# nicolasavru/objective-slam

Hardware: AMD Instinct MI355X
Metric: scene_ppf_votes_per_sec (higher is better)
Workload: dtype f32; 1 GPU; 5k-point model vs 100k-point scene (BASELINE.json metric config), one resident model table, Model::ppf_lookup per step; model_points=5000, scene_points=100000, ref_point_df=8, ref_points_per_gpu=12500, vote_mode=exact, parallelism=scene-ref-shard x1, exchange=single GPU

## Files before the change

include/oslam.h:

```cpp
#ifndef OSLAM_H
#define OSLAM_H

#include <stddef.h>
#include <stdint.h>

#ifdef __cplusplus
extern "C" {
#endif

#define OSLAM_OK 0
#define OSLAM_E_INVALID 1
#define OSLAM_E_DEVICE 2
#define OSLAM_E_NOMEM 3
#define OSLAM_E_NO_VOTES 4
#define OSLAM_E_LIMIT 5
#define OSLAM_E_PEER 6

#define OSLAM_VOTE_EXACT 0
#define OSLAM_VOTE_FAST 1

typedef struct oslam_params {
    unsigned ref_point_df;
    float vote_count_threshold;
    int cpu_clustering;
    int use_l1_norm;
    int use_averaged_clusters;
    int dev;
    int vote_mode;
    int shard_rank;
    int shard_world;
    unsigned max_cells;
    unsigned pose_gpu_min;
    int no_bucket_spread;
    unsigned scratch_gib;
    int pose_two_sorts;
    int vote_order;
    int reserved[1];
} oslam_params;

typedef struct oslam_stats {
    uint64_t num_scene_ppfs;
    uint64_t num_hits;
    uint64_t num_votes;
    uint64_t num_unique_votes;
    uint64_t num_model_keys;
    uint64_t num_top;
    uint32_t max_count;
    uint32_t num_emitted;
    float ms_vote;
    float ms_total;
    uint32_t vote_launches;
    float ms_vote_kernel;
    float ms_key_kernel;
    uint32_t wide_workgroups;
    uint64_t num_pairs_probed;
    uint64_t scratch_bytes;
    uint64_t num_entries_streamed;
    uint64_t num_items;
} oslam_stats;

typedef struct oslam_cell {
    uint64_t code;
    uint32_t count;
    uint32_t pad;
} oslam_cell;

typedef struct oslam_model oslam_model;
typedef struct oslam_scene oslam_scene;

int oslam_params_default(oslam_params *p);

int oslam_d_dist_from_cloud(const float *xyz, size_t n, size_t stride_bytes, float tau_d,
                            float *d_dist_out);

int oslam_model_create(const float *xyz, const float *nrm, size_t n, size_t stride_bytes,
                       float d_dist, const oslam_params *params, oslam_model **out);
void oslam_model_destroy(oslam_model *m);

int oslam_model_save(const oslam_model *m, const char *path);
int oslam_model_load(const char *path, const oslam_params *params, oslam_model **out);
int oslam_model_info(const oslam_model *m, size_t *n_points, float *d_dist, uint64_t *table_bytes);

int oslam_model_set_point_weights(oslam_model *m, const float *weights, size_t n);

int oslam_scene_create(const float *xyz, const float *nrm, size_t n, size_t stride_bytes,
                       float d_dist, unsigned ref_point_downsample_factor,
                       const oslam_params *params, oslam_scene **out);
void oslam_scene_destroy(oslam_scene *s);

int oslam_align(oslam_model *m, oslam_scene *s, float T_rowmajor[16], oslam_stats *stats);

int oslam_align_prepare(oslam_model *m, oslam_scene *s);

typedef struct oslam_db oslam_db;
int oslam_db_create(oslam_model *const *models, size_t n, oslam_db **out);
void oslam_db_destroy(oslam_db *db);
void oslam_db_destroy_with_models(oslam_db *db);
int oslam_db_align(oslam_db *db, oslam_scene *s, float *T_out, oslam_stats *stats);
int oslam_db_size(const oslam_db *db, size_t *n_models, size_t *n_groups);

int oslam_ppf_registration(const float *const *scene_xyz, const float *const *scene_nrm,
                           const size_t *scene_n, size_t n_scenes, const float *const *model_xyz,
                           const float *const *model_nrm, const size_t *model_n, size_t n_models,
                           size_t stride_bytes, const float *model_d_dists,
                           unsigned ref_point_downsample_factor, float vote_count_threshold,
                           int cpu_clustering, int use_l1_norm, int use_averaged_clusters, int devUse,
                           const float *model_weights, float *T_out);

int oslam_ht_dist(const float A[16], const float B[16], float out[2]);

int oslam_voxel_grid(const float *xyz, const float *nrm, size_t n, size_t stride_bytes, float leaf,
                     int dev, float *xyz_out, float *nrm_out, size_t cap, size_t *n_out);

typedef struct oslam_camera {
    float fx, fy, cx, cy;
    float depth_scale;
    float z_min, z_max;
    float max_jump;
} oslam_camera;
int oslam_depth_to_cloud(const void *depth, int depth_is_u16, int width, int height, const oslam_camera *cam,
// ... 594 lines not shown
    uint32_t hits;
    uint32_t normals;
    uint32_t bricks;
    uint32_t window_bricks;
    uint32_t launches;
    int32_t anchor[3], box_lo[3], box_hi[3];
    float ms_total;
} oslam_world_raycast_result;

int oslam_world_raycast_params_default(oslam_world_raycast_params *p);
int oslam_world_raycast(oslam_world *w, oslam_volume *vol, const oslam_world_raycast_params *rp, const float T_vol_cam[16],
                        const oslam_camera *cam, int width, int height, oslam_view **view_out, oslam_world_raycast_result *res);
int oslam_world_track(oslam_world *w, oslam_volume *vol, const oslam_world_raycast_params *rp, oslam_view *v,
                      const float T_vol_cam_prev[16], const oslam_egomotion_params *ep, float T_vol_cam_out[16],
                      oslam_egomotion_result *ego_res);

#define OSLAM_NORMALS_SWEEPS 4
typedef struct oslam_normals_params {
    float radius;
    unsigned min_neighbours;
    float viewpoint[3];
    int orient;
    float line_ratio;
    int reserved[4];
} oslam_normals_params;

typedef struct oslam_normals_result {
    uint32_t n_valid;
    uint32_t n_cells;
    float edge;
    uint32_t launches;
    float ms_total;
    float ms_grid, ms_kernel;
} oslam_normals_result;

int oslam_normals_params_default(oslam_normals_params *p);
int oslam_cloud_normals(const float *xyz, size_t n, size_t stride_bytes, const oslam_normals_params *np, int dev,
                        float *nrm_out, float *curvature_out, uint8_t *valid_out, oslam_normals_result *res);
int oslam_cloud_normal_moments(const float *xyz, size_t n, size_t stride_bytes, const oslam_normals_params *np, int dev,
                               int64_t *moments_out);
int oslam_mesh_normals(const float *xyz, size_t nv, size_t stride_bytes, const uint32_t *tri, size_t nt, float *nrm_out,
                       uint8_t *valid_out);
int oslam_ply_read_mesh(const char *path, float **xyz_out, float **nrm_out, uint32_t **tri_out, size_t *nv_out,
                        size_t *nt_out);

typedef struct oslam_colour_params {
    unsigned max_weight;
    float band;
    int reserved[6];
} oslam_colour_params;

int oslam_view_set_colour(oslam_view *v, const uint8_t *rgb, size_t row_stride_bytes, const uint8_t *valid);
int oslam_view_colour(oslam_view *v, uint32_t *rgba_out);
int oslam_view_has_colour(const oslam_view *v);
int oslam_colour_params_default(oslam_colour_params *p);
int oslam_volume_colour_enable(oslam_volume *vol, const oslam_colour_params *cp);
int oslam_volume_colour_words(oslam_volume *vol, uint32_t *words_out);
int oslam_volume_set_colour_words(oslam_volume *vol, const uint32_t *words);
int oslam_volume_integrate_colour(oslam_volume *vol, const oslam_view *v, const oslam_view *c, const float T_vol_cam[16],
                                  oslam_integrate_result *res, uint32_t *coloured_out);
int oslam_volume_colours(oslam_volume *vol, const float *xyz, size_t n, size_t stride_bytes, uint8_t *rgb_out,
                         uint8_t *valid_out, size_t *n_valid_out);
int oslam_volume_paint_view(oslam_volume *vol, const float T_vol_cam[16], oslam_view *v, uint32_t *painted_out);
int oslam_ply_write_colour(const char *path, const float *xyz, const float *nrm, const uint8_t *rgb, size_t n, int binary);
int oslam_ply_write_mesh_colour(const char *path, const float *xyz, const float *nrm, const uint8_t *rgb, size_t nv,
                                const uint32_t *tri, size_t nt, int binary);
int oslam_world_colours(oslam_world *w, oslam_volume *vol, const oslam_world_surface_params *sp, const float *xyz, size_t n,
                        size_t stride_bytes, uint8_t *rgb_out, uint8_t *valid_out, size_t *n_valid_out);
int oslam_world_paint_view(oslam_world *w, oslam_volume *vol, const oslam_world_surface_params *sp, const float T_vol_cam[16],
                           oslam_view *v, uint32_t *painted_out);

int oslam_scene_keys(oslam_scene *s, size_t ref_index, uint32_t *keys_out);
int oslam_model_keys(oslam_model *m, size_t ref_index, uint32_t *keys_out);
int oslam_model_bucket(oslam_model *m, uint32_t key, uint32_t *pairs_out, size_t cap,
                       size_t *count_out);
int oslam_model_bucket_words(oslam_model *m, uint32_t key, int slice, uint32_t *words_out, size_t cap,
                             size_t *count_out);
int oslam_model_key_numbers(oslam_model *m, uint32_t *keys_out, uint32_t *numbers_out, uint64_t *weights_out, size_t cap,
                            size_t *n_out);
int oslam_vote_ref_order(const uint32_t *keep, size_t n, uint32_t *order_out);
int oslam_vote_accumulator(oslam_model *m, oslam_scene *s, size_t ref_index, uint32_t *acc_out);
int oslam_vote_hits(oslam_model *m, oslam_scene *s, size_t ref_index, uint32_t *numbers_out, uint32_t *theta_out,
                    uint32_t *idx_out, size_t cap, size_t *n_out, uint32_t *keep_out);
int oslam_sort_hits_tap(const uint32_t *numbers, const uint32_t *theta, const uint32_t *idx, const uint32_t *offsets,
                        const uint32_t *counts, size_t n_lists, uint32_t id_bits, int dev, uint32_t *numbers_out,
                        uint32_t *theta_out, uint32_t *idx_out, uint32_t *runs_out, uint32_t *run_counts_out);
int oslam_last_cells(oslam_model *m, oslam_cell *cells_out, float *poses_out, size_t cap,
                     size_t *n_out);
int oslam_tail_scores(oslam_model *m, oslam_scene *s, const oslam_cell *cells, size_t n, uint32_t global_max, int path,
                      oslam_cell *cells_out, float *scores_out, size_t cap, size_t *n_out, uint32_t *max_idx_out,
                      float T[16], int *path_out);

int oslam_set_stream(void *hip_stream);
int oslam_release_scratch(int dev);
const char *oslam_last_error(void);
int oslam_set_host_threads(int n);
int oslam_selftest_math(size_t n, uint64_t seed, uint64_t *mismatches);

#ifdef __cplusplus
}
#endif
#endif
```

objective-slam_amd/csrc/oslam_host.c:

```c
#include <pthread.h>
#include <stdio.h>

#include "oslam_internal.h"

static __thread char g_err[512];
static __thread void *g_stream;

const char *oslam_last_error(void) { return g_err; }

int oslam_set_stream(void *hip_stream)
{
    g_stream = hip_stream;
    return OSLAM_OK;
}

void *oslam_stream(void) { return g_stream; }

int oslam_fail(int code, const char *what)
{
    if (what != g_err) snprintf(g_err, sizeof g_err, "%s", what);
    return code;
}

int oslam_fail_call(const char *call, int err, const char *file, int line)
{
    snprintf(g_err, sizeof g_err, "%s: %s (%s:%d)", call, hipGetErrorString((hipError_t)err), file, line);
    return OSLAM_E_DEVICE;
}

int oslam_params_default(oslam_params *p)
{
    if (!p) return fail(OSLAM_E_INVALID, "params is NULL");
    memset(p, 0, sizeof *p);
    p->ref_point_df = 1;
    p->vote_count_threshold = 0.4f;
    p->cpu_clustering = 0;
    p->use_l1_norm = 0;
    p->use_averaged_clusters = 0;
    p->dev = 0;
    p->vote_mode = OSLAM_VOTE_EXACT;
    p->shard_rank = 0;
    p->shard_world = 1;
    p->max_cells = 1u << 22;
    p->pose_gpu_min = 0;
    p->no_bucket_spread = 0;
    p->scratch_gib = 0;
    p->vote_order = 0;
    return OSLAM_OK;
}

int oslam_d_dist_from_cloud(const float *xyz, size_t n, size_t stride_bytes, float tau_d,
                            float *d_dist_out)
{
    float lo[3], hi[3], ext;
    size_t i;
    int a;
    if (!xyz || !d_dist_out || n == 0 || stride_bytes < 12) return fail(OSLAM_E_INVALID, "bad cloud");
    for (a = 0; a < 3; a++) lo[a] = hi[a] = xyz[a];
    for (i = 1; i < n; i++) {
        const float *p = (const float *)((const char *)xyz + i * stride_bytes);
        for (a = 0; a < 3; a++) {
            if (p[a] < lo[a]) lo[a] = p[a];
            if (p[a] > hi[a]) hi[a] = p[a];
        }
    }
    ext = hi[0] - lo[0];
    if (hi[1] - lo[1] > ext) ext = hi[1] - lo[1];
    if (hi[2] - lo[2] > ext) ext = hi[2] - lo[2];
    *d_dist_out = tau_d * ext;
    return OSLAM_OK;
}

int oslam_pick_device(int dev_req, int *dev_out)
{
    int n = 0;
    hipError_t e = hipGetDeviceCount(&n);
    if (e != hipSuccess || n <= 0) return fail(OSLAM_E_DEVICE, "no HIP device available (the PPF path has no CPU fallback)");
    if (dev_req < 0) dev_req = 0;
    *dev_out = dev_req < n - 1 ? dev_req : n - 1;
    e = hipSetDevice(*dev_out);
    if (e != hipSuccess) return fail(OSLAM_E_DEVICE, hipGetErrorString(e));
    return OSLAM_OK;
}

#define DEVCACHE_SLOTS 64
#define DEVCACHE_MAX_BLOCK ((size_t)1 << 30)
typedef struct {
    void *p;
    size_t bytes;
    int dev, used;
} devblock;
static devblock g_devcache[DEVCACHE_SLOTS];
static pthread_mutex_t g_devcache_mu = PTHREAD_MUTEX_INITIALIZER;

int oslam_dev_alloc(void **out, size_t bytes)
{
    int dev = 0, i, best = -1, spare = -1;
    hipError_t e;
    size_t want;
    *out = NULL;
    if (bytes == 0) bytes = 16;
    if (hipGetDevice(&dev) != hipSuccess) return (int)hipErrorInvalidDevice;
    pthread_mutex_lock(&g_devcache_mu);
    for (i = 0; i < DEVCACHE_SLOTS; i++) {
        devblock *b = &g_devcache[i];
        if (!b->p) { if (spare < 0) spare = i; continue; }
        if (b->used || b->dev != dev || b->bytes < bytes || b->bytes > 2 * bytes + 65536) continue;
        if (best < 0 || b->bytes < g_devcache[best].bytes) best = i;
    }
    if (best >= 0) {
        g_devcache[best].used = 1;
        *out = g_devcache[best].p;
        pthread_mutex_unlock(&g_devcache_mu);
        return 0;
    }
    want = bytes <= DEVCACHE_MAX_BLOCK ? bytes + bytes / 8 + 256 : bytes;
    e = hipMalloc(out, want);
    if (e != hipSuccess) {
        (void)hipGetLastError();
        for (i = 0; i < DEVCACHE_SLOTS; i++)
            if (g_devcache[i].p && !g_devcache[i].used && g_devcache[i].dev == dev) {
                (void)hipFree(g_devcache[i].p);
                memset(&g_devcache[i], 0, sizeof g_devcache[i]);
                if (spare < 0) spare = i;
            }
        want = bytes;
        e = hipMalloc(out, want);
    }
    if (e == hipSuccess && spare >= 0 && want <= DEVCACHE_MAX_BLOCK) {
        g_devcache[spare].p = *out;
// ... 35 lines not shown
```

objective-slam_amd/csrc/oslam_internal.h:

```cpp
#ifndef OSLAM_INTERNAL_H
#define OSLAM_INTERNAL_H

#include <hip/hip_runtime_api.h>
#include <limits.h>
#include <stddef.h>
#include <stdint.h>
#include <stdlib.h>
#include <string.h>
#include <time.h>

#include "oslam.h"
#include "oslam_kernels.h"
#include "oslam_rigid.h"

typedef struct cloud_buf {
    int n;
    float *h_xyz, *h_nrm;
    float *d_soa;
    oslamk_cloud k;
} cloud_buf;

struct oslam_model {
    int dev;
    cloud_buf c;
// ... 73 lines not shown
    int dev;
    oslam_view *view;
    size_t n_hyp;
    int32_t *d_labels;
    float *d_tol;
};

typedef struct db_group {
    int n;
    size_t *members;
    uint32_t *ukeys, *reach, *kmap, *uids;
} db_group;

struct oslam_db {
    int dev;
    size_t n;
    oslam_model **models;
    int n_groups;
    db_group *groups;
};

int oslam_fail(int code, const char *what);
static inline int fail(int code, const char *what) { return oslam_fail(code, what); }
int oslam_fail_call(const char *call, int err, const char *file, int line);

#define KCHK(call)                                                                          \
    do {                                                                                    \
        const int k_ = (int)(call);                                                         \
        if (k_ != 0) { rc = oslam_fail_call(#call, k_, __FILE__, __LINE__); goto done; }    \
    } while (0)
#define HIPCHK(call) KCHK(call)

static inline double now_ms(void)
{
    struct timespec ts;
    clock_gettime(CLOCK_MONOTONIC, &ts);
    return ts.tv_sec * 1e3 + ts.tv_nsec * 1e-6;
}

static inline size_t align256(size_t b) { return (b + 255) & ~(size_t)255; }

static inline int oslam_counters_open(uint32_t **d_cnt, size_t n_words, void *stream)
{
    const int k = oslam_dev_alloc((void **)d_cnt, 256 + sizeof(uint32_t) * n_words);
    return k != 0 ? k : (int)hipMemsetAsync(*d_cnt, 0, 256, (hipStream_t)stream);
}

static inline void split_points(const float *pts6, size_t n, float *xyz_out, float *nrm_out)
{
    size_t i;
    for (i = 0; i < n; i++) {
        memcpy(xyz_out + 3 * i, pts6 + 6 * i, 3 * sizeof(float));
        memcpy(nrm_out + 3 * i, pts6 + 6 * i + 3, 3 * sizeof(float));
    }
}

void *oslam_stream(void);
int oslam_pick_device(int dev_req, int *dev_out);

void oslam_cloud_free(cloud_buf *c);
int oslam_cloud_make(cloud_buf *c, const float *xyz, const float *nrm, size_t stride, const float *d_aos6, size_t n);
oslamk_cloud oslam_soa_cloud(const float *d_soa, size_t n);
int oslam_depth_points(const void *depth, int depth_is_u16, int width, int height, const oslam_camera *cam, int dev,
                       void **d_img, float **d_pts6, uint32_t *np);

int oslam_build_kmap(oslamk_table *t, float d_dist, const oslamk_table *parts, int n_parts, int vote_order);
int oslam_build_union(oslam_model *m, uint32_t distinct, uint32_t *d_n_keys, uint32_t *d_overflow);
int oslam_build_uinfo(oslam_model *m);

void oslam_refine_release_grids(oslam_scene *s);

typedef struct scratch_pool scratch_pool;
int oslam_check_pair(const oslam_model *m, const oslam_scene *s);
int oslam_pool_enter(int dev, scratch_pool **pool);
void oslam_pool_unlock(scratch_pool *p);
int oslam_pool_reserve_counts(scratch_pool *p, size_t n_ref);
void oslam_ref_order(const uint32_t *keep, size_t n, uint32_t *order);
typedef struct oslam_vote_times {
    float ms;
    float ms_vote_kernel, ms_key_kernel;
    uint32_t launches;
    uint64_t probed;
} oslam_vote_times;
int oslam_pool_read_hits(const scratch_pool *p, uint32_t *numbers_out, uint32_t *theta_out, uint32_t *idx_out, size_t cap,
                         size_t *n_out, uint32_t *keep_out);
int oslam_run_votes_group(scratch_pool *pool, oslam_model *const *ms, int nm, oslam_scene *s, const uint32_t *d_ref_idx,
                          const float *d_tsg, int n_ref, uint32_t fixed_gmax, uint32_t *acc_dump, oslamk_counters *cnt,
                          oslam_vote_times *t);
void oslam_vote_stats(oslam_stats *st, const scratch_pool *pool, const oslam_model *m, const oslam_scene *s,
                      const oslamk_counters *cnt, const oslam_vote_times *t);
int oslam_vote_records(scratch_pool *pool, oslam_model *m, oslam_scene *s, oslamk_counters *cnt, size_t *n_cells,
                       oslam_stats *st, int to_host);
int oslam_grow_records(oslam_model *m, uint64_t need);
int oslam_cluster_scores_on_device(size_t n, const float *trans, const float *quat, const float *wv,
                                   const int32_t *cell, const uint32_t *hash_idx, float d_dist, int use_l1,
                                   float *score);

typedef struct oslam_inst_req {
    oslamk_inst_args a;
    const oslam_instance_params *ip;
    float extent;
} oslam_inst_req;
size_t oslam_pose_gpu_from(const oslam_model *m);
void oslam_drop_last(oslam_model *m);
int oslam_pose_tables(oslam_model *m, oslam_scene *s);
int oslam_ensure_pose_buffers(oslam_model *m, size_t n);
const float *oslam_rotx(void);
int oslam_finish_after_votes(oslam_model *m, oslam_scene *s, size_t n, uint32_t gmax, int try_device, float T[16],
                             oslam_stats *stats, const oslam_inst_req *req, oslamk_inst_out *sel);

int oslam_db_align_frame(oslam_db *db, oslam_scene *s, float *T_out, oslam_stats *stats, const oslam_inst_req *reqs,
                         oslamk_inst_out *sels);

int oslam_refine_check_params(const oslam_refine_params *rp, oslam_refine_params *out);
int oslam_refine_check_rigid(const float T[16]);
int oslam_refine_members(oslam_model *const *ms, size_t n, oslam_scene *s, const float *T_in, const oslam_refine_params *p,
                         float *T_out, oslam_refine_result *res);

int oslam_view_check_pair(const oslam_model *m, const oslam_view *v);
int oslam_check_poses(oslam_model *const *ms, const float *T, size_t n, int hypotheses);
int oslam_check_handles(oslam_model *const *ms, const float *T, size_t n, const oslam_view *v);
int oslam_view_camera_ok(const oslam_camera *cam, int width, int height, int with_depth_scale, int with_max_jump);
int oslam_view_new(int dev, int width, int height, const oslam_camera *cam, oslam_view **out);
void oslam_view_camera(const oslam_view *v, oslam_camera *cam);

int oslam_verify_check_params(const oslam_verify_params *vp, oslam_verify_params *out);
void oslam_verify_fill_result(oslam_verify_result *r, const uint32_t *c, const oslam_verify_params *p);
void oslam_verify_set_member(oslamk_verify_member *d, const oslam_model *m, const float T[16], float depth_tol);
int oslam_verify_members(oslam_model *const *ms, size_t n, const oslam_view *v, const float *T, const oslam_verify_params *p,
                         oslam_verify_result *res);

int oslam_track_check_params(const oslam_track_params *tp, oslam_track_params *out);
void oslam_track_release_maps(oslam_view *v);
void oslam_track_release(void);
int oslam_track_view_maps(oslam_view *v, int *built);
void oslam_ego_release(void);
int oslam_ego_check_params(const oslam_egomotion_params *ep, oslam_egomotion_params *out);
int oslam_ego_check_pyramid_schedule(const oslam_egomotion_params *p, unsigned n_levels);
typedef struct oslam_ego_pair {
    oslam_view *src, *dst;
    unsigned lattice;
} oslam_ego_pair;
int oslam_ego_run(const oslam_ego_pair *pair, const float T0[16], const oslam_egomotion_params *p, float T_out[16],
                  oslam_egomotion_result *res);
int oslam_pyramid_check_params(const oslam_pyramid_params *pp, oslam_pyramid_params *out);
void oslam_volume_lock(void);
void oslam_volume_unlock(void);
static inline size_t oslam_volume_bytes(const oslam_volume_params *p)
{
    return (size_t)p->nx * (size_t)p->ny * (size_t)p->nz * sizeof(uint32_t);
}
int oslam_volume_integrate_views(oslam_volume *vol, const oslam_view *v, const oslam_view *c, const float T_vol_cam[16],
                                 oslam_integrate_result *res, uint32_t *coloured);
void oslam_colour_release_view(oslam_view *v);
int oslam_surface_check_params(const oslam_surface_params *sp, oslam_surface_params *out);
int oslam_volume_surface_cloud(oslam_volume *vol, unsigned min_weight, int *dev, float **d_pts6, uint32_t *np);
struct oslam_world_stage;
int oslam_world_stage_fit(struct oslam_world_stage *st, size_t bytes);
int oslam_world_surface_check_params(const oslam_world_surface_params *sp, oslam_world_surface_params *out);
int oslam_world_surface_cloud(oslam_world *w, oslam_volume *vol, const oslam_world_surface_params *p, int *dev, float **d_pts6,
                              uint32_t *np);
typedef struct oslam_world_map {
    oslamk_brick_map m;
    uint8_t *d_map;
    uint32_t bricks, window_bricks, launches;
    int32_t anchor[3];
// ... 16 lines not shown
```

objective-slam_amd/csrc/oslam_kernels.h:

```cpp
#ifndef OSLAM_KERNELS_H
#define OSLAM_KERNELS_H

#include <stddef.h>
#include <stdint.h>

#ifdef __cplusplus
extern "C" {
#endif

#define OSLAMK_SLICE 2046
#define OSLAMK_ROWS 1024
#define OSLAMK_NBIN 32

typedef struct oslamk_slot {
    uint32_t key;
    uint32_t start;
    uint32_t len;
    uint32_t cur;
} oslamk_slot;

typedef struct oslamk_uv {
    float uy, uz;
} oslamk_uv;

typedef struct oslamk_entries {
    uint32_t *e4;
    oslamk_uv *uv;
    uint16_t *mi;
    uint32_t *pw;
    oslamk_uv *puv;
    uint16_t *pdir;
    uint32_t n_real;
} oslamk_entries;
#define OSLAMK_PSEG 4096
#ifndef OSLAMK_PDIR_SHIFT
#define OSLAMK_PDIR_SHIFT 0
#endif
#define OSLAMK_PDIR_CELLS_RAW(m) ((m) <= 1u ? 1u : 1u << (31 - __builtin_clz((m) - 1u)))
#define OSLAMK_PDIR_CELLS(n) (OSLAMK_PDIR_CELLS_RAW((n) << OSLAMK_PDIR_SHIFT) > 4096u ? 4096u : OSLAMK_PDIR_CELLS_RAW((n) << OSLAMK_PDIR_SHIFT))

typedef struct oslamk_cloud {
    const float *px, *py, *pz, *nx, *ny, *nz;
    int n;
} oslamk_cloud;

typedef struct oslamk_order {
    const float *sx, *sy, *sz;
    const uint32_t *perm;
    const float *box;
} oslamk_order;
#define OSLAMK_ORDER_GROUP 64

typedef struct oslamk_uinfo {
    uint32_t start;
    uint32_t len;
} oslamk_uinfo;

typedef struct oslamk_table {
    oslamk_slot *slots;
    uint32_t cap;
    uint32_t shift;
    int n_slices;
    uint32_t *ukeys;
    uint32_t ucap;
    uint32_t ushift;
    uint32_t *reach;
    uint32_t reach_words;
    uint32_t *kmap;
    uint32_t kmap_bins;
    uint32_t *uids;
    uint32_t n_ids, id_bits, uinfo_stride;
    oslamk_uinfo *uinfo;
} oslamk_table;
#define OSLAMK_UWEIGHTS(t) ((unsigned long long *)((t).uids + (t).ucap))
#define OSLAMK_KMAP_NONE 0xffffffffu
#define OSLAMK_KMAP_MAX_BINS 2048

#define OSLAMK_REACH_BINS 16384

typedef struct oslamk_counters {
    unsigned long long hits;
    unsigned long long votes;
    unsigned long long nonzero_cells;
    uint32_t gmax;
    uint32_t out_count;
    uint32_t redo_count;
    uint32_t redo_total;
    unsigned long long entries;
    unsigned long long items;
    unsigned long long prof[4];
    uint32_t list_overflow;
    uint32_t pad_;
} oslamk_counters;

typedef struct oslamk_cell {
    unsigned long long code;
    uint32_t count;
    uint32_t pad;
} oslamk_cell;

int oslamk_row_keys(oslamk_cloud c, int ref, float d_dist, float inv_d_dist, uint32_t *keys_out,
                    void *stream);

int oslamk_model_count(oslamk_cloud c, float d_dist, float inv_d_dist, oslamk_table t,
                       uint32_t *n_unique, uint32_t *overflow, void *stream);
int oslamk_table_scan(oslamk_table t, uint32_t *total_out, void *stream);
int oslamk_union_build(oslamk_table t, uint32_t *n_keys, uint32_t *overflow, void *stream);
int oslamk_reach_build(oslamk_table t, float d_dist, void *stream);
int oslamk_union_weights(oslamk_table t, unsigned long long *weights, void *stream);
int oslamk_kmap_build(oslamk_table t, float d_dist, void *stream);
int oslamk_model_fill(oslamk_cloud c, float d_dist, float inv_d_dist, oslamk_table t,
                      const float *tmg, oslamk_entries ent, void *stream);

int oslamk_bucket_spread(oslamk_table t, oslamk_entries ent, void *stream);
int oslamk_bucket_psort(oslamk_table t, oslamk_entries ent, void *stream);

typedef struct oslamk_pay {
    uint32_t theta_t22;
    uint32_t idx;
} oslamk_pay;

typedef struct oslamk_run {
    uint32_t slot_r;
    uint32_t first;
} oslamk_run;
#define OSLAMK_RUN_SHIFT 26

typedef struct oslamk_vote_args {
    oslamk_cloud scene;
    const uint32_t *ref_idx;
    const float *tsg;
    int n_ref;
    float d_dist, inv_d_dist;
    oslamk_table table;
    oslamk_entries ent;
    float thresh;
    uint32_t fixed_gmax;
    oslamk_counters *counters;
    oslamk_cell *out;
    uint32_t out_cap;
    uint32_t *acc_dump;
    int dump_ref;
    int first_ref;
    int n_launch;
    int mode;
    uint32_t *keep_count;
    const uint32_t *hit_off;
    uint32_t *hit_key;
    oslamk_pay *hit_pay;
    oslamk_pay *hit_sorted;
    oslamk_run *runs;
    uint32_t *hit_count;
    uint32_t *run_count;
    uint32_t *redo;
    const uint32_t *ref_order;
    oslamk_order order;
} oslamk_vote_args;

int oslamk_uinfo_build(oslamk_table t, void *stream);

int oslamk_scene_count(const oslamk_vote_args *a, void *stream);
int oslamk_scene_hits(const oslamk_vote_args *a, void *stream);
int oslamk_sort_hits(const oslamk_vote_args *a, void *stream);
int oslamk_vote(const oslamk_vote_args *a, void *stream);
int oslamk_vote_wide(const oslamk_vote_args *a, void *stream);
int oslamk_vote_group(const oslamk_vote_args *d_all, const oslamk_vote_args *h_all, int nm, void *stream);

int oslamk_voxel_grid(oslamk_cloud c, float leaf, float *out6, uint32_t *n_out, void *stream);

int oslamk_depth_to_cloud(const void *d_img, int is_u16, int w, int h, float fx, float fy, float cx, float cy,
                          float scale, float z_min, float z_max, float max_jump, float *d_out6, uint32_t *n_out,
                          void *stream);

int oslam_dev_alloc(void **p, size_t bytes);
void oslam_dev_free(void *p);
void oslam_dev_cache_release(int dev);

int oslamk_aos6_to_soa(const float *d_in6, size_t n, float *d_soa, void *stream);

int oslamk_cluster_scores(int n, const int *cell, const uint32_t *shash, const uint32_t *sidx,
                          const float *sq, const float *st, const float *sw, float d_dist, int use_l1,
                          float *score, int whole_host, const unsigned long long *whole_dev, uint32_t *table, void *stream);
size_t oslamk_cluster_table_words(int n);

#define OSLAMK_MAX_INSTANCES 64
typedef struct oslamk_inst_args {
    uint32_t max_instances;
    float ratio, sep2, cos_thr;
    int32_t rot_on;
    float c[3];
} oslamk_inst_args;
typedef struct oslamk_inst_out {
    uint32_t n;
    uint32_t idx[OSLAMK_MAX_INSTANCES];
    float score[OSLAMK_MAX_INSTANCES];
    float T[OSLAMK_MAX_INSTANCES][16];
} oslamk_inst_out;

int oslamk_pose_stage(const oslamk_cell *d_cells_in, uint32_t n_in, float min_votecount, const float *d_Tm16,
                      const float *d_Ts16, uint32_t df, const float *d_weights, const float *h_rotx_cs, float d_dist,
                      int use_l1, oslamk_cell *d_cells_out, float *d_poses, uint32_t gmax, uint32_t model_points,
                      uint32_t scene_points, int two_sorts, const oslamk_inst_args *ia, uint32_t *n_out, uint32_t *best_out,
                      float T_best[16], oslamk_inst_out *inst, void *stream);

int oslamk_pose_reserve(uint32_t n_max, uint32_t slots, const float *h_rotx_cs, void *stream);
int oslamk_pose_select_async(const oslamk_cell *d_in, uint32_t n_in, float min_votecount, oslamk_cell *d_sel, uint32_t slot,
                             void *stream);
uint32_t oslamk_pose_selected(uint32_t slot);
int oslamk_pose_finish_async(uint32_t n, const oslamk_cell *d_sel, const float *d_Tm16, const float *d_Ts16, uint32_t df,
                             const float *d_weights, float d_dist, int use_l1, oslamk_cell *d_cells_out, float *d_poses,
                             uint32_t gmax, uint32_t model_points, uint32_t scene_points, int two_sorts,
                             const oslamk_inst_args *ia, uint32_t slot, void *stream);
void oslamk_pose_result(uint32_t slot, uint32_t *best_out, float T_best[16]);
int oslamk_pose_scores(uint32_t n, float *h_score, void *stream);
void oslamk_pose_instances(uint32_t slot, oslamk_inst_out *out);

int oslamk_select_cells(const oslamk_cell *d_in, uint32_t n_in, float min_votecount, oslamk_cell *d_out, uint32_t *n_out,
                        void *stream);
void oslamk_pose_release(void);

int oslamk_selftest(const float *x, const float *y, const float *x2, size_t n, float *out_acos,
                    float *out_atan2, uint32_t *out_quant, uint32_t *out_bin, void *stream);

#define OSLAMK_REFINE_THREADS 256
#define OSLAMK_REFINE_SUMS 29
#define OSLAMK_REFINE_STRIDE 32
#define OSLAMK_SCAN_ITEMS 4096
#define OSLAMK_GRID_MAX_CELLS (1u << 24)
#define OSLAMK_REFINE_STEP 0
#define OSLAMK_REFINE_SCORE 1
#define OSLAMK_REFINE_TAP 2

typedef struct oslamk_grid {
    double lo[3];
    double inv_edge;
    int dim[3];
    uint32_t n_cells;
    int n;
    uint32_t *start;
    float *pts;
    uint32_t *local;
    uint32_t *bsum;
// ... 328 lines not shown
```

objective-slam_amd/csrc/oslam_model.c:

```c
#include <stdio.h>

#include "oslam_internal.h"
#include "oslam_pose.h"
#include "ppf_core.h"

void oslam_model_destroy(oslam_model *m)
{
    if (!m) return;
    (void)hipSetDevice(m->dev);
    oslam_cloud_free(&m->c);
    if (m->table.slots) (void)hipFree(m->table.slots);
    if (m->ent.e4) (void)hipFree(m->ent.e4);
    if (m->ent.uv) (void)hipFree(m->ent.uv);
    if (m->ent.pw) (void)hipFree(m->ent.pw);
    if (m->ent.puv) (void)hipFree(m->ent.puv);
    if (m->ent.pdir) (void)hipFree(m->ent.pdir);
    if (m->ent.mi) (void)hipFree(m->ent.mi);
    if (m->table.ukeys && !m->shared_union) (void)hipFree(m->table.ukeys);
    if (m->table.reach && !m->shared_union) (void)hipFree(m->table.reach);
    if (m->table.kmap && !m->shared_union) (void)hipFree(m->table.kmap);
    if (m->table.uids && !m->shared_union) (void)hipFree(m->table.uids);
    if (m->d_counters) (void)hipFree(m->d_counters);
    if (m->d_out) (void)hipFree(m->d_out);
    if (m->d_union) (void)hipFree(m->d_union);
    if (m->table.uinfo) (void)hipFree(m->table.uinfo);
    if (m->d_Tm16) (void)hipFree(m->d_Tm16);
    if (m->d_weights) (void)hipFree(m->d_weights);
    if (m->d_pose_cells) (void)hipFree(m->d_pose_cells);
    if (m->d_pose_T) (void)hipFree(m->d_pose_T);
    free(m->h_out);
    free(m->weights);
    free(m->last_cells);
    free(m->last_poses);
    free(m->h_slots);
    free(m);
}

typedef struct key_rank {
    uint64_t weight;
    uint32_t key, slot;
} key_rank;

static void rank_pass(const key_rank *src, key_rank *dst, size_t n, int by_weight, unsigned shift, uint32_t *count)
{
    size_t i;
    uint32_t run = 0, d;
    memset(count, 0, sizeof(uint32_t) * 65536);
    for (i = 0; i < n; i++) {
        d = by_weight ? 0xffffu - (uint32_t)((src[i].weight >> shift) & 0xffffu) : (src[i].key >> shift) & 0xffffu;
        count[d]++;
    }
    for (d = 0; d < 65536; d++) {
        const uint32_t c = count[d];
        count[d] = run;
        run += c;
    }
    for (i = 0; i < n; i++) {
        d = by_weight ? 0xffffu - (uint32_t)((src[i].weight >> shift) & 0xffffu) : (src[i].key >> shift) & 0xffffu;
        dst[count[d]++] = src[i];
    }
}

static key_rank *rank_keys(key_rank *r, key_rank *tmp, size_t n, uint32_t *count)
{
    uint64_t top = 0;
    unsigned shift;
    size_t i;
    key_rank *t;
    for (i = 0; i < n; i++) if (r[i].weight > top) top = r[i].weight;
    for (shift = 0; shift < 32; shift += 16) {
        rank_pass(r, tmp, n, 0, shift, count);
        t = r; r = tmp; tmp = t;
    }
    for (shift = 0; shift < 64 && (top >> shift); shift += 16) {
        rank_pass(r, tmp, n, 1, shift, count);
        t = r; r = tmp; tmp = t;
    }
    return r;
}

int oslam_build_kmap(oslamk_table *t, float d_dist, const oslamk_table *parts, int n_parts, int vote_order)
{
    int rc = OSLAM_OK, j;
    uint32_t h_reach[OSLAMK_REACH_BINS / 32], w, top = 0, n_ids = 0, slot;
    uint32_t *h_keys = NULL, *h_ids = NULL, *count = NULL;
    uint64_t *h_w = NULL;
    key_rank *r = NULL, *r2 = NULL, *res;
    const size_t ucap = t->ucap;
    const int ranked = vote_order == 0 || vote_order == 2;
    t->kmap = NULL;
    t->kmap_bins = 0;
    t->reach_words = 0;
    t->uids = NULL;
    t->n_ids = t->id_bits = t->uinfo_stride = 0;
    HIPCHK(hipMalloc((void **)&t->uids, (sizeof(uint32_t) + sizeof(uint64_t)) * ucap));
    HIPCHK(hipMemsetAsync(t->uids, 0, (sizeof(uint32_t) + sizeof(uint64_t)) * ucap, (hipStream_t)oslam_stream()));
    for (j = 0; j < n_parts; j++) {
        oslamk_table p = parts[j];
        p.ukeys = t->ukeys;
// ... 6 lines not shown
    h_w = (uint64_t *)malloc(sizeof(uint64_t) * ucap);
    count = (uint32_t *)malloc(sizeof(uint32_t) * 65536);
    if (!h_keys || !h_ids || !h_w || !count) { rc = fail(OSLAM_E_NOMEM, "host allocation failed"); goto done; }
    HIPCHK(hipStreamSynchronize((hipStream_t)oslam_stream()));
    HIPCHK(hipMemcpy(h_keys, t->ukeys, sizeof(uint32_t) * ucap, hipMemcpyDeviceToHost));
    HIPCHK(hipMemcpy(h_w, OSLAMK_UWEIGHTS(*t), sizeof(uint64_t) * ucap, hipMemcpyDeviceToHost));
    for (slot = 0; slot < ucap; slot++) n_ids += h_keys[slot] != 0u;
    if (ranked) {
        size_t i = 0;
        r = (key_rank *)malloc(sizeof *r * (n_ids ? n_ids : 1));
        r2 = (key_rank *)malloc(sizeof *r2 * (n_ids ? n_ids : 1));
        if (!r || !r2) { rc = fail(OSLAM_E_NOMEM, "host allocation failed"); goto done; }
        for (slot = 0; slot < ucap; slot++)
            if (h_keys[slot] != 0u) {
                r[i].weight = h_w[slot];
                r[i].key = h_keys[slot];
                r[i].slot = slot;
                i++;
            }
        res = rank_keys(r, r2, n_ids, count);
        for (i = 0; i < n_ids; i++) h_ids[res[i].slot] = (uint32_t)i;
    } else {
        uint32_t next = 0;
        for (slot = 0; slot < ucap; slot++)
            if (h_keys[slot] != 0u) h_ids[slot] = next++;
    }
    HIPCHK(hipMemcpy(t->uids, h_ids, sizeof(uint32_t) * ucap, hipMemcpyHostToDevice));
    t->n_ids = n_ids;
    t->id_bits = 1;
    while (t->id_bits < 32u && ((uint64_t)1 << t->id_bits) < (uint64_t)n_ids) t->id_bits++;
    t->uinfo_stride = (n_ids + 63u) & ~63u;
    if (t->uinfo_stride == 0) t->uinfo_stride = 64;
    HIPCHK(hipMemcpy(h_reach, t->reach, sizeof h_reach, hipMemcpyDeviceToHost));
    for (w = 0; w < OSLAMK_REACH_BINS / 32; w++)
        if (h_reach[w]) {
            t->reach_words = w + 1;
            top = 32u * w + (32u - (uint32_t)__builtin_clz(h_reach[w]));
        }
    t->kmap_bins = top < OSLAMK_KMAP_MAX_BINS ? top : OSLAMK_KMAP_MAX_BINS;
    if (t->kmap_bins) {
        HIPCHK(hipMalloc((void **)&t->kmap, sizeof(uint32_t) * (size_t)t->kmap_bins * PC_ANGLE_COMBOS));
        KCHK(oslamk_kmap_build(*t, d_dist, oslam_stream()));
    }
done:
    free(h_keys);
    free(h_ids);
    free(h_w);
    free(count);
    free(r);
    free(r2);
    return rc;
}

int oslam_build_union(oslam_model *m, uint32_t distinct, uint32_t *d_n_keys, uint32_t *d_overflow)
{
    int rc = OSLAM_OK;
    uint32_t lg = 16;
    while ((1u << lg) < 4u * distinct && lg < OSLAMK_RUN_SHIFT) lg++;
    if ((1u << lg) < 2u * distinct) return fail(OSLAM_E_LIMIT, "more distinct pair keys than the union table can index");
    if (m->table.ukeys && !m->shared_union) (void)hipFree(m->table.ukeys);
    if (m->table.reach && !m->shared_union) (void)hipFree(m->table.reach);
    if (m->table.kmap && !m->shared_union) (void)hipFree(m->table.kmap);
    if (m->table.uids && !m->shared_union) (void)hipFree(m->table.uids);
    m->table.ukeys = NULL;
    m->table.reach = NULL;
    m->table.kmap = NULL;
    m->table.uids = NULL;
    m->shared_union = 0;
    m->table.ucap = 1u << lg;
    m->table.ushift = 32 - lg;
    HIPCHK(hipMalloc((void **)&m->table.ukeys, sizeof(uint32_t) * (size_t)m->table.ucap));
    HIPCHK(hipMemsetAsync(m->table.ukeys, 0, sizeof(uint32_t) * (size_t)m->table.ucap, (hipStream_t)oslam_stream()));
    HIPCHK(hipMemsetAsync(d_overflow, 0, sizeof(uint32_t), (hipStream_t)oslam_stream()));
    HIPCHK(hipMemsetAsync(d_n_keys, 0, sizeof(uint32_t), (hipStream_t)oslam_stream()));
    KCHK(oslamk_union_build(m->table, d_n_keys, d_overflow, oslam_stream()));
    HIPCHK(hipMalloc((void **)&m->table.reach, sizeof(uint32_t) * (OSLAMK_REACH_BINS / 32)));
    HIPCHK(hipMemsetAsync(m->table.reach, 0, sizeof(uint32_t) * (OSLAMK_REACH_BINS / 32), (hipStream_t)oslam_stream()));
    KCHK(oslamk_reach_build(m->table, m->d_dist, oslam_stream()));
    rc = oslam_build_kmap(&m->table, m->d_dist, &m->table, 1, m->params.vote_order);
done:
    return rc;
}

int oslam_build_uinfo(oslam_model *m)
{
    int rc = OSLAM_OK;
    const size_t bytes = sizeof(oslamk_uinfo) * (size_t)m->table.n_slices * (size_t)m->table.uinfo_stride;
    if (m->table.uinfo) { (void)hipFree(m->table.uinfo); m->table.uinfo = NULL; }
    HIPCHK(hipMalloc((void **)&m->table.uinfo, bytes));
    HIPCHK(hipMemsetAsync(m->table.uinfo, 0, bytes, (hipStream_t)oslam_stream()));
    KCHK(oslamk_uinfo_build(m->table, oslam_stream()));
done:
    return rc;
}

int oslam_model_create(const float *xyz, const float *nrm, size_t n, size_t stride_bytes,
                       float d_dist, const oslam_params *params, oslam_model **out)
{
    int rc = OSLAM_OK;
    oslam_model *m = NULL;
    uint32_t *d_small = NULL;
    uint32_t h_small[64 + 3];
    float *h_tmg = NULL, *d_tmg = NULL;
    int n_slices, s;
    uint32_t cap;
    size_t n_pairs;

    if (!out) return fail(OSLAM_E_INVALID, "out is NULL");
    *out = NULL;
    if (!xyz || !nrm || stride_bytes < 12 || !(d_dist > 0.0f)) return fail(OSLAM_E_INVALID, "bad model arguments");
    if (n < 2) return fail(OSLAM_E_INVALID, "model needs at least 2 points");
    if (n > 46340) return fail(OSLAM_E_LIMIT, "model larger than 46340 points (32-bit pair index, kernel.cu:433)");
    m = (oslam_model *)calloc(1, sizeof *m);
    if (!m) return fail(OSLAM_E_NOMEM, "host allocation failed");
    if (params) m->params = *params; else oslam_params_default(&m->params);
    if (m->params.max_cells == 0) m->params.max_cells = 1u << 22;
    rc = oslam_pick_device(m->params.dev, &m->dev);
    if (rc != OSLAM_OK) goto done;
    rc = oslam_cloud_make(&m->c, xyz, nrm, stride_bytes, NULL, n);
    if (rc != OSLAM_OK) goto done;
    oslam_cloud_shape(m->c.h_xyz, n, m->cm, m->inst_c, &m->inst_extent);
    m->d_dist = d_dist;
    m->inv_d_dist = 1.0f / d_dist;
    m->weights = (float *)malloc(sizeof(float) * n);
    if (!m->weights) { rc = fail(OSLAM_E_NOMEM, "host allocation failed"); goto done; }
    for (s = 0; s < (int)n; s++) m->weights[s] = 1.0f;

    n_slices = (int)((n + OSLAMK_SLICE - 1) / OSLAMK_SLICE);
    if (n_slices > 64) { rc = fail(OSLAM_E_LIMIT, "too many model slices"); goto done; }
    HIPCHK(hipMalloc((void **)&d_small, sizeof(uint32_t) * (64 + 3)));

    for (cap = 1u << 16;; cap <<= 1) {
        int grow = 0;
        uint32_t lg = 0;
        while ((1u << lg) < cap) lg++;
        if (m->table.slots) { (void)hipFree(m->table.slots); m->table.slots = NULL; }
        HIPCHK(hipMalloc((void **)&m->table.slots, sizeof(oslamk_slot) * (size_t)cap * n_slices));
        HIPCHK(hipMemsetAsync(m->table.slots, 0, sizeof(oslamk_slot) * (size_t)cap * n_slices, (hipStream_t)oslam_stream()));
        HIPCHK(hipMemsetAsync(d_small, 0, sizeof(uint32_t) * (64 + 3), (hipStream_t)oslam_stream()));
        m->table.cap = cap;
        m->table.shift = 32 - lg;
        m->table.n_slices = n_slices;
        KCHK(oslamk_model_count(m->c.k, m->d_dist, m->inv_d_dist, m->table, d_small, d_small + 64, oslam_stream()));
        HIPCHK(hipStreamSynchronize((hipStream_t)oslam_stream()));
        HIPCHK(hipMemcpy(h_small, d_small, sizeof h_small, hipMemcpyDeviceToHost));
        if (h_small[64]) grow = 1;
        for (s = 0; s < n_slices; s++) if (h_small[s] > cap / 2) grow = 1;
        if (!grow) break;
        if (cap >= (1u << 26)) { rc = fail(OSLAM_E_LIMIT, "model hash table would exceed 2^26 slots per slice"); goto done; }
    }
    KCHK(oslamk_table_scan(m->table, d_small + 65, oslam_stream()));
    {
        uint32_t sum = 0;
        for (s = 0; s < n_slices; s++) sum += h_small[s];
        rc = oslam_build_union(m, sum, d_small + 66, d_small + 64);
        if (rc != OSLAM_OK) goto done;
    }
    HIPCHK(hipStreamSynchronize((hipStream_t)oslam_stream()));
    HIPCHK(hipMemcpy(h_small, d_small, sizeof h_small, hipMemcpyDeviceToHost));
    if (h_small[64]) { rc = fail(OSLAM_E_LIMIT, "union key table overflow"); goto done; }
    m->n_entries = h_small[65];
    m->ent.n_real = m->n_entries;
    m->num_model_keys = (uint64_t)h_small[66] + 1;
    n_pairs = m->n_entries ? m->n_entries : 1;

    h_tmg = (float *)malloc(sizeof(float) * 8 * n);
    if (!h_tmg) { rc = fail(OSLAM_E_NOMEM, "host allocation failed"); goto done; }
    oslam_T_g_rows(m->c.h_xyz, m->c.h_nrm, NULL, n, h_tmg);
    HIPCHK(hipMalloc((void **)&d_tmg, sizeof(float) * 8 * n));
    HIPCHK(hipMemcpy(d_tmg, h_tmg, sizeof(float) * 8 * n, hipMemcpyHostToDevice));
    HIPCHK(hipMalloc((void **)&m->ent.e4, sizeof(uint32_t) * (n_pairs + 256)));
    HIPCHK(hipMalloc((void **)&m->ent.mi, sizeof(uint16_t) * n_pairs));
    if (m->params.vote_mode != OSLAM_VOTE_FAST)
        HIPCHK(hipMalloc((void **)&m->ent.uv, sizeof(oslamk_uv) * n_pairs));
// ... 194 lines not shown
        goto done;
    }
    sum = fnv64(sum, xyz, 12 * n);
    sum = fnv64(sum, nrm, 12 * n);
    sum = fnv64(sum, m->weights, 4 * n);
    sum = fnv64(sum, h_slots, sizeof(oslamk_slot) * n_slots);
    {
        uint64_t run = 0;
        for (i = 0; i < n_slots; i++) {
            if (h_slots[i].start != run || run + h_slots[i].len > hd.n_entries) {
                rc = fail(OSLAM_E_INVALID, "model file: a bucket lies outside the entry arrays or out of order");
                goto done;
            }
            run += ((uint64_t)h_slots[i].len + 3u) & ~(uint64_t)3u;
        }
    }
    rc = oslam_cloud_make(&m->c, xyz, nrm, 12, NULL, n);
    if (rc != OSLAM_OK) goto done;
    oslam_cloud_shape(m->c.h_xyz, n, m->cm, m->inst_c, &m->inst_extent);
    m->d_dist = hd.d_dist;
    m->inv_d_dist = hd.inv_d_dist;
    m->table.cap = hd.cap;
    m->table.shift = hd.shift;
    m->table.n_slices = (int)hd.n_slices;
    m->table.ucap = hd.ucap;
    m->table.ushift = hd.ushift;
    m->n_entries = hd.n_entries;
    m->ent.n_real = hd.n_entries;
    m->num_model_keys = hd.num_model_keys;
    n_pairs = hd.n_entries ? hd.n_entries : 1;
    HIPCHK(hipMalloc((void **)&m->table.slots, sizeof(oslamk_slot) * n_slots));
    HIPCHK(hipMalloc((void **)&m->table.ukeys, sizeof(uint32_t) * (size_t)hd.ucap));
    HIPCHK(hipMalloc((void **)&m->table.reach, sizeof(uint32_t) * (OSLAMK_REACH_BINS / 32)));
    HIPCHK(hipMalloc((void **)&m->ent.e4, sizeof(uint32_t) * (n_pairs + 256)));
    HIPCHK(hipMalloc((void **)&m->ent.mi, sizeof(uint16_t) * n_pairs));
    if (hd.has_uv) {
        HIPCHK(hipMalloc((void **)&m->ent.pw, sizeof(uint32_t) * n_pairs));
        HIPCHK(hipMalloc((void **)&m->ent.puv, sizeof(oslamk_uv) * n_pairs));
        HIPCHK(hipMalloc((void **)&m->ent.pdir, sizeof(uint16_t) * ((n_pairs + 256) << OSLAMK_PDIR_SHIFT)));
    }
    HIPCHK(hipMemcpy(m->table.slots, h_slots, sizeof(oslamk_slot) * n_slots, hipMemcpyHostToDevice));
    HIPCHK(hipMemsetD32Async((hipDeviceptr_t)m->ent.e4, (int)PC_ROW_SINK, n_pairs + 256, (hipStream_t)oslam_stream()));
    HIPCHK(hipStreamSynchronize((hipStream_t)oslam_stream()));
    rc = db_read_dev(f, m->table.ukeys, sizeof(uint32_t) * (size_t)hd.ucap, &sum);
    if (rc == OSLAM_OK) rc = db_read_dev(f, m->table.reach, sizeof(uint32_t) * (OSLAMK_REACH_BINS / 32), &sum);
    if (rc == OSLAM_OK) rc = db_read_dev(f, m->ent.e4, sizeof(uint32_t) * (size_t)hd.n_entries, &sum);
    if (rc == OSLAM_OK) rc = db_read_dev(f, m->ent.mi, sizeof(uint16_t) * (size_t)hd.n_entries, &sum);
    if (rc == OSLAM_OK && hd.has_uv) rc = db_read_dev(f, m->ent.pw, sizeof(uint32_t) * (size_t)hd.n_entries, &sum);
    if (rc == OSLAM_OK && hd.has_uv) rc = db_read_dev(f, m->ent.puv, sizeof(oslamk_uv) * (size_t)hd.n_entries, &sum);
    if (rc == OSLAM_OK && hd.has_uv) rc = db_read_dev(f, m->ent.pdir, sizeof(uint16_t) * ((size_t)hd.n_entries << OSLAMK_PDIR_SHIFT), &sum);
    if (rc != OSLAM_OK) goto done;
    if (sum != hd.checksum) { rc = fail(OSLAM_E_INVALID, "model file checksum mismatch"); goto done; }
    m->h_slots = h_slots;
    h_slots = NULL;
    rc = oslam_build_kmap(&m->table, m->d_dist, &m->table, 1, m->params.vote_order);
    if (rc != OSLAM_OK) goto done;
    rc = oslam_build_uinfo(m);
    if (rc != OSLAM_OK) goto done;
    HIPCHK(hipStreamSynchronize((hipStream_t)oslam_stream()));
    m->out_cap = m->params.max_cells;
    HIPCHK(hipMalloc((void **)&m->d_counters, sizeof(oslamk_counters)));
    HIPCHK(hipMalloc((void **)&m->d_out, sizeof(oslamk_cell) * (size_t)m->out_cap));
    m->h_out = (oslam_cell *)malloc(sizeof(oslam_cell) * (size_t)m->out_cap);
    if (!m->h_out) { rc = fail(OSLAM_E_NOMEM, "host allocation failed"); goto done; }
done:
    if (f) fclose(f);
    free(xyz);
    free(nrm);
    free(h_slots);
    if (rc != OSLAM_OK) { oslam_model_destroy(m); return rc; }
    *out = m;
    return OSLAM_OK;
}

int oslam_model_info(const oslam_model *m, size_t *n_points, float *d_dist, uint64_t *table_bytes)
{
    if (!m) return fail(OSLAM_E_INVALID, "NULL handle");
    if (n_points) *n_points = (size_t)m->c.n;
    if (d_dist) *d_dist = m->d_dist;
    if (table_bytes)
        *table_bytes = sizeof(oslamk_slot) * (uint64_t)m->table.cap * (uint64_t)m->table.n_slices +
                       sizeof(uint32_t) * (uint64_t)m->table.ucap + sizeof(uint32_t) * (OSLAMK_REACH_BINS / 32) +
                       sizeof(oslamk_uinfo) * (uint64_t)m->table.uinfo_stride * (uint64_t)m->table.n_slices +
                       (uint64_t)m->n_entries * (4 + 2 + (m->ent.pw ? 12 + (2 << OSLAMK_PDIR_SHIFT) : 0)) + 24ull * (uint64_t)m->c.n;
    return OSLAM_OK;
}

int oslam_model_set_point_weights(oslam_model *m, const float *weights, size_t n)
{
    if (!m || !weights || n != (size_t)m->c.n) return fail(OSLAM_E_INVALID, "bad weights");
    memcpy(m->weights, weights, sizeof(float) * n);
    if (m->d_weights) {
        if (hipSetDevice(m->dev) != hipSuccess ||
            hipMemcpy(m->d_weights, m->weights, sizeof(float) * n, hipMemcpyHostToDevice) != hipSuccess)
            return fail(OSLAM_E_DEVICE, "cannot update the weights on the device");
    }
    return OSLAM_OK;
}
```

objective-slam_amd/csrc/oslam_taps.c:

```c

#include "oslam_internal.h"
#include "oslam_pose.h"
#include "ppf_core.h"

static int cloud_row_keys(cloud_buf *c, size_t ref, float d_dist, uint32_t *keys_out)
{
    int rc = OSLAM_OK;
    uint32_t *d = NULL;
    if (!keys_out || ref >= (size_t)c->n) return fail(OSLAM_E_INVALID, "bad reference index");
    HIPCHK(hipMalloc((void **)&d, sizeof(uint32_t) * c->n));
    KCHK(oslamk_row_keys(c->k, (int)ref, d_dist, 1.0f / d_dist, d, oslam_stream()));
    HIPCHK(hipStreamSynchronize((hipStream_t)oslam_stream()));
    HIPCHK(hipMemcpy(keys_out, d, sizeof(uint32_t) * c->n, hipMemcpyDeviceToHost));
done:
    if (d) (void)hipFree(d);
    return rc;
}

int oslam_scene_keys(oslam_scene *s, size_t ref_index, uint32_t *keys_out)
{
    if (!s) return fail(OSLAM_E_INVALID, "NULL handle");
    if (!(s->d_dist > 0.0f)) return fail(OSLAM_E_INVALID, "this scene was made for models of any d_dist (d_dist 0): it has no keys of its own");
    if (hipSetDevice(s->dev) != hipSuccess) return fail(OSLAM_E_DEVICE, "hipSetDevice failed");
    return cloud_row_keys(&s->c, ref_index, s->d_dist, keys_out);
// ... 65 lines not shown
    *count_out = 0;
    if (hipSetDevice(m->dev) != hipSuccess) return fail(OSLAM_E_DEVICE, "hipSetDevice failed");
    tab = (oslamk_slot *)malloc(sizeof(oslamk_slot) * m->table.cap);
    if (!tab) return fail(OSLAM_E_NOMEM, "host allocation failed");
    HIPCHK(hipMemcpy(tab, m->table.slots + (size_t)slice * m->table.cap, sizeof(oslamk_slot) * m->table.cap, hipMemcpyDeviceToHost));
    mask = m->table.cap - 1;
    slot = (key * 2654435761u) >> m->table.shift;
    for (probe = 0; probe <= mask; probe++, slot = (slot + 1) & mask) {
        if (tab[slot].key == key) {
            size_t n = tab[slot].len < cap ? tab[slot].len : cap;
            *count_out = tab[slot].len;
            if (words_out && n) HIPCHK(hipMemcpy(words_out, m->ent.e4 + tab[slot].start, sizeof(uint32_t) * n, hipMemcpyDeviceToHost));
            break;
        }
        if (tab[slot].key == 0) break;
    }
done:
    free(tab);
    return rc;
}

typedef struct key_row {
    uint64_t weight;
    uint32_t key, number;
} key_row;

static int key_row_order(const void *a, const void *b)
{
    const uint32_t x = ((const key_row *)a)->key, y = ((const key_row *)b)->key;
    return x < y ? -1 : (x > y);
}

int oslam_model_key_numbers(oslam_model *m, uint32_t *keys_out, uint32_t *numbers_out, uint64_t *weights_out, size_t cap,
                            size_t *n_out)
{
    int rc = OSLAM_OK;
    uint32_t *h_keys = NULL, *h_ids = NULL, slot;
    uint64_t *h_w = NULL;
    key_row *rows = NULL;
    size_t n = 0, i, ucap;
    if (!m || !n_out) return fail(OSLAM_E_INVALID, "NULL argument");
    *n_out = 0;
    if (m->unusable || !m->table.ukeys || !m->table.uids) return fail(OSLAM_E_INVALID, "this model has no key tables");
    if (hipSetDevice(m->dev) != hipSuccess) return fail(OSLAM_E_DEVICE, "hipSetDevice failed");
    ucap = m->table.ucap;
    h_keys = (uint32_t *)malloc(sizeof(uint32_t) * ucap);
    h_ids = (uint32_t *)malloc(sizeof(uint32_t) * ucap);
    h_w = (uint64_t *)malloc(sizeof(uint64_t) * ucap);
    rows = (key_row *)malloc(sizeof *rows * ucap);
    if (!h_keys || !h_ids || !h_w || !rows) { rc = fail(OSLAM_E_NOMEM, "host allocation failed"); goto done; }
    HIPCHK(hipMemcpy(h_keys, m->table.ukeys, sizeof(uint32_t) * ucap, hipMemcpyDeviceToHost));
    HIPCHK(hipMemcpy(h_ids, m->table.uids, sizeof(uint32_t) * ucap, hipMemcpyDeviceToHost));
    HIPCHK(hipMemcpy(h_w, OSLAMK_UWEIGHTS(m->table), sizeof(uint64_t) * ucap, hipMemcpyDeviceToHost));
    for (slot = 0; slot < ucap; slot++)
        if (h_keys[slot] != 0u) {
            rows[n].key = h_keys[slot];
            rows[n].number = h_ids[slot];
            rows[n].weight = h_w[slot];
            n++;
        }
    qsort(rows, n, sizeof *rows, key_row_order);
    for (i = 0; i < n && i < cap; i++) {
        if (keys_out) keys_out[i] = rows[i].key;
        if (numbers_out) numbers_out[i] = rows[i].number;
        if (weights_out) weights_out[i] = rows[i].weight;
    }
    *n_out = n;
done:
    free(h_keys);
    free(h_ids);
    free(h_w);
    free(rows);
    return rc;
}

int oslam_vote_ref_order(const uint32_t *keep, size_t n, uint32_t *order_out)
{
    if ((!keep || !order_out) && n) return fail(OSLAM_E_INVALID, "NULL argument");
    oslam_ref_order(keep, n, order_out);
    return OSLAM_OK;
}

static int tap_one_ref(oslam_model *m, oslam_scene *s, size_t ref_index, uint32_t *acc_out, uint32_t *numbers_out,
                       uint32_t *theta_out, uint32_t *idx_out, size_t cap, size_t *n_out, uint32_t *keep_out)
{
    int rc = OSLAM_OK;
    uint32_t *d_dump = NULL, *d_ref = NULL, *h_dump = NULL;
    float *d_tsg = NULL;
    float rows[8];
    uint32_t ref = (uint32_t)ref_index;
    oslamk_counters cnt;
    scratch_pool *pool = NULL;
    size_t cells;
    rc = oslam_check_pair(m, s);
    if (rc != OSLAM_OK) return rc;
    if (ref_index >= (size_t)s->c.n) return fail(OSLAM_E_INVALID, "bad reference index");
    cells = (size_t)m->table.n_slices * OSLAMK_SLICE * OSLAMK_NBIN;
    oslam_T_g_rows(s->c.h_xyz, s->c.h_nrm, &ref, 1, rows);
    rc = oslam_pool_enter(m->dev, &pool);
    if (rc != OSLAM_OK) return rc;
    HIPCHK(hipMalloc((void **)&d_dump, sizeof(uint32_t) * cells));
    HIPCHK(hipMalloc((void **)&d_ref, sizeof(uint32_t)));
    HIPCHK(hipMalloc((void **)&d_tsg, sizeof rows));
    HIPCHK(hipMemcpy(d_ref, &ref, sizeof ref, hipMemcpyHostToDevice));
    HIPCHK(hipMemcpy(d_tsg, rows, sizeof rows, hipMemcpyHostToDevice));
    rc = oslam_run_votes_group(pool, &m, 1, s, d_ref, d_tsg, 1, 0xffffffffu, d_dump, &cnt, NULL);
    if (rc != OSLAM_OK) goto done;
    if (n_out) {
        rc = oslam_pool_read_hits(pool, numbers_out, theta_out, idx_out, cap, n_out, keep_out);
        if (rc != OSLAM_OK) goto done;
    }
    if (acc_out) {
        h_dump = (uint32_t *)malloc(sizeof(uint32_t) * cells);
        if (!h_dump) { rc = fail(OSLAM_E_NOMEM, "host allocation failed"); goto done; }
        HIPCHK(hipMemcpy(h_dump, d_dump, sizeof(uint32_t) * cells, hipMemcpyDeviceToHost));
        memcpy(acc_out, h_dump, sizeof(uint32_t) * OSLAMK_NBIN * (size_t)m->c.n);
    }
done:
    oslam_pool_unlock(pool);
    free(h_dump);
    if (d_dump) (void)hipFree(d_dump);
    if (d_ref) (void)hipFree(d_ref);
    if (d_tsg) (void)hipFree(d_tsg);
    return rc;
}

int oslam_vote_accumulator(oslam_model *m, oslam_scene *s, size_t ref_index, uint32_t *acc_out)
{
    if (!acc_out) return fail(OSLAM_E_INVALID, "bad reference index");
    return tap_one_ref(m, s, ref_index, acc_out, NULL, NULL, NULL, 0, NULL, NULL);
}

int oslam_vote_hits(oslam_model *m, oslam_scene *s, size_t ref_index, uint32_t *numbers_out, uint32_t *theta_out,
                    uint32_t *idx_out, size_t cap, size_t *n_out, uint32_t *keep_out)
{
    if (!n_out) return fail(OSLAM_E_INVALID, "NULL argument");
    *n_out = 0;
    return tap_one_ref(m, s, ref_index, NULL, numbers_out, theta_out, idx_out, cap, n_out, keep_out);
}

int oslam_sort_hits_tap(const uint32_t *numbers, const uint32_t *theta, const uint32_t *idx, const uint32_t *offsets,
                        const uint32_t *counts, size_t n_lists, uint32_t id_bits, int dev, uint32_t *numbers_out,
                        uint32_t *theta_out, uint32_t *idx_out, uint32_t *runs_out, uint32_t *run_counts_out)
{
    int rc = OSLAM_OK, devsel;
    size_t total, i, slots;
    oslamk_pay *h_pay = NULL;
    uint32_t *d_off = NULL, *d_cnt = NULL, *d_key = NULL, *d_rc = NULL;
    oslamk_pay *d_pay = NULL, *d_sorted = NULL;
    oslamk_run *d_runs = NULL;
    oslamk_vote_args a;
    hipStream_t st;
    if (!numbers || !theta || !idx || !offsets || !counts || !numbers_out || !theta_out || !idx_out || !runs_out || !run_counts_out)
        return fail(OSLAM_E_INVALID, "NULL argument");
    if (id_bits < 1u || id_bits > OSLAMK_RUN_SHIFT) return fail(OSLAM_E_INVALID, "id_bits outside 1 .. 26");
    if (n_lists > 0x7fffffffu) return fail(OSLAM_E_INVALID, "too many lists");
    for (i = 0; i < n_lists; i++)
        if (offsets[i + 1] < offsets[i]) return fail(OSLAM_E_INVALID, "the offsets descend");
    total = offsets[n_lists];
    for (i = 0; i < total; i++)
        if (numbers[i] >> id_bits) return fail(OSLAM_E_INVALID, "a key number does not fit id_bits");
    if (n_lists == 0) return OSLAM_OK;
    rc = oslam_pick_device(dev, &devsel);
    if (rc != OSLAM_OK) return rc;
    st = (hipStream_t)oslam_stream();
    slots = total ? total : 1;
    h_pay = (oslamk_pay *)malloc(sizeof *h_pay * slots);
    if (!h_pay) return fail(OSLAM_E_NOMEM, "host allocation failed");
    for (i = 0; i < total; i++) {
        h_pay[i].theta_t22 = theta[i];
        h_pay[i].idx = idx[i];
    }
    HIPCHK(hipMalloc((void **)&d_off, sizeof(uint32_t) * (n_lists + 1)));
    HIPCHK(hipMalloc((void **)&d_cnt, sizeof(uint32_t) * n_lists));
    HIPCHK(hipMalloc((void **)&d_rc, sizeof(uint32_t) * n_lists));
    HIPCHK(hipMalloc((void **)&d_key, sizeof(uint32_t) * slots));
    HIPCHK(hipMalloc((void **)&d_pay, sizeof(oslamk_pay) * slots));
    HIPCHK(hipMalloc((void **)&d_sorted, sizeof(oslamk_pay) * slots));
    HIPCHK(hipMalloc((void **)&d_runs, sizeof(oslamk_run) * slots));
    HIPCHK(hipMemcpy(d_off, offsets, sizeof(uint32_t) * (n_lists + 1), hipMemcpyHostToDevice));
    HIPCHK(hipMemcpy(d_cnt, counts, sizeof(uint32_t) * n_lists, hipMemcpyHostToDevice));
    if (total) {
        HIPCHK(hipMemcpy(d_key, numbers, sizeof(uint32_t) * total, hipMemcpyHostToDevice));
        HIPCHK(hipMemcpy(d_pay, h_pay, sizeof(oslamk_pay) * total, hipMemcpyHostToDevice));
    }
    HIPCHK(hipMemsetAsync(d_sorted, 0xA5, sizeof(oslamk_pay) * slots, st));
    HIPCHK(hipMemsetAsync(d_runs, 0xA5, sizeof(oslamk_run) * slots, st));
    HIPCHK(hipMemsetAsync(d_rc, 0xA5, sizeof(uint32_t) * n_lists, st));
    memset(&a, 0, sizeof a);
    a.hit_off = d_off;
    a.hit_count = d_cnt;
    a.hit_key = d_key;
    a.hit_pay = d_pay;
    a.hit_sorted = d_sorted;
    a.runs = d_runs;
    a.run_count = d_rc;
    a.table.id_bits = id_bits;
    a.n_launch = (int)n_lists;
    KCHK(oslamk_sort_hits(&a, st));
    HIPCHK(hipStreamSynchronize(st));
    HIPCHK(hipMemcpy(run_counts_out, d_rc, sizeof(uint32_t) * n_lists, hipMemcpyDeviceToHost));
    if (total) {
        HIPCHK(hipMemcpy(numbers_out, d_key, sizeof(uint32_t) * total, hipMemcpyDeviceToHost));
        HIPCHK(hipMemcpy(runs_out, d_runs, sizeof(oslamk_run) * total, hipMemcpyDeviceToHost));
        HIPCHK(hipMemcpy(h_pay, d_sorted, sizeof(oslamk_pay) * total, hipMemcpyDeviceToHost));
        for (i = 0; i < total; i++) {
            theta_out[i] = h_pay[i].theta_t22;
            idx_out[i] = h_pay[i].idx;
        }
    }
done:
    free(h_pay);
    if (d_off) (void)hipFree(d_off);
    if (d_cnt) (void)hipFree(d_cnt);
    if (d_rc) (void)hipFree(d_rc);
    if (d_key) (void)hipFree(d_key);
    if (d_pay) (void)hipFree(d_pay);
    if (d_sorted) (void)hipFree(d_sorted);
    if (d_runs) (void)hipFree(d_runs);
    return rc;
}
// ... 213 lines not shown
```

objective-slam_amd/csrc/oslam_vote.c:

```c
#include <pthread.h>
#include <stdio.h>

#include "oslam_internal.h"
#include "oslam_vote_plan.h"

int oslam_check_pair(const oslam_model *m, const oslam_scene *s)
{
    if (!m || !s) return fail(OSLAM_E_INVALID, "NULL handle");
    if (m->unusable) return fail(OSLAM_E_INVALID, "this model lost its key tables with its database: it can only be destroyed");
    if (m->dev != s->dev) return fail(OSLAM_E_INVALID, "model and scene live on different devices");
    if (s->d_dist != 0.0f && m->d_dist != s->d_dist) return fail(OSLAM_E_INVALID, "scene d_dist differs from the model's (ppf.cu:64-67)");
    return OSLAM_OK;
}

#define MAX_DEVICES 64
#define MAX_BATCH_EVENTS 64
#define N_EVENTS (4 + 3 * MAX_BATCH_EVENTS)
#define SLOT_BYTES (sizeof(oslamk_pay) * 2 + sizeof(oslamk_run) + sizeof(uint32_t))

enum { HOST_NONE, HOST_PINNED, HOST_MALLOC };
typedef struct pool_buf {
    void *d, *h;
    int host;
    size_t cap;
} pool_buf;

enum {
    BUF_HITS,
    BUF_COUNTS,
    BUF_CLUSTER,
    BUF_REDO,
    BUF_VARGS,
    BUF_ORDER,
    N_BUFS
};
static const int g_buf_host[N_BUFS] = {HOST_NONE, HOST_MALLOC, HOST_NONE, HOST_NONE, HOST_PINNED, HOST_PINNED};

struct scratch_pool {
    pthread_mutex_t lock;
    pool_buf b[N_BUFS];
    oslam_vote_plan plan;
    hipEvent_t ev[N_EVENTS];
    int have_events;
};
static scratch_pool g_pool[MAX_DEVICES];
static pthread_once_t g_pool_once = PTHREAD_ONCE_INIT;

static void pool_init_all(void)
{
    int i, k;
    for (i = 0; i < MAX_DEVICES; i++) {
        pthread_mutex_init(&g_pool[i].lock, NULL);
        for (k = 0; k < N_BUFS; k++) g_pool[i].b[k].host = g_buf_host[k];
    }
}

static __thread scratch_pool *g_cur_pool;

static scratch_pool *pool_lock(int dev)
{
    pthread_once(&g_pool_once, pool_init_all);
    if (dev < 0 || dev >= MAX_DEVICES) return NULL;
    pthread_mutex_lock(&g_pool[dev].lock);
    g_cur_pool = &g_pool[dev];
    return g_cur_pool;
}

void oslam_pool_unlock(scratch_pool *p)
{
    if (!p) return;
    g_cur_pool = NULL;
    pthread_mutex_unlock(&p->lock);
}

int oslam_pool_enter(int dev, scratch_pool **pool)
{
    *pool = NULL;
    if (hipSetDevice(dev) != hipSuccess) return fail(OSLAM_E_DEVICE, "hipSetDevice failed");
    *pool = pool_lock(dev);
    return *pool ? OSLAM_OK : fail(OSLAM_E_LIMIT, "device ordinal too large");
}

static void pool_buf_free(pool_buf *b)
{
    if (b->d) (void)hipFree(b->d);
    if (b->h && b->host == HOST_PINNED) (void)hipHostFree(b->h);
    if (b->host == HOST_MALLOC) free(b->h);
    b->d = NULL;
    b->h = NULL;
    b->cap = 0;
}

static int pool_buf_grow(pool_buf *b, size_t need, size_t cap, size_t d_bytes, size_t h_bytes)
{
    int rc = OSLAM_OK;
    if (b->cap >= need) return OSLAM_OK;
    pool_buf_free(b);
    HIPCHK(hipMalloc(&b->d, d_bytes));
    if (b->host == HOST_PINNED) HIPCHK(hipHostMalloc(&b->h, h_bytes, hipHostMallocDefault));
    if (b->host == HOST_MALLOC && !(b->h = malloc(h_bytes))) { rc = fail(OSLAM_E_NOMEM, "host allocation failed"); goto done; }
    b->cap = cap;
done:
    if (rc != OSLAM_OK) pool_buf_free(b);
    return rc;
}

int oslam_release_scratch(int dev)
{
    scratch_pool *p = pool_lock(dev);
    int i, any;
    if (!p) return fail(OSLAM_E_INVALID, "device ordinal out of range");
    any = p->have_events;
    for (i = 0; i < N_BUFS; i++) any |= p->b[i].d != NULL || p->b[i].h != NULL;
    if (any) {
        if (hipSetDevice(dev) != hipSuccess) { oslam_pool_unlock(p); return fail(OSLAM_E_DEVICE, "hipSetDevice failed"); }
        for (i = 0; i < N_BUFS; i++) pool_buf_free(&p->b[i]);
        oslamk_pose_release();
        if (p->have_events)
            for (i = 0; i < N_EVENTS; i++) (void)hipEventDestroy(p->ev[i]);
        p->have_events = 0;
    }
    if (hipSetDevice(dev) == hipSuccess) oslam_dev_cache_release(dev);
    oslam_arbitrate_release();
    oslam_track_release();
    oslam_ego_release();
    free(p->plan.b);
    memset(&p->plan, 0, sizeof p->plan);
    oslam_pool_unlock(p);
    return OSLAM_OK;
}

static size_t scratch_limit(const oslam_model *m)
{
    return (size_t)(m && m->params.scratch_gib > 0 ? m->params.scratch_gib : 4) << 30;
}

int oslam_pool_reserve_counts(scratch_pool *p, size_t n_ref)
{
    int rc = OSLAM_OK, i;
    const size_t cap = n_ref + n_ref / 4 + 64;
    if (!p->have_events) {
        for (i = 0; i < N_EVENTS; i++) HIPCHK(hipEventCreate(&p->ev[i]));
        p->have_events = 1;
    }
    rc = pool_buf_grow(&p->b[BUF_COUNTS], n_ref, cap, sizeof(uint32_t) * (5 * cap + 2), sizeof(uint32_t) * (3 * cap + 2));
done:
    return rc;
}

static int pool_reserve_slots(scratch_pool *p, size_t slots, size_t limit)
{
    pool_buf *b = &p->b[BUF_HITS];
    const size_t base = (slots ? slots : 1) * SLOT_BYTES + 1024;
    size_t want = base;
    if (b->cap >= want) return OSLAM_OK;
    pool_buf_free(b);
    want += want / 8;
    if (want > limit + 1024) want = base > limit + 1024 ? base : limit + 1024;
    if (hipMalloc(&b->d, want) != hipSuccess) {
        (void)hipGetLastError();
        b->d = NULL;
        want = base;
        if (hipMalloc(&b->d, want) != hipSuccess) {
            (void)hipGetLastError();
            b->d = NULL;
            return fail(OSLAM_E_NOMEM, "no device memory for the hit lists");
        }
    }
    b->cap = want;
    return OSLAM_OK;
}

static void carve_scratch(oslamk_vote_args *a, const scratch_pool *p, size_t slots)
{
    char *b = (char *)p->b[BUF_HITS].d;
    a->redo = (uint32_t *)p->b[BUF_REDO].d;
    a->hit_pay = (oslamk_pay *)b;
    b += slots * sizeof(oslamk_pay);
    a->hit_sorted = (oslamk_pay *)b;
    b += slots * sizeof(oslamk_pay);
    a->runs = (oslamk_run *)b;
    b += slots * sizeof(oslamk_run);
    a->hit_key = (uint32_t *)b;
}

int oslam_pool_read_hits(const scratch_pool *p, uint32_t *numbers_out, uint32_t *theta_out, uint32_t *idx_out, size_t cap,
                         size_t *n_out, uint32_t *keep_out)
{
    int rc = OSLAM_OK;
    oslamk_vote_args a;
    oslamk_pay *pay = NULL;
    uint32_t n = 0;
    size_t i, m;
    *n_out = 0;
    if (keep_out) *keep_out = ((const uint32_t *)p->b[BUF_COUNTS].h)[0];
    if (p->plan.nb < 1) return OSLAM_OK;
    carve_scratch(&a, p, p->plan.b[0].slots);
    HIPCHK(hipMemcpy(&n, (const uint32_t *)p->b[BUF_COUNTS].d + p->b[BUF_COUNTS].cap, sizeof n, hipMemcpyDeviceToHost));
    *n_out = n;
    m = n < cap ? n : cap;
    if (!m) return OSLAM_OK;
    pay = (oslamk_pay *)malloc(sizeof *pay * m);
    if (!pay) return fail(OSLAM_E_NOMEM, "host allocation failed");
    HIPCHK(hipMemcpy(pay, a.hit_sorted, sizeof *pay * m, hipMemcpyDeviceToHost));
    if (numbers_out) {
        HIPCHK(hipMemcpy(numbers_out, a.hit_key, sizeof(uint32_t) * m, hipMemcpyDeviceToHost));
        for (i = 0; i < m; i++) numbers_out[i] &= 0x7fffffffu;
    }
    for (i = 0; i < m; i++) {
        if (theta_out) theta_out[i] = pay[i].theta_t22;
        if (idx_out) idx_out[i] = pay[i].idx;
    }
done:
    free(pay);
    return rc;
}

#define REF_ORDER_CLASSES 1024
void oslam_ref_order(const uint32_t *keep, size_t n, uint32_t *order)
{
    uint32_t start[REF_ORDER_CLASSES + 1], top = 0;
    size_t i;
    int c;
    for (i = 0; i < n; i++) if (keep[i] > top) top = keep[i];
    if (top == 0) top = 1;
    memset(start, 0, sizeof start);
    for (i = 0; i < n; i++) start[1 + (REF_ORDER_CLASSES - 1) - (int)((uint64_t)keep[i] * (REF_ORDER_CLASSES - 1) / top)]++;
    for (c = 0; c < REF_ORDER_CLASSES; c++) start[c + 1] += start[c];
    for (i = 0; i < n; i++) order[start[(REF_ORDER_CLASSES - 1) - (int)((uint64_t)keep[i] * (REF_ORDER_CLASSES - 1) / top)]++] = (uint32_t)i;
}

typedef struct vote_pass {
    scratch_pool *pool;
    oslam_model *const *ms;
    int nm, n_ref;
    hipStream_t st;
    oslamk_vote_args a;
    uint32_t *d_keep, *d_hitc, *d_runc, *d_off, *h_keep, *h_off;
    size_t limit;
    size_t widest;
    size_t redo_stride;
    int ordered;
    int one_grid;
} vote_pass;

static void member_args(oslamk_vote_args *a, const oslam_model *m)
{
    a->table.uinfo = m->table.uinfo;
    a->table.n_slices = m->table.n_slices;
    a->table.slots = m->table.slots;
    a->table.cap = m->table.cap;
    a->ent = m->ent;
    a->thresh = m->params.vote_count_threshold;
    a->counters = m->d_counters;
    a->out = m->d_out;
    a->out_cap = m->out_cap;
    a->mode = (m->params.vote_mode == OSLAM_VOTE_FAST) ? 1 : 0;
}

static void pass_open(vote_pass *v, scratch_pool *pool, oslam_model *const *ms, int nm, const oslam_scene *s,
                      const uint32_t *d_ref_idx, const float *d_tsg, int n_ref, uint32_t fixed_gmax, uint32_t *acc_dump)
{
    int j;
    memset(v, 0, sizeof *v);
    v->pool = pool;
    v->ms = ms;
    v->nm = nm;
    v->n_ref = n_ref;
    v->st = (hipStream_t)oslam_stream();
    v->limit = scratch_limit(ms[0]);
    v->widest = 1;
    for (j = 0; j < nm; j++) if ((size_t)ms[j]->table.n_slices > v->widest) v->widest = (size_t)ms[j]->table.n_slices;
    v->ordered = (ms[0]->params.vote_order == 0 || ms[0]->params.vote_order == 3) && !acc_dump && n_ref > 1;
    v->one_grid = nm > 1 && n_ref > 0 && !acc_dump && ((size_t)n_ref + 7) / 8 * 8 * v->widest <= 2048;
    for (j = 1; j < nm && v->one_grid; j++)
        if ((ms[j]->params.vote_mode == OSLAM_VOTE_FAST) != (ms[0]->params.vote_mode == OSLAM_VOTE_FAST)) v->one_grid = 0;
    v->a.scene = s->c.k;
    v->a.order = s->order;
    v->a.ref_idx = d_ref_idx;
    v->a.tsg = d_tsg;
    v->a.n_ref = n_ref;
    v->a.d_dist = ms[0]->d_dist;
    v->a.inv_d_dist = ms[0]->inv_d_dist;
    v->a.table = ms[0]->table;
    v->a.fixed_gmax = fixed_gmax;
    v->a.acc_dump = acc_dump;
    v->a.dump_ref = acc_dump ? 0 : -1;
    member_args(&v->a, ms[0]);
}

static int pass_reserve(vote_pass *v)
{
    scratch_pool *pool = v->pool;
    const size_t n = (size_t)(v->n_ref > 0 ? v->n_ref : 1), nm = (size_t)v->nm;
    size_t need, cap;
    int rc = oslam_pool_reserve_counts(pool, n);
    if (rc != OSLAM_OK) return rc;
    need = v->redo_stride = (n + 7) / 8 * 8 * v->widest;
    if (nm > 1) need *= nm;
    cap = need + need / 4;
    rc = pool_buf_grow(&pool->b[BUF_REDO], need, cap, sizeof(uint32_t) * cap, 0);
    if (rc != OSLAM_OK) return rc;
    if (v->ordered) {
        cap = n + n / 4 + 64;
        rc = pool_buf_grow(&pool->b[BUF_ORDER], n, cap, sizeof(uint32_t) * cap, sizeof(uint32_t) * cap);
        if (rc != OSLAM_OK) return rc;
    }
    if (v->one_grid) {
        cap = nm + nm / 2 + 8;
        rc = pool_buf_grow(&pool->b[BUF_VARGS], nm, cap, sizeof(oslamk_vote_args) * cap, sizeof(oslamk_vote_args) * cap);
        if (rc != OSLAM_OK) return rc;
    }
    cap = pool->b[BUF_COUNTS].cap;
    v->d_keep = (uint32_t *)pool->b[BUF_COUNTS].d;
    v->d_hitc = v->d_keep + cap;
    v->d_runc = v->d_hitc + cap;
    v->d_off = v->d_runc + cap;
    v->h_keep = (uint32_t *)pool->b[BUF_COUNTS].h;
    v->h_off = v->h_keep + cap;
    return OSLAM_OK;
}

static int pass_demand(vote_pass *v, oslam_vote_times *t)
{
    int rc = OSLAM_OK, i;
    hipEvent_t *ev = v->pool->ev;
    float k0 = 0.0f;
    uint64_t sum = 0;
    if (v->n_ref <= 0) return OSLAM_OK;
    HIPCHK(hipMemsetAsync(v->d_keep, 0, sizeof(uint32_t) * (size_t)v->n_ref, v->st));
    v->a.first_ref = 0;
    v->a.n_launch = v->n_ref;
    v->a.keep_count = v->d_keep;
    KCHK(oslamk_scene_count(&v->a, oslam_stream()));
    HIPCHK(hipEventRecord(ev[2], v->st));
    HIPCHK(hipMemcpyAsync(v->h_keep, v->d_keep, sizeof(uint32_t) * (size_t)v->n_ref, hipMemcpyDeviceToHost, v->st));
    HIPCHK(hipStreamSynchronize(v->st));
    HIPCHK(hipEventElapsedTime(&k0, ev[0], ev[2]));
    if (t) {
        for (i = 0; i < v->n_ref; i++) sum += v->h_keep[i];
        t->ms_key_kernel += k0;
        t->probed = sum;
    }
done:
    return rc;
}

static int pass_plan(vote_pass *v)
{
    oslam_vote_plan *plan = &v->pool->plan;
    int rc = OSLAM_OK;
    if (oslam_vote_plan_build(plan, v->h_keep, v->n_ref, v->limit / SLOT_BYTES, v->h_off) != 0)
        return fail(OSLAM_E_NOMEM, "host allocation failed");
    rc = pool_reserve_slots(v->pool, plan->max_slots, v->limit);
    if (rc != OSLAM_OK) return rc;
    if (plan->n_off) HIPCHK(hipMemcpyAsync(v->d_off, v->h_off, sizeof(uint32_t) * plan->n_off, hipMemcpyHostToDevice, v->st));
    v->one_grid = v->one_grid && oslam_vote_plan_is_one_batch(plan);
done:
    return rc;
}

static int pass_batch(vote_pass *v, int nb)
{
    scratch_pool *pool = v->pool;
    const oslam_vote_batch *b = &pool->plan.b[nb];
    oslamk_vote_args *a = &v->a, *d_vargs = (oslamk_vote_args *)pool->b[BUF_VARGS].d, *h_vargs = (oslamk_vote_args *)pool->b[BUF_VARGS].h;
    hipEvent_t *ev = nb < MAX_BATCH_EVENTS ? pool->ev + 4 + 3 * nb : NULL;
    int rc = OSLAM_OK, j;
    a->first_ref = b->first;
    a->n_launch = b->n;
    a->keep_count = NULL;
    a->hit_off = v->d_off + b->off_at;
    a->hit_count = v->d_hitc;
    a->run_count = v->d_runc;
    carve_scratch(a, pool, b->slots);
    HIPCHK(hipMemsetAsync(v->d_hitc, 0, sizeof(uint32_t) * (size_t)b->n, v->st));
    if (ev) HIPCHK(hipEventRecord(ev[0], v->st));
    KCHK(oslamk_scene_hits(a, oslam_stream()));
    KCHK(oslamk_sort_hits(a, oslam_stream()));
    if (ev) HIPCHK(hipEventRecord(ev[1], v->st));
    a->ref_order = NULL;
    if (v->ordered) {
        uint32_t *d_order = (uint32_t *)pool->b[BUF_ORDER].d + b->first, *h_order = (uint32_t *)pool->b[BUF_ORDER].h + b->first;
        oslam_ref_order(v->h_keep + b->first, (size_t)b->n, h_order);
        HIPCHK(hipMemcpyAsync(d_order, h_order, sizeof(uint32_t) * (size_t)b->n, hipMemcpyHostToDevice, v->st));
        a->ref_order = d_order;
    }
    for (j = 0; j < v->nm; j++) {
        member_args(a, v->ms[j]);
        if (v->one_grid) {
            a->redo = (uint32_t *)pool->b[BUF_REDO].d + (size_t)j * v->redo_stride;
            h_vargs[j] = *a;
            continue;
        }
        KCHK(oslamk_vote(a, oslam_stream()));
        HIPCHK(hipMemsetAsync(&v->ms[j]->d_counters->redo_count, 0, sizeof(uint32_t), v->st));
    }
    if (v->one_grid) {
        HIPCHK(hipMemcpyAsync(d_vargs, h_vargs, sizeof(oslamk_vote_args) * (size_t)v->nm, hipMemcpyHostToDevice, v->st));
        KCHK(oslamk_vote_group(d_vargs, h_vargs, v->nm, oslam_stream()));
    }
    if (ev) HIPCHK(hipEventRecord(ev[2], v->st));
done:
    return rc;
}

static int pass_collect(vote_pass *v, oslamk_counters *cnt, oslam_vote_times *t)
{
    scratch_pool *pool = v->pool;
    const oslamk_vote_args *h_vargs = (const oslamk_vote_args *)pool->b[BUF_VARGS].h;
    hipEvent_t *ev = pool->ev;
    int rc = OSLAM_OK, i, j, again = 0;
    HIPCHK(hipEventRecord(ev[1], v->st));
    for (j = 0; j < v->nm; j++) HIPCHK(hipMemcpyAsync(&cnt[j], v->ms[j]->d_counters, sizeof *cnt, hipMemcpyDeviceToHost, v->st));
    HIPCHK(hipStreamSynchronize(v->st));
    for (j = 0; j < v->nm && v->one_grid; j++)
        if (cnt[j].redo_count) {
            KCHK(oslamk_vote_wide(&h_vargs[j], oslam_stream()));
            HIPCHK(hipMemcpyAsync(&cnt[j], v->ms[j]->d_counters, sizeof *cnt, hipMemcpyDeviceToHost, v->st));
            again = 1;
        }
    if (again) HIPCHK(hipStreamSynchronize(v->st));
    for (j = 0; j < v->nm; j++)
        if (cnt[j].list_overflow)
            return fail(OSLAM_E_DEVICE, cnt[j].list_overflow & 1u
                            ? "a hit list overflowed: the counting pass and the hit pass disagreed on the pairs within reach"
                            : cnt[j].list_overflow & 2u ? "near-edge search: a hit's key number lies outside the model's bucket records"
                            : cnt[j].list_overflow & 4u ? "near-edge search: a bucket lies outside the model's entry arrays"
                                                        : "near-edge search: a directory place lies outside its bucket segment");
    if (!t) return OSLAM_OK;
    HIPCHK(hipEventElapsedTime(&t->ms, ev[0], ev[1]));
    for (i = 0; i < pool->plan.nb && i < MAX_BATCH_EVENTS; i++) {
        float k = 0.0f, vk = 0.0f;
        HIPCHK(hipEventElapsedTime(&k, ev[4 + 3 * i], ev[4 + 3 * i + 1]));
        HIPCHK(hipEventElapsedTime(&vk, ev[4 + 3 * i + 1], ev[4 + 3 * i + 2]));
        t->ms_key_kernel += k;
        t->ms_vote_kernel += vk;
    }
    t->launches += (uint32_t)pool->plan.nb;
done:
    return rc;
}

int oslam_run_votes_group(scratch_pool *pool, oslam_model *const *ms, int nm, oslam_scene *s, const uint32_t *d_ref_idx,
                          const float *d_tsg, int n_ref, uint32_t fixed_gmax, uint32_t *acc_dump, oslamk_counters *cnt,
                          oslam_vote_times *t)
{
    vote_pass v;
    int rc = OSLAM_OK, j, nb;
    pass_open(&v, pool, ms, nm, s, d_ref_idx, d_tsg, n_ref, fixed_gmax, acc_dump);
    rc = pass_reserve(&v);
    if (rc != OSLAM_OK) return rc;
    for (j = 0; j < nm; j++) HIPCHK(hipMemsetAsync(ms[j]->d_counters, 0, sizeof(oslamk_counters), v.st));
    HIPCHK(hipEventRecord(pool->ev[0], v.st));
    rc = pass_demand(&v, t);
    if (rc == OSLAM_OK) rc = pass_plan(&v);
    for (nb = 0; rc == OSLAM_OK && nb < pool->plan.nb; nb++) rc = pass_batch(&v, nb);
    if (rc == OSLAM_OK) rc = pass_collect(&v, cnt, t);
done:
    return rc;
}

static int run_votes(scratch_pool *pool, oslam_model *m, oslam_scene *s, uint32_t fixed_gmax, oslamk_counters *cnt,
                     oslam_vote_times *t)
{
    const int rc = oslam_run_votes_group(pool, &m, 1, s, s->d_ref_idx, s->d_tsg, s->n_ref, fixed_gmax, NULL, cnt, t);
    if (rc == OSLAM_OK && fixed_gmax) cnt->gmax = fixed_gmax;
    return rc;
}

int oslam_grow_records(oslam_model *m, uint64_t need)
{
    oslamk_cell *d_new = NULL;
    oslam_cell *h_new;
    if (need > ((uint64_t)1 << 28)) return fail(OSLAM_E_LIMIT, "more than 2^28 accumulator peaks above the threshold");
    if (hipMalloc((void **)&d_new, sizeof(oslamk_cell) * need) != hipSuccess) {
        (void)hipGetLastError();
        return fail(OSLAM_E_NOMEM, "no device memory for the accumulator peaks");
    }
    h_new = (oslam_cell *)malloc(sizeof(oslam_cell) * need);
    if (!h_new) { (void)hipFree(d_new); return fail(OSLAM_E_NOMEM, "host allocation failed"); }
    (void)hipFree(m->d_out);
    free(m->h_out);
    m->d_out = d_new;
    m->h_out = h_new;
    m->out_cap = (uint32_t)need;
    m->n_local = 0;
    return OSLAM_OK;
}

void oslam_vote_stats(oslam_stats *st, const scratch_pool *pool, const oslam_model *m, const oslam_scene *s,
                      const oslamk_counters *cnt, const oslam_vote_times *t)
{
    st->num_scene_ppfs = (uint64_t)s->n_ref * (uint64_t)(s->c.n - 1);
    st->num_hits = cnt->hits;
    st->num_votes = cnt->votes;
    st->num_unique_votes = cnt->nonzero_cells;
    st->num_model_keys = m->num_model_keys;
    st->max_count = cnt->gmax;
    st->num_emitted = cnt->out_count;
    st->ms_vote = t->ms;
    st->ms_vote_kernel = t->ms_vote_kernel;
    st->ms_key_kernel = t->ms_key_kernel;
    st->vote_launches = t->launches;
    st->num_pairs_probed = t->probed;
    st->num_entries_streamed = cnt->entries;
    st->num_items = cnt->items;
    st->wide_workgroups = cnt->redo_total;
    st->scratch_bytes = pool->b[BUF_HITS].cap;
}

int oslam_vote_records(scratch_pool *pool, oslam_model *m, oslam_scene *s, oslamk_counters *cnt, size_t *n_cells,
                       oslam_stats *st, int to_host)
{
    int rc = OSLAM_OK;
    oslam_vote_times t;
    float ms_first;
    memset(&t, 0, sizeof t);
    rc = run_votes(pool, m, s, 0, cnt, &t);
    if (rc != OSLAM_OK) return rc;
    ms_first = t.ms;
    t.ms = 0.0f;
    if (cnt->out_count > m->out_cap) {
        const uint32_t g = cnt->gmax;
        rc = run_votes(pool, m, s, g, cnt, &t);
        if (rc != OSLAM_OK) return rc;
        if (cnt->out_count > m->out_cap) {
            rc = oslam_grow_records(m, (uint64_t)cnt->out_count + cnt->out_count / 8 + 1024);
            if (rc == OSLAM_OK) rc = run_votes(pool, m, s, g, cnt, &t);
            if (rc != OSLAM_OK) return rc;
            if (cnt->out_count > m->out_cap)
                return fail(OSLAM_E_LIMIT, "more accumulator peaks than the record buffer after growing it");
        }
    }
    t.ms += ms_first;
    if (getenv("OSLAM_PROF"))
        fprintf(stderr, "[oslam prof] k_vote wave cycles: pre-scan %llu, voting %llu, wait at the barrier behind it %llu, "
                        "of the voting: near-edge search %llu\n",
                cnt->prof[0], cnt->prof[1], cnt->prof[2], cnt->prof[3]);
    *n_cells = cnt->out_count;
    if (to_host && *n_cells) HIPCHK(hipMemcpy(m->h_out, m->d_out, sizeof(oslam_cell) * *n_cells, hipMemcpyDeviceToHost));
    if (st) oslam_vote_stats(st, pool, m, s, cnt, &t);
done:
    return rc;
}

int oslam_cluster_scores_on_device(size_t n, const float *trans, const float *quat, const float *wv,
                                    const int32_t *cell, const uint32_t *hash_idx, float d_dist, int use_l1,
                                    float *score)
{
    int rc = OSLAM_OK;
    char *d = NULL, *h = NULL;
    const size_t o_c = 0, o_sh = o_c + 12 * n, o_si = o_sh + 4 * n, o_sq = o_si + 4 * n,
                 o_st = o_sq + 16 * n, o_sw = o_st + 12 * n, o_sc = o_sw + 4 * n, o_tab = o_sc + 4 * n,
                 total = o_tab + 4 * oslamk_cluster_table_words((int)n);
    size_t j;
    int whole = 1;
    uint64_t whole_sum = 0;
    hipStream_t st = (hipStream_t)oslam_stream();
    h = (char *)malloc(o_sc);
    if (!h) return OSLAM_E_NOMEM;
    memcpy(h + o_c, cell, 12 * n);
    for (j = 0; j < n; j++) {
        const uint32_t o = hash_idx[2 * j + 1];
        ((uint32_t *)(h + o_sh))[j] = hash_idx[2 * j];
        ((uint32_t *)(h + o_si))[j] = o;
        memcpy(h + o_sq + 16 * j, quat + 4 * o, 16);
        memcpy(h + o_st + 12 * j, trans + 3 * o, 12);
        ((float *)(h + o_sw))[j] = wv[o];
        if (whole && wv[o] >= 0.0f && wv[o] < 16777216.0f && wv[o] == (float)(uint32_t)wv[o]) whole_sum += (uint32_t)wv[o];
        else whole = 0;
    }
    if (whole_sum >= (1u << 24) - 1u) whole = 0;
    if (!g_cur_pool) { rc = OSLAM_E_DEVICE; goto done; }
    rc = pool_buf_grow(&g_cur_pool->b[BUF_CLUSTER], total, total + total / 4, total + total / 4, 0);
    if (rc != OSLAM_OK) goto done;
    d = (char *)g_cur_pool->b[BUF_CLUSTER].d;
    HIPCHK(hipMemcpyAsync(d, h, o_sc, hipMemcpyHostToDevice, st));
    KCHK(oslamk_cluster_scores((int)n, (const int *)(d + o_c), (const uint32_t *)(d + o_sh), (const uint32_t *)(d + o_si),
                               (const float *)(d + o_sq), (const float *)(d + o_st),
                               (const float *)(d + o_sw), d_dist, use_l1, (float *)(d + o_sc), whole, NULL, (uint32_t *)(d + o_tab), oslam_stream()));
    HIPCHK(hipMemcpyAsync(score, d + o_sc, 4 * n, hipMemcpyDeviceToHost, st));
    HIPCHK(hipStreamSynchronize(st));
done:
    free(h);
    return rc;
}
```

objective-slam_amd/csrc/oslam_vote_body.inc:

```
#ifndef OSLAM_VOTE_BODY_INC
#define OSLAM_VOTE_BODY_INC

#define WAVE 64
#ifndef VOTE_THREADS
#define VOTE_THREADS 1024
#endif
#ifndef ACC_STRIDE
#define ACC_STRIDE 31
#endif
#define ACC_CELLS (OSLAMK_ROWS * ACC_STRIDE)
#define ACC_REAL_CELLS (1023 * ACC_STRIDE)

static __device__ const uint32_t k_alpha_thr[32] = {PC_ALPHA_THR_FLAT};

__device__ __forceinline__ uint32_t wave_max_u32(uint32_t v)
{
    for (int o = 32; o > 0; o >>= 1) {
        uint32_t w = __shfl_xor(v, o, WAVE);
        v = v > w ? v : w;
    }
    return v;
}
__device__ __forceinline__ uint32_t wave_sum_u32(uint32_t v)
{
// ... 331 lines not shown
        __syncthreads();
        if (s_qn <= VOTE_QCAP) break;
        T *= 2;
        __syncthreads();
    }
    const uint32_t n_q = uni_u32(s_qn);
    T = uni_u32(T);
    if (PASS == 0 && s_tot[0] > VOTE_WIDE_DIRECT) {
        if (tid == 0) {
            a.redo[atomicAdd(&a.counters->redo_count, 1u)] = wg;
            atomicAdd(&a.counters->redo_total, 1u);
        }
        return;
    }
#ifdef VOTE_PROF
    const long long ptA = clock64();
#endif

    const uint32_t pass = PASS;
    const uint32_t inc_lo = PASS == 2 ? 0u : 1u, inc_hi = PASS == 0 ? 0x10000u : PASS == 2 ? 1u : 0u;
    {
        uint2 B_ru = make_uint2(0, 0), B_inf = make_uint2(0, 0);
        auto bperm = [&](uint32_t from_lane, uint32_t v) -> uint32_t {
            return (uint32_t)__builtin_amdgcn_ds_bpermute((int)(from_lane << 2), (int)v);
        };
        auto step_at = [&](uint32_t ve0, uint32_t vh0, uint32_t vmisc, int l) -> VoteStep {
            VoteStep d;
            const uint32_t misc = readlane_u(vmisc, l);
            d.e0 = readlane_u(ve0, l);
            d.h0 = readlane_u(vh0, l);
            d.ne = d.e0 + (misc >> 20) * 16u;
            d.nh = d.h0 + (misc & 63u) * 8u + 8u;
            d.R = (misc & 63u) + 1u;
            d.i0 = (misc >> 6) & 127u;
            d.i1 = (misc >> 13) & 127u;
            d.nl = misc >> 20;
            d.valid = true;
            return d;
        };
        auto split_of = [&](uint32_t R, bool split) -> uint32_t { return !split ? 0u : R > 32u ? 2u : R > 16u ? 1u : 0u; };
        auto vote_set = [&](bool take, bool split, uint32_t u0, uint32_t stride) {
            uint32_t excl, incl;
            {
                const uint32_t R = (B_ru.x >> OSLAMK_RUN_SHIFT) + 1u;
                const uint32_t nu = take ? (((B_inf.y & 0x7fffffffu) + 255u) >> 8) << split_of(R, split) : 0u;
                incl = nu;
                for (int o = 1; o < WAVE; o <<= 1) {
                    const uint32_t up = __shfl_up(incl, o, WAVE);
                    if (lane >= o) incl += up;
                }
                excl = incl - nu;
            }
            const uint32_t total = readlane_u(incl, WAVE - 1);
            for (uint32_t ub = u0; ub < total; ub += stride * WAVE) {
                const uint32_t u = ub + stride * (uint32_t)lane;
                const bool act = u < total;
                uint32_t lo = 0;
    #pragma unroll
                for (uint32_t s2 = WAVE / 2; s2 > 0; s2 >>= 1) lo += bperm(lo + s2 - 1u, incl) <= u ? s2 : 0u;
                lo = lo < (uint32_t)WAVE - 1u ? lo : (uint32_t)WAVE - 1u;
                const uint32_t st = bperm(lo, B_inf.x), ln = bperm(lo, B_inf.y) & 0x7fffffffu, h0 = bperm(lo, B_ru.y) & 0x7fffffffu;
                const uint32_t R = (bperm(lo, B_ru.x) >> OSLAMK_RUN_SHIFT) + 1u, lg = split_of(R, split);
                const uint32_t local = u - bperm(lo, excl);
                const uint32_t c = local >> lg, hs = local & ((1u << lg) - 1u), per = (R + (1u << lg) - 1u) >> lg;
                const uint32_t i0 = hs * per, i1 = i0 + per < R ? i0 + per : R;
                const uint32_t left = ln - (c << 8), nl = left < 256u ? (left + 3u) >> 2 : 64u;
                const uint32_t w_e0 = act ? (st - e_first + (c << 8)) * 4u : 0u, w_h0 = act ? h0 * 8u : 0u,
                               w_misc = act ? (R - 1u) | (i0 << 6) | (i1 << 13) | (nl << 20) : 0u;
                const uint32_t rest = (total - ub + stride - 1u) / stride, n_w = rest < (uint32_t)WAVE ? rest : (uint32_t)WAVE;
                for (uint32_t g0 = 0; g0 < n_w; g0 += VOTE_GROUP) {
                    VR regs[VOTE_GROUP];
                    VoteStep ds[VOTE_GROUP];
    #pragma unroll
                    for (int g = 0; g < VOTE_GROUP; g++) {
                        ds[g] = step_at(w_e0, w_h0, w_misc, (int)g0 + g);
                        regs[g].load(e4, hits, ds[g], lane);
                    }
                    asm volatile("" ::: "memory");
    #pragma unroll
                    for (int g = 0; g < VOTE_GROUP; g++) regs[g].vote(acc, ds[g], lane, inc_lo, inc_hi);
                }
            }
        };
        const uint32_t *skeys = a.hit_key + off;
        const uint32_t n_hits = a.hit_count[ref_local] < (uint32_t)(a.hit_off[ref_local + 1] - off) ? a.hit_count[ref_local]
                                                                                                   : (uint32_t)(a.hit_off[ref_local + 1] - off);
        const uint32_t n_cq = (n_hits + WAVE - 1u) / WAVE;
        uint32_t cq = uni_u32((uint32_t)wid);
#ifdef VOTE_PROF
        long long prof_corr = 0;
#endif
        auto correct_pass = [&]() {
#ifdef VOTE_PROF
            const long long pc0 = clock64();
#endif
            const uint32_t *pw = a.ent.pw;
            const uint16_t *pdir = a.ent.pdir;
            const uint32_t hit = cq * WAVE + (uint32_t)lane;
            cq += VOTE_THREADS / WAVE;
            const bool in = hit < n_hits;
            const uint32_t kw = skeys[in ? hit : 0u];
            const bool key_ok = (kw & RUN_SLOT_MASK) < a.table.uinfo_stride;
            const oslamk_uinfo ui = uinfo[key_ok ? kw & RUN_SLOT_MASK : 0u];
            uint32_t ln = in && key_ok && !((kw | ui.len) >> 31) ? ui.len : 0u;
            const bool bucket_ok = ln == 0u || (ui.start <= a.ent.n_real && ln <= a.ent.n_real - ui.start);
            if (!bucket_ok) ln = 0;
            if (__ballot((in && !key_ok) || !bucket_ok)) {
                if (in && !key_ok) atomicOr(&a.counters->list_overflow, 2u);
                if (!bucket_ok) atomicOr(&a.counters->list_overflow, 4u);
            }
            const uint32_t A = pc_vote_base_t32(hits[in ? hit : 0u].theta_t22) * 30u - (PC_T24_EDGE - 1u), B = A + (PC_T24_EDGE - 1u);
            for (uint32_t seg = 0; __ballot(seg < ln); seg += OSLAMK_PSEG) {
                const uint32_t n = seg < ln ? (ln - seg < OSLAMK_PSEG ? ln - seg : OSLAMK_PSEG) : 0u;
                const uint32_t sbase = n ? ui.start + seg : 0u, K = OSLAMK_PDIR_CELLS(n);
                const uint32_t cA = __umulhi(A, K), cB = __umulhi(B, K);
                const uint32_t d0 = n ? pdir[((size_t)sbase << OSLAMK_PDIR_SHIFT) + cA] : 0u, d1 = n ? pdir[((size_t)sbase << OSLAMK_PDIR_SHIFT) + cB + 1u] : 0u;
                uint32_t cnt = K == 1u ? n : B < A ? n - d0 + d1 : d1 - d0;
#ifdef VOTE_DIAG_NOCAND
                cnt = 0;
#endif
                if (d0 > n || d1 > n || cnt > 2u * n) {
                    atomicOr(&a.counters->list_overflow, 8u);
                    cnt = 0;
                }
                uint32_t incl = cnt;
                for (int o = 1; o < WAVE; o <<= 1) {
                    const uint32_t up = __shfl_up(incl, o, WAVE);
                    if (lane >= o) incl += up;
                }
                const uint32_t excl = incl - cnt, total = readlane_u(incl, WAVE - 1);
                const uint32_t hit0 = hit - (uint32_t)lane;
                for (uint32_t base = 0; base < total; base += 4u * WAVE) {
                    uint32_t kk[4], own[4], w[4];
                    bool inl[4];
    #pragma unroll
                    for (int u = 0; u < 4; u++) {
                        const uint32_t f = base + (uint32_t)u * WAVE + (uint32_t)lane;
                        inl[u] = f < total;
                        kk[u] = own[u] = w[u] = 0;
                        if (base + (uint32_t)u * WAVE >= total) continue;
                        uint32_t o = 0;
    #pragma unroll
                        for (uint32_t s2 = WAVE / 2; s2 > 0; s2 >>= 1) o += bperm(o + s2 - 1u, incl) <= f ? s2 : 0u;
                        o = o < (uint32_t)WAVE - 1u ? o : (uint32_t)WAVE - 1u;
                        const uint32_t no = bperm(o, n), d0o = bperm(o, d0), exo = bperm(o, excl), sbo = bperm(o, sbase);
                        uint32_t k = d0o + (f - exo);
                        k = k >= no ? k - no : k;
                        k = k < no ? k : 0u;
                        own[u] = o;
                        kk[u] = inl[u] ? sbo + k : 0u;
                        w[u] = pw[kk[u]];
                    }
    #pragma unroll
                    for (int u = 0; u < 4; u++) {
                        if (base + (uint32_t)u * WAVE >= total) continue;
                        const uint32_t Ao = bperm(own[u], A);
                        const bool near = inl[u] && w[u] * 30u - Ao < PC_T24_EDGE;
                        const unsigned long long nm = __ballot(near);
                        if (nm) sq_n = slow_push((lds_ctx *)sc, (lds_u32 *)acc, (lds_u32 *)s_tbl, (lds_u64 *)sq, sq_n, nm, kk[u] | SLOW_VERIFY, (hit0 + own[u]) | (1u << SLOW_HIT_BITS), lane);
                    }
                }
            }
#ifdef VOTE_PROF
            prof_corr += clock64() - pc0;
#endif
        };
        auto marked = [&](const uint2 &ru, const uint2 &inf) -> bool { return MODE == 0 && ((inf.y | ru.y) >> 31); };

        {
            const uint32_t tail_runs = n_runs < VOTE_TAIL_RUNS ? n_runs : VOTE_TAIL_RUNS;
            const uint32_t n_big = (n_runs - tail_runs) / VOTE_BLOCK;
            const uint32_t n_blocks = n_big + (n_runs - n_big * VOTE_BLOCK + VOTE_TAIL - 1) / VOTE_TAIL;
            auto block_first = [&](uint32_t b) -> uint32_t { return b < n_big ? b * VOTE_BLOCK : n_big * VOTE_BLOCK + (b - n_big) * VOTE_TAIL; };
            auto block_len = [&](uint32_t b) -> uint32_t { return b < n_big ? (uint32_t)VOTE_BLOCK : (uint32_t)VOTE_TAIL; };
            const uint32_t my_slot = (uint32_t)lane / VOTE_BLOCK, k_in = (uint32_t)lane % VOTE_BLOCK;
            auto grab = [&]() -> uint32_t {
                uint32_t b = 0;
                if (lane == 0) b = atomicAdd(&s_next, 1u);
                return uni_u32(readlane_u(b, 0));
            };
            auto fetch_runs = [&](uint32_t b, uint32_t slot) {
                if (my_slot == slot) {
                    const uint32_t k = block_first(b) + k_in;
                    B_ru = make_uint2(0, 0);
                    B_inf = make_uint2(0, 0);
                    if (k_in < block_len(b) && k < n_runs) {
                        const oslamk_run rr = runs[k];
                        B_ru = make_uint2(rr.slot_r, rr.first);
                    }
                }
            };
            auto fetch_info = [&](uint32_t b, uint32_t slot) {
                if (my_slot == slot && k_in < block_len(b) && block_first(b) + k_in < n_runs) {
                    const oslamk_uinfo ui = uinfo[B_ru.x & RUN_SLOT_MASK];
                    B_inf = make_uint2(ui.start, ui.len);
                }
            };
            uint32_t cur_b = 0, nx1_b = 0, nx2_b = 0, turn = 0;
            uint32_t tw = 0;
            bool started = false;
            for (;;) {
                bool take, split;
                uint32_t u0, stride;
                if (tw < n_q) {
                    const uint32_t t = tw + (uint32_t)lane;
                    B_ru = make_uint2(0, 0);
                    B_inf = make_uint2(0, 0);
                    if (t < n_q) {
                        const oslamk_run rr = runs[s_q[t]];
                        const oslamk_uinfo ui = uinfo[rr.slot_r & RUN_SLOT_MASK];
                        B_ru = make_uint2(rr.slot_r, rr.first);
                        B_inf = make_uint2(ui.start, ui.len);
                    }
                    tw += WAVE;
                    take = t < n_q;
                    split = true;
                    u0 = uni_u32((uint32_t)wid);
                    stride = VOTE_THREADS / WAVE;
                } else {
                    if (!started) {
                        started = true;
                        cur_b = grab();
                        fetch_runs(cur_b, 0u);
                        nx1_b = grab();
                        fetch_runs(nx1_b, 1u);
                        nx2_b = grab();
                        fetch_runs(nx2_b, 2u);
                        fetch_info(cur_b, 0u);
                        fetch_info(nx1_b, 1u);
                    }
                    if (cur_b >= n_blocks) break;
                    const uint32_t ln = B_inf.y & 0x7fffffffu, R = (B_ru.x >> OSLAMK_RUN_SHIFT) + 1u;
                    take = my_slot == (turn & 3u) && ln != 0u && ((ln + 255u) >> 8) * R <= T && !marked(B_ru, B_inf);
                    split = false;
                    u0 = 0u;
                    stride = 1u;
                    cur_b = nx1_b;
                    nx1_b = nx2_b;
                    fetch_info(nx1_b, (turn + 2u) & 3u);
                    nx2_b = grab();
                    fetch_runs(nx2_b, (turn + 3u) & 3u);
                    turn++;
                }
                vote_set(take, split, u0, stride);
#ifndef VOTE_DIAG_NOCORRECT
                if (MODE == 0 && cq < n_cq) correct_pass();
#endif
            }
        }
#ifndef VOTE_DIAG_NOCORRECT
        if (MODE == 0) {
            while (cq < n_cq) correct_pass();
#ifdef VOTE_PROF
            if (lane == 0) atomicAdd(&a.counters->prof[3], (unsigned long long)prof_corr);
#endif
        }
#endif
        if (MODE == 0) {
            for (uint32_t k0 = (uint32_t)wid * WAVE; k0 < n_runs; k0 += VOTE_THREADS) {
                const uint32_t k = k0 + (uint32_t)lane;
                oslamk_run rr;
                oslamk_uinfo ui;
                rr.slot_r = rr.first = 0;
                ui.start = ui.len = 0;
                if (k < n_runs) {
                    rr = runs[k];
                    ui = uinfo[rr.slot_r & RUN_SLOT_MASK];
                }
                unsigned long long fm = __ballot((ui.len & 0x7fffffffu) != 0u && ((ui.len | rr.first) >> 31));
                while (fm) {
                    const int j = __ffsll((long long)fm) - 1;
                    fm &= fm - 1ull;
                    sq_n = forced_item((lds_ctx *)sc, (lds_u32 *)acc, (lds_u32 *)s_tbl, (lds_u64 *)sq, sq_n, readlane_u(ui.start, j),
                                       readlane_u(ui.len, j) & 0x7fffffffu, readlane_u(rr.first, j) & 0x7fffffffu,
                                       (readlane_u(rr.slot_r, j) >> OSLAMK_RUN_SHIFT) + 1u, lane);
                }
            }
            if (sq_n) slow_queue_flush((lds_ctx *)sc, (lds_u32 *)acc, (lds_u32 *)s_tbl, (lds_u64 *)sq, sq_n, lane);
        }
#ifdef VOTE_PROF
        const long long pt1 = clock64();
#endif
        asm volatile("s_waitcnt lgkmcnt(0)" ::: "memory");
        __syncthreads();
#ifdef VOTE_PROF
        const long long pt2 = clock64();
        if (lane == 0) {
            atomicAdd(&a.counters->prof[0], (unsigned long long)(ptA - pt0));
            atomicAdd(&a.counters->prof[1], (unsigned long long)(pt1 - ptA));
            atomicAdd(&a.counters->prof[2], (unsigned long long)(pt2 - pt1));
        }
#endif


        auto lower_of = [&](uint32_t w) -> uint32_t { return pass == 0 ? w & 0xffffu : pass == 1 ? w : 0u; };
        auto upper_of = [&](uint32_t w) -> uint32_t { return pass == 0 ? w >> 16 : pass == 2 ? w : 0u; };
        uint32_t lmax = 0, nz = 0;
        unsigned long long sum = 0;
#pragma unroll 2
        for (int c = tid; c < ACC_REAL_CELLS; c += VOTE_THREADS) {
            const uint32_t w = acc[c], v0 = lower_of(w), v1 = upper_of(w);
            lmax = max(lmax, max(v0, v1));
            nz += (v0 != 0) + (v1 != 0);
            sum += (unsigned long long)v0 + v1;
        }
        lmax = wave_max_u32(lmax);
        nz = wave_sum_u32(nz);
        sum = wave_sum_u64(sum);
        if (lane == 0) {
            s_wave[wid] = lmax;
            s_wave2[wid] = nz;
            s_sum[wid] = sum;
        }
        __syncthreads();
        if (tid == 0) {
            uint32_t m = 0, n = 0;
            unsigned long long tot = 0;
            for (int w = 0; w < VOTE_THREADS / WAVE; w++) {
                m = s_wave[w] > m ? s_wave[w] : m;
                n += s_wave2[w];
                tot += s_sum[w];
            }
            s_redo = pass == 0 && tot != s_tot[0] - s_ctx.dropped;
#if defined(VOTE_DIAG_NOLOOP) || defined(VOTE_DIAG_NOATOM)
            s_redo = 0;
#endif
            if (s_redo) {
                a.redo[atomicAdd(&a.counters->redo_count, 1u)] = wg;
                atomicAdd(&a.counters->redo_total, 1u);
            }
            if (!s_redo) {
                if (pass <= 1) {
                    const unsigned long long h = slice == 0 ? (unsigned long long)a.hit_count[ref_local] : 0ull;
                    if (h) atomicAdd(&a.counters->hits, h);
                    if (s_tot[0]) atomicAdd(&a.counters->votes, s_tot[0]);
                    if (s_tot[1]) {
                        atomicAdd(&a.counters->entries, s_tot[1] & 0xffffffffffull);
                        atomicAdd(&a.counters->items, s_tot[1] >> 40);
                    }
// ... 81 lines not shown
```

objective-slam_amd/csrc/oslam_vote_plan.h:

```cpp
#ifndef OSLAM_VOTE_PLAN_H
#define OSLAM_VOTE_PLAN_H

#include <stddef.h>
#include <stdint.h>
#include <stdlib.h>

#define OSLAM_BATCH_SLOTS_MAX 0xfffffff0u

typedef struct oslam_vote_batch {
    int first, n;
    size_t slots;
    size_t off_at;
} oslam_vote_batch;

typedef struct oslam_vote_plan {
    oslam_vote_batch *b;
    int nb, cap;
    size_t n_off;
    size_t max_slots;
} oslam_vote_plan;

static inline int oslam_vote_batch_extent(const uint32_t *keep, int first, int n_ref, size_t limit_slots, uint32_t *off,
                                          size_t *slots)
{
    size_t t = 0;
    int n = 0;
    while (first + n < n_ref) {
        const size_t need = ((size_t)keep[first + n] + 1u) & ~(size_t)1u;
        if (n > 0 && (t + need > limit_slots || t + need > OSLAM_BATCH_SLOTS_MAX)) break;
        off[n] = (uint32_t)t;
        t += need;
        n++;
    }
    off[n] = (uint32_t)t;
    *slots = t;
    return n;
}

static inline int oslam_vote_plan_build(oslam_vote_plan *p, const uint32_t *keep, int n_ref, size_t limit_slots, uint32_t *off)
{
    int first = 0;
    p->nb = 0;
    p->n_off = 0;
    p->max_slots = 0;
    while (first < n_ref) {
        oslam_vote_batch *b;
        if (p->nb == p->cap) {
            const int cap = p->cap ? 2 * p->cap : 4;
            oslam_vote_batch *grown = (oslam_vote_batch *)realloc(p->b, sizeof *grown * (size_t)cap);
            if (!grown) { p->nb = 0; p->n_off = 0; p->max_slots = 0; return -1; }
            p->b = grown;
            p->cap = cap;
        }
        b = &p->b[p->nb++];
        b->first = first;
        b->off_at = p->n_off;
        b->n = oslam_vote_batch_extent(keep, first, n_ref, limit_slots, off + p->n_off, &b->slots);
        if (b->slots > p->max_slots) p->max_slots = b->slots;
        p->n_off += (size_t)b->n + 1;
        first += b->n;
    }
    return 0;
}

static inline int oslam_vote_plan_is_one_batch(const oslam_vote_plan *p) { return p->nb == 1; }

#endif
```

objective-slam_amd/ppf.py:

```python
import ctypes as C
import os

import numpy as np

_HERE = os.path.dirname(os.path.abspath(__file__))
LIB_PATH = os.environ.get("OSLAM_LIB", os.path.join(_HERE, "liboslam_hip.so"))
_LIB = None

OSLAM_OK, OSLAM_E_INVALID, OSLAM_E_DEVICE, OSLAM_E_NOMEM, OSLAM_E_NO_VOTES, OSLAM_E_LIMIT, OSLAM_E_PEER = range(7)
STAGE_VOTE, STAGE_SELECT, STAGE_GROW = 1, 2, 3
VOTE_EXACT, VOTE_FAST = 0, 1
COMM_ID_BYTES = 128


class OslamError(RuntimeError):
    def __init__(self, code, msg):
        super().__init__("oslam error %d: %s" % (code, msg))
        self.code = code


class Params(C.Structure):
    _fields_ = [("ref_point_df", C.c_uint), ("vote_count_threshold", C.c_float),
                ("cpu_clustering", C.c_int), ("use_l1_norm", C.c_int), ("use_averaged_clusters", C.c_int),
                ("dev", C.c_int), ("vote_mode", C.c_int), ("shard_rank", C.c_int), ("shard_world", C.c_int),
                ("max_cells", C.c_uint), ("pose_gpu_min", C.c_uint), ("no_bucket_spread", C.c_int),
                ("scratch_gib", C.c_uint), ("pose_two_sorts", C.c_int), ("vote_order", C.c_int), ("reserved", C.c_int * 1)]


class Stats(C.Structure):
    _fields_ = [("num_scene_ppfs", C.c_uint64), ("num_hits", C.c_uint64), ("num_votes", C.c_uint64),
                ("num_unique_votes", C.c_uint64), ("num_model_keys", C.c_uint64), ("num_top", C.c_uint64),
                ("max_count", C.c_uint32), ("num_emitted", C.c_uint32), ("ms_vote", C.c_float),
                ("ms_total", C.c_float), ("vote_launches", C.c_uint32), ("ms_vote_kernel", C.c_float),
                ("ms_key_kernel", C.c_float), ("wide_workgroups", C.c_uint32), ("num_pairs_probed", C.c_uint64),
                ("scratch_bytes", C.c_uint64), ("num_entries_streamed", C.c_uint64), ("num_items", C.c_uint64)]

    def asdict(self):
        return {f: getattr(self, f) for f, _ in self._fields_}


class RefineParams(C.Structure):
    _fields_ = [("max_iterations", C.c_uint), ("max_corr_dist", C.c_float), ("min_normal_dot", C.c_float),
                ("inlier_dist", C.c_float), ("min_fitness", C.c_float), ("stop_rot", C.c_float), ("stop_trans", C.c_float),
                ("reserved", C.c_int * 4)]


class RefineResult(C.Structure):
    _fields_ = [("fitness_in", C.c_float), ("fitness", C.c_float), ("rmse", C.c_float), ("inliers", C.c_uint32),
                ("correspondences", C.c_uint32), ("iterations", C.c_uint32), ("converged", C.c_int32),
                ("found", C.c_int32), ("launches", C.c_uint32), ("ms_total", C.c_float)]

    def asdict(self):
        return {f: getattr(self, f) for f, _ in self._fields_}


class VerifyParams(C.Structure):
    _fields_ = [("depth_tol", C.c_float), ("window", C.c_uint), ("min_view_fitness", C.c_float),
                ("min_coverage", C.c_float), ("min_supported", C.c_uint), ("reserved", C.c_int * 4)]


class VerifyResult(C.Structure):
    _fields_ = [("back", C.c_uint32), ("out", C.c_uint32), ("supported", C.c_uint32), ("occluded", C.c_uint32),
                ("conflict", C.c_uint32), ("unknown", C.c_uint32), ("view_fitness", C.c_float), ("coverage", C.c_float),
                ("found", C.c_int32), ("launches", C.c_uint32), ("ms_total", C.c_float)]

    def asdict(self):
        return {f: getattr(self, f) for f, _ in self._fields_}


VERIFY_BACK, VERIFY_OUT, VERIFY_SUPPORTED, VERIFY_OCCLUDED, VERIFY_CONFLICT, VERIFY_UNKNOWN = range(6)


class InstanceParams(C.Structure):
    _fields_ = [("max_instances", C.c_uint), ("min_separation", C.c_float), ("max_angle", C.c_float),
                ("min_score_ratio", C.c_float), ("keep_not_found", C.c_int), ("reserved", C.c_int * 4)]


class Instance(C.Structure):
    _fields_ = [("T", C.c_float * 16), ("T_vote", C.c_float * 16), ("score", C.c_float), ("candidate", C.c_uint32),
                ("refine", RefineResult)]

    def astuple(self):
        T = np.array(self.T, np.float32).reshape(4, 4)
        return T, {"T_vote": np.array(self.T_vote, np.float32).reshape(4, 4), "score": float(self.score),
                   "candidate": int(self.candidate), "refine": self.refine.asdict()}


MAX_INSTANCES = 64


class ArbitrateParams(C.Structure):
    _fields_ = [("depth_tol", C.c_float), ("window", C.c_uint), ("tile", C.c_uint), ("tile_spacing", C.c_float),
                ("min_tiles", C.c_uint), ("min_owned_share", C.c_float), ("reserved", C.c_int * 4)]


class ArbitrateResult(C.Structure):
    _fields_ = [("claimed", C.c_uint32), ("owned", C.c_uint32), ("share", C.c_float), ("mean_residual", C.c_float),
                ("kept", C.c_int32), ("suppressed_by", C.c_int32), ("tile", C.c_uint32), ("rounds", C.c_uint32),
                ("launches", C.c_uint32), ("ms_total", C.c_float)]

    def asdict(self):
        return {f: getattr(self, f) for f, _ in self._fields_}


class DetectParams(C.Structure):
    _fields_ = [("instances", InstanceParams), ("refine", RefineParams), ("verify", VerifyParams),
                ("arbitrate", ArbitrateParams), ("reserved", C.c_int * 4)]


# ... 375 lines not shown
    "oslam_render_create": (_i, [_vp, _vp, _sz, _vp, _i, _i, C.POINTER(RenderParams), C.POINTER(_vp), _vp]),
    "oslam_db_render": (_i, [_vp, _vp, _vp, _sz, _vp, _i, _i, C.POINTER(RenderParams), C.POINTER(_vp), _vp]),
    "oslam_render_view": (_i, [_vp, C.POINTER(_vp)]),
    "oslam_explain_params_default": (_i, [C.POINTER(ExplainParams)]),
    "oslam_explain": (_i, [_vp, _vp, _sz, _vp, C.POINTER(ExplainParams), _vp]),
    "oslam_db_explain": (_i, [_vp, _vp, _vp, C.POINTER(ExplainParams), _vp]),
    "oslam_explain_rect": (_i, [_vp, C.c_double, _vp, _vp, _i, _i, C.c_uint, _vp]),
    "oslam_explain_z": (_i, [_vp, _vp, _sz, _vp, C.POINTER(ExplainParams), _sz, _vp]),
    "oslam_explain_claims": (_i, [_vp, _vp, _sz, _vp, C.POINTER(ExplainParams), _vp, _vp, _sz, C.POINTER(C.c_uint32),
                                  C.POINTER(_sz)]),
    "oslam_render_labels": (_i, [_vp, _vp]),
    "oslam_render_destroy": (_i, [_vp]),
    "oslam_view_info": (_i, [_vp, _vp, C.POINTER(_i), C.POINTER(_i)]),
    "oslam_mask_params_default": (_i, [C.POINTER(MaskParams)]),
    "oslam_view_mask": (_i, [_vp, _vp, C.POINTER(MaskParams), C.POINTER(_vp), C.POINTER(MaskResult)]),
    "oslam_bilateral_params_default": (_i, [C.POINTER(BilateralParams)]),
    "oslam_view_bilateral": (_i, [_vp, C.POINTER(BilateralParams), C.POINTER(_vp), C.POINTER(BilateralResult)]),
    "oslam_gauss_table": (_i, [_u, C.POINTER(_f)]),
    "oslam_surface_params_default": (_i, [C.POINTER(SurfaceParams)]),
    "oslam_volume_surface": (_i, [_vp, C.POINTER(SurfaceParams), _vp, _vp, _sz, C.POINTER(_sz), C.POINTER(SurfaceResult)]),
    "oslam_scene_from_volume": (_i, [_vp, C.POINTER(SurfaceParams), _f, _f, _u, C.POINTER(Params), C.POINTER(_vp),
                                     C.POINTER(_sz)]),
    "oslam_volume_set_voxels": (_i, [_vp, _vp, _vp]),
    "oslam_volume_shift": (_i, [_vp, _vp, C.POINTER(ShiftResult)]),
    "oslam_volume_window": (_i, [_vp, _vp, _vp]),
    "oslam_volume_leaving": (_i, [_vp, _vp, C.POINTER(SurfaceParams), _vp, _vp, _sz, C.POINTER(_sz), C.POINTER(SurfaceResult)]),
    "oslam_follow_params_default": (_i, [_vp, C.POINTER(FollowParams)]),
    "oslam_volume_follow": (_i, [_vp, _vp, C.POINTER(FollowParams), _vp]),
    "oslam_world_params_of": (_i, [_vp, C.POINTER(WorldParams)]),
    "oslam_world_create": (_i, [C.POINTER(WorldParams), C.POINTER(_vp)]),
    "oslam_world_destroy": (_i, [_vp]),
    "oslam_world_clear": (_i, [_vp]),
    "oslam_world_stats_get": (_i, [_vp, C.POINTER(WorldStats)]),
    "oslam_world_put": (_i, [_vp, _vp, _vp, _sz]),
    "oslam_world_box": (_i, [_vp, _vp, _vp, _vp, _i]),
    "oslam_world_has_colour": (_i, [_vp]),
    "oslam_world_put_colour": (_i, [_vp, _vp, _vp, _vp, _sz]),
    "oslam_world_box_colour": (_i, [_vp, _vp, _vp, _vp, _vp, _i]),
    "oslam_world_colours": (_i, [_vp, _vp, C.POINTER(WorldSurfaceParams), _vp, _sz, _sz, _vp, _vp, C.POINTER(_sz)]),
    "oslam_world_surface_params_default": (_i, [C.POINTER(WorldSurfaceParams)]),
    "oslam_world_surface": (_i, [_vp, _vp, C.POINTER(WorldSurfaceParams), _vp, _vp, _vp, _sz, C.POINTER(_sz),
                                 C.POINTER(WorldSurfaceResult)]),
    "oslam_world_mesh": (_i, [_vp, _vp, C.POINTER(WorldSurfaceParams), _vp, _vp, _vp, _sz, _vp, _sz, C.POINTER(_sz),
                              C.POINTER(_sz), C.POINTER(WorldMeshResult)]),
    "oslam_world_bricks": (_i, [_vp, _vp, _sz, C.POINTER(_sz)]),
    "oslam_world_raycast_params_default": (_i, [C.POINTER(WorldRaycastParams)]),
    "oslam_world_raycast": (_i, [_vp, _vp, C.POINTER(WorldRaycastParams), _vp, _vp, _i, _i, C.POINTER(_vp),
                                 C.POINTER(WorldRaycastResult)]),
    "oslam_world_track": (_i, [_vp, _vp, C.POINTER(WorldRaycastParams), _vp, _vp, C.POINTER(EgomotionParams), _vp,
                               C.POINTER(EgomotionResult)]),
    "oslam_world_paint_view": (_i, [_vp, _vp, C.POINTER(WorldSurfaceParams), _vp, _vp, C.POINTER(C.c_uint32)]),
    "oslam_scene_from_world": (_i, [_vp, _vp, C.POINTER(WorldSurfaceParams), _f, _f, _u, C.POINTER(Params), C.POINTER(_vp),
                                    C.POINTER(_sz)]),
    "oslam_volume_shift_world": (_i, [_vp, _vp, _vp, C.POINTER(ReloadResult)]),
    "oslam_volume_pack": (_i, [_vp, _vp, _vp, _vp, _sz, C.POINTER(_sz)]),
    "oslam_volume_pack_colour": (_i, [_vp, _vp, _vp, _vp, _vp, _sz, C.POINTER(_sz)]),
    "oslam_mesh_params_default": (_i, [C.POINTER(MeshParams)]),
    "oslam_volume_mesh": (_i, [_vp, C.POINTER(MeshParams), _vp, _vp, _sz, _vp, _sz, C.POINTER(_sz), C.POINTER(_sz),
                               C.POINTER(MeshResult)]),
    "oslam_ply_write_mesh": (_i, [C.c_char_p, _vp, _vp, _sz, _vp, _sz, _i]),
    "oslam_mc_table_row": (_i, [_u, _vp, C.POINTER(_u)]),
    "oslam_normals_params_default": (_i, [C.POINTER(NormalsParams)]),
    "oslam_cloud_normals": (_i, [_vp, _sz, _sz, C.POINTER(NormalsParams), _i, _vp, _vp, _vp, C.POINTER(NormalsResult)]),
    "oslam_cloud_normal_moments": (_i, [_vp, _sz, _sz, C.POINTER(NormalsParams), _i, _vp]),
    "oslam_mesh_normals": (_i, [_vp, _sz, _sz, _vp, _sz, _vp, _vp]),
    "oslam_ply_read_mesh": (_i, [C.c_char_p, C.POINTER(_vp), C.POINTER(_vp), C.POINTER(_vp), C.POINTER(_sz), C.POINTER(_sz)]),
    "oslam_view_set_colour": (_i, [_vp, _vp, _sz, _vp]),
    "oslam_view_colour": (_i, [_vp, _vp]),
    "oslam_view_has_colour": (_i, [_vp]),
    "oslam_colour_params_default": (_i, [C.POINTER(ColourParams)]),
    "oslam_volume_colour_enable": (_i, [_vp, C.POINTER(ColourParams)]),
    "oslam_volume_colour_words": (_i, [_vp, _vp]),
    "oslam_volume_set_colour_words": (_i, [_vp, _vp]),
    "oslam_volume_integrate_colour": (_i, [_vp, _vp, _vp, _vp, C.POINTER(IntegrateResult), C.POINTER(C.c_uint32)]),
    "oslam_volume_colours": (_i, [_vp, _vp, _sz, _sz, _vp, _vp, C.POINTER(_sz)]),
    "oslam_volume_paint_view": (_i, [_vp, _vp, _vp, C.POINTER(C.c_uint32)]),
    "oslam_ply_write_colour": (_i, [C.c_char_p, _vp, _vp, _vp, _sz, _i]),
    "oslam_ply_write_mesh_colour": (_i, [C.c_char_p, _vp, _vp, _vp, _sz, _vp, _sz, _i]),
    "oslam_scene_keys": (_i, [_vp, _sz, _vp]),
    "oslam_model_keys": (_i, [_vp, _sz, _vp]),
    "oslam_model_bucket": (_i, [_vp, C.c_uint32, _vp, _sz, C.POINTER(_sz)]),
    "oslam_model_bucket_words": (_i, [_vp, C.c_uint32, _i, _vp, _sz, C.POINTER(_sz)]),
    "oslam_vote_accumulator": (_i, [_vp, _vp, _sz, _vp]),
    "oslam_vote_hits": (_i, [_vp, _vp, _sz, _vp, _vp, _vp, _sz, C.POINTER(_sz), C.POINTER(C.c_uint32)]),
    "oslam_sort_hits_tap": (_i, [_vp, _vp, _vp, _vp, _vp, _sz, C.c_uint32, _i, _vp, _vp, _vp, _vp, _vp]),
    "oslam_model_key_numbers": (_i, [_vp, _vp, _vp, _vp, _sz, C.POINTER(_sz)]),
    "oslam_vote_ref_order": (_i, [_vp, _sz, _vp]),
    "oslam_last_cells": (_i, [_vp, _vp, _vp, _sz, C.POINTER(_sz)]),
    "oslam_tail_scores": (_i, [_vp, _vp, _vp, _sz, C.c_uint32, _i, _vp, _vp, _sz, C.POINTER(_sz), C.POINTER(C.c_uint32), _vp,
                               C.POINTER(_i)]),
    "oslam_set_stream": (_i, [_vp]),
    "oslam_last_error": (C.c_char_p, []),
    "oslam_set_host_threads": (_i, [_i]),
    "oslam_selftest_math": (_i, [_sz, C.c_uint64, C.POINTER(C.c_uint64)]),
}


def lib():
    global _LIB
    if _LIB is None:
        if not os.path.exists(LIB_PATH):
            raise OslamError(OSLAM_E_DEVICE, "%s not built: run `python -c 'import __graft_entry__ as g; g.build()'` "
                                             "(there is no CPU fallback)" % LIB_PATH)
        L = C.CDLL(LIB_PATH)
        for name, (res, args) in _SIGNATURES.items():
            fn = getattr(L, name)
            fn.restype = res
            fn.argtypes = args
        _LIB = L
    return _LIB


def _check(rc):
    if rc != OSLAM_OK:
        raise OslamError(rc, lib().oslam_last_error().decode("utf-8", "replace"))


def _p(a):
    return a.ctypes.data_as(C.c_void_p)


DEFAULT_OVERRIDES = {}


def default_params(**kw):
    p = Params()
    _check(lib().oslam_params_default(C.byref(p)))
    for k, v in {**DEFAULT_OVERRIDES, **kw}.items():
        if not hasattr(p, k):
            raise TypeError("unknown parameter %r" % k)
        setattr(p, k, v)
    return p


def vote_ref_order(keep):
    keep = np.ascontiguousarray(keep, np.uint32)
    out = np.zeros(len(keep), np.uint32)
    _check(lib().oslam_vote_ref_order(_p(keep), len(keep), _p(out)))
    return out


def sort_hits(numbers, theta, idx, offsets, counts, id_bits, dev=0):
    numbers, theta, idx, offsets, counts = (np.ascontiguousarray(a, np.uint32) for a in (numbers, theta, idx, offsets, counts))
    n_lists = len(counts)
    if len(offsets) != n_lists + 1:
        raise ValueError("offsets holds one word more than counts")
    total = int(offsets[-1])
    if not (len(numbers) == len(theta) == len(idx) == total):
        raise ValueError("numbers, theta and idx hold offsets[-1] words each")
    num_o, th_o, idx_o = (np.zeros(max(total, 1), np.uint32) for _ in range(3))
    runs, rc = np.zeros((max(total, 1), 2), np.uint32), np.zeros(max(n_lists, 1), np.uint32)
    _check(lib().oslam_sort_hits_tap(_p(numbers), _p(theta), _p(idx), _p(offsets), _p(counts), n_lists, int(id_bits), int(dev),
                                     _p(num_o), _p(th_o), _p(idx_o), _p(runs), _p(rc)))
    return num_o[:total], th_o[:total], idx_o[:total], runs[:total], rc[:n_lists]


def default_refine_params(**kw):
    p = RefineParams()
    _check(lib().oslam_refine_params_default(C.byref(p)))
    for k, v in kw.items():
        if not hasattr(p, k) or k == "reserved":
            raise TypeError("unknown refine parameter %r" % k)
        setattr(p, k, v)
    return p


# ... 596 lines not shown

    def align_multi(self, scene, comm, allow_no_votes=False):
        T = np.zeros(16, np.float32)
        st = Stats()
        rc = lib().oslam_align_multi(self._h, scene._h, comm._h, _p(T), C.byref(st))
        if not (allow_no_votes and rc == OSLAM_E_NO_VOTES):
            _check(rc)
        self.best_T = T.reshape(4, 4)
        self.stats = st.asdict()
        return self.best_T

    def align_finish(self, scene, cells, global_max, allow_no_votes=False):
        cells = np.ascontiguousarray(cells, CELL_DTYPE)
        T = np.zeros(16, np.float32)
        st = Stats()
        rc = lib().oslam_align_finish(self._h, scene._h, _p(cells), len(cells), int(global_max), _p(T), C.byref(st))
        if not (allow_no_votes and rc == OSLAM_E_NO_VOTES):
            _check(rc)
        self.best_T = T.reshape(4, 4)
        if self.stats is not None:
            self.stats["num_top"], self.stats["max_count"] = st.num_top, st.max_count
        return self.best_T

    def last_cells(self):
        n = C.c_size_t(0)
        _check(lib().oslam_last_cells(self._h, None, None, 0, C.byref(n)))
        cells = np.zeros(n.value, CELL_DTYPE)
        poses = np.zeros((n.value, 16), np.float32)
        if n.value:
            _check(lib().oslam_last_cells(self._h, _p(cells), _p(poses), n.value, C.byref(n)))
        return cells, poses

    @property
    def transformations(self):
        return self.last_cells()[1]

    def last_result(self, scene):
        n = C.c_size_t(0)
        _check(lib().oslam_last_cells(self._h, None, None, 0, C.byref(n)))
        k = max(n.value, 1)
        tr, ro, sc = np.zeros((k, 3), np.float32), np.zeros((k, 4), np.float32), np.zeros(k, np.float32)
        best = C.c_uint32(0)
        _check(lib().oslam_last_result(self._h, scene._h, _p(tr), _p(ro), _p(sc), k, C.byref(n), C.byref(best)))
        return tr[: n.value], ro[: n.value], sc[: n.value], int(best.value)

    def tail_scores(self, scene, cells, global_max, path):
        cells = np.ascontiguousarray(cells, CELL_DTYPE)
        k = max(len(cells), 1)
        kept, sc, T = np.zeros(k, CELL_DTYPE), np.zeros(k, np.float32), np.zeros(16, np.float32)
        n, best, ran = C.c_size_t(0), C.c_uint32(0), C.c_int(-1)
        _check(lib().oslam_tail_scores(self._h, scene._h, _p(cells), len(cells), int(global_max), int(path), _p(kept), _p(sc), k,
                                       C.byref(n), C.byref(best), _p(T), C.byref(ran)))
        return kept[: n.value].copy(), sc[: n.value].copy(), int(best.value), T.reshape(4, 4), int(ran.value)

    def getHashKeys(self, ref_index):
        out = np.zeros(self.n, np.uint32)
        _check(lib().oslam_model_keys(self._h, int(ref_index), _p(out)))
        return out

    def bucket(self, key, cap=1 << 20):
        out = np.zeros(cap, np.uint32)
        n = C.c_size_t(0)
        _check(lib().oslam_model_bucket(self._h, int(key), _p(out), cap, C.byref(n)))
        return out[: min(n.value, cap)].copy(), n.value

    def bucket_words(self, key, slice_index=0, cap=1 << 20):
        out = np.zeros(cap, np.uint32)
        n = C.c_size_t(0)
        _check(lib().oslam_model_bucket_words(self._h, int(key), int(slice_index), _p(out), cap, C.byref(n)))
        return out[: min(n.value, cap)].copy()

    def key_numbers(self):
        n = C.c_size_t(0)
        _check(lib().oslam_model_key_numbers(self._h, None, None, None, 0, C.byref(n)))
        keys, nums, w = np.zeros(n.value, np.uint32), np.zeros(n.value, np.uint32), np.zeros(n.value, np.uint64)
        if n.value:
            _check(lib().oslam_model_key_numbers(self._h, _p(keys), _p(nums), _p(w), n.value, C.byref(n)))
        return keys, nums, w

    def vote_accumulator(self, scene, ref_index):
        acc = np.zeros((self.n, 32), np.uint32)
        _check(lib().oslam_vote_accumulator(self._h, scene._h, int(ref_index), _p(acc)))
        return acc

    def vote_hits(self, scene, ref_index):
        n, keep = C.c_size_t(0), C.c_uint32(0)
        _check(lib().oslam_vote_hits(self._h, scene._h, int(ref_index), None, None, None, 0, C.byref(n), C.byref(keep)))
        num, th, idx = (np.zeros(n.value, np.uint32) for _ in range(3))
        if n.value:
            _check(lib().oslam_vote_hits(self._h, scene._h, int(ref_index), _p(num), _p(th), _p(idx), n.value, C.byref(n), C.byref(keep)))
        return num, th, idx, int(keep.value)

    def close(self):
        if getattr(self, "_db", None) is not None:
            self._db.close()
        if self._h:
            lib().oslam_model_destroy(self._h)
            self._h = C.c_void_p(0)

    def __del__(self):
        try:
            self.close()
        except Exception:
            pass


class Database:

    def __init__(self, models):
        self.models = list(models)
        self._h = C.c_void_p(0)
        arr = (C.c_void_p * len(self.models))(*[m._h for m in self.models])
        _check(lib().oslam_db_create(arr, len(self.models), C.byref(self._h)))
        n, g = C.c_size_t(0), C.c_size_t(0)
        _check(lib().oslam_db_size(self._h, C.byref(n), C.byref(g)))
        self.n_groups = g.value
        for m in self.models:
            m._db = self

    def align(self, scene):
        n = len(self.models)
        T = np.zeros((n, 4, 4), np.float32)
        st = (Stats * n)()
        _check(lib().oslam_db_align(self._h, scene._h, _p(T), st))
        stats = [s.asdict() for s in st]
        for m, t, d in zip(self.models, T, stats):
            m.best_T, m.stats = t, d
        return T, stats

    def refine(self, scene, T, params=None):
        n = len(self.models)
        Ti = np.ascontiguousarray(np.asarray(T, np.float32).reshape(n, 16))
        To = np.zeros((n, 4, 4), np.float32)
        res = (RefineResult * n)()
        p = params if params is not None else default_refine_params()
        _check(lib().oslam_db_refine(self._h, scene._h, _p(Ti), C.byref(p), _p(To), res))
        out = [r.asdict() for r in res]
        return To, out, np.array([bool(r["found"]) for r in out])

    def verify(self, view, T, params=None):
        n = len(self.models)
        Ti = np.ascontiguousarray(np.asarray(T, np.float32).reshape(n, 16))
        res = (VerifyResult * max(n, 1))()
        p = params if params is not None else default_verify_params()
        _check(lib().oslam_db_verify(self._h, view._h, _p(Ti), C.byref(p), res))
        out = [res[j].asdict() for j in range(n)]
        return out, np.array([bool(r["found"]) for r in out], dtype=bool)

    def arbitrate(self, view, T, params=None):
        n = len(self.models)
        Ti = np.ascontiguousarray(np.asarray(T, np.float32).reshape(n, 16))
        res = (ArbitrateResult * max(n, 1))()
        p = params if params is not None else default_arbitrate_params()
        _check(lib().oslam_db_arbitrate(self._h, view._h, _p(Ti), C.byref(p), res))
        out = [res[j].asdict() for j in range(n)]
        return out, np.array([bool(r["kept"]) for r in out], dtype=bool)

    def explain(self, view, T, params=None):
        n = len(self.models)
        Ti = np.ascontiguousarray(np.asarray(T, np.float32).reshape(n, 16))
        res = (ExplainResult * max(n, 1))()
        p = params if params is not None else default_explain_params()
        _check(lib().oslam_db_explain(self._h, view._h, _p(Ti), C.byref(p), res))
        return [res[j].asdict() for j in range(n)]

    def detect(self, scene, view, params=None):
# ... 979 lines not shown
```

Baseline: 26.20 billion scene PPFs/s.

## Move exact-vote edge correction into separate search and re-evaluation kernels

The in-kernel correction pass for exact-mode voting, which searched bucket edges and pushed candidates through a slow LDS queue inside the vote kernel, is taken out. Two pre-pass kernels now do this work. k_edge_search finds near-edge model pairs per hit using a new per-key sorted placement table (kwx/kdir) built across slices. k_edge_reeval recomputes alpha bins and writes compact move records. The vote kernel then only applies these records as atomic subtract/add on its LDS accumulator. This lightens the main vote kernel and spreads the correction work across more blocks, at the cost of extra launches, a global move buffer, a per-key sort prepass, and overflow risk when the buffer is too small.

```diff
diff --git a/include/oslam.h b/include/oslam.h
--- a/include/oslam.h
+++ b/include/oslam.h
@@ -35,7 +35,7 @@
     unsigned scratch_gib;
     int pose_two_sorts;
     int vote_order;
-    int reserved[1];
+    unsigned move_words;
 } oslam_params;
 
 typedef struct oslam_stats {
@@ -796,6 +796,8 @@
 int oslam_vote_accumulator(oslam_model *m, oslam_scene *s, size_t ref_index, uint32_t *acc_out);
 int oslam_vote_hits(oslam_model *m, oslam_scene *s, size_t ref_index, uint32_t *numbers_out, uint32_t *theta_out,
                     uint32_t *idx_out, size_t cap, size_t *n_out, uint32_t *keep_out);
+int oslam_vote_moves(oslam_model *m, oslam_scene *s, size_t ref_index, uint32_t *records_out, size_t cap, size_t *n_out,
+                     uint32_t *acc_out);
 int oslam_sort_hits_tap(const uint32_t *numbers, const uint32_t *theta, const uint32_t *idx, const uint32_t *offsets,
                         const uint32_t *counts, size_t n_lists, uint32_t id_bits, int dev, uint32_t *numbers_out,
                         uint32_t *theta_out, uint32_t *idx_out, uint32_t *runs_out, uint32_t *run_counts_out);
diff --git a/objective-slam_amd/csrc/oslam_edge.hip b/objective-slam_amd/csrc/oslam_edge.hip
--- /dev/null
+++ b/objective-slam_amd/csrc/oslam_edge.hip
@@ -0,0 +1,319 @@
+#include <hip/hip_runtime.h>
+
+#include "oslam_kernels.h"
+#include "ppf_core.h"
+#include "oslam_vote_body.inc"
+
+__global__ void k_key_lens(oslamk_table t, uint32_t *klen)
+{
+    const uint32_t k = blockIdx.x * blockDim.x + threadIdx.x;
+    if (k >= t.uinfo_stride) return;
+    uint32_t n = 0, mark = 0;
+    for (int s = 0; s < t.n_slices; s++) {
+        const uint32_t l = t.uinfo[(size_t)s * t.uinfo_stride + k].len;
+        n += l & 0x7fffffffu;
+        mark |= l & 0x80000000u;
+    }
+    klen[k] = n < 0x7fffffffu ? n | mark : 0x7fffffffu;
+}
+
+#define KEY_SORT_THREADS 256
+__global__ __launch_bounds__(KEY_SORT_THREADS) void k_key_psort(oslamk_table t, oslamk_entries ent, oslamk_kplace *kwx, uint16_t *kdir)
+{
+    __shared__ unsigned long long key[OSLAMK_PSEG];
+    __shared__ uint32_t s_w[OSLAMK_PSEG], s_ix[OSLAMK_PSEG];
+    __shared__ uint32_t s_pre[65], s_st[64], s_mk[64];
+    const uint32_t k = blockIdx.x;
+    const int tid = threadIdx.x;
+    const oslamk_uinfo rec = ent.krec[k];
+    const uint32_t L = rec.len & 0x7fffffffu;
+    if (L == 0) return;
+    if (tid == 0) {
+        uint32_t run = 0;
+        for (int s = 0; s < t.n_slices && s < 64; s++) {
+            const oslamk_uinfo ui = t.uinfo[(size_t)s * t.uinfo_stride + k];
+            s_pre[s] = run;
+            s_st[s] = ui.start;
+            s_mk[s] = ui.len >> 31;
+            run += ui.len & 0x7fffffffu;
+        }
+        s_pre[t.n_slices < 64 ? t.n_slices : 64] = run;
+    }
+    __syncthreads();
+    const int nsl = t.n_slices < 64 ? t.n_slices : 64;
+    if (s_pre[nsl] != L || rec.start > ent.k_real || L > ent.k_real - rec.start) return;
+    for (uint32_t seg = 0; seg < L; seg += OSLAMK_PSEG) {
+        const uint32_t n = L - seg < OSLAMK_PSEG ? L - seg : OSLAMK_PSEG;
+        const size_t base = (size_t)rec.start + seg;
+        uint32_t P = 2;
+        while (P < n) P <<= 1;
+        for (uint32_t i = tid; i < P; i += KEY_SORT_THREADS) {
+            if (i < n) {
+                const uint32_t g = seg + i;
+                int s = 0;
+                while (s + 1 < nsl && s_pre[s + 1] <= g) s++;
+                const uint32_t ix = s_st[s] + (g - s_pre[s]);
+                const uint32_t w = ix < ent.n_real ? ent.pw[ix] : 0u;
+                s_w[i] = w;
+                s_ix[i] = s_mk[s] ? OSLAMK_KPLACE_MARKED : ix;
+                key[i] = ((unsigned long long)(w * 30u) << 32) | i;
+            } else {
+                key[i] = ~0ull;
+            }
+        }
+        __syncthreads();
+        for (uint32_t kk = 2; kk <= P; kk <<= 1) {
+            for (uint32_t j = kk >> 1; j > 0; j >>= 1) {
+                for (uint32_t x = tid; x < P / 2; x += KEY_SORT_THREADS) {
+                    const uint32_t lo = ((x & ~(j - 1)) << 1) | (x & (j - 1)), hi = lo | j;
+                    const unsigned long long a = key[lo], b = key[hi];
+                    const bool up = (lo & kk) == 0;
+                    if ((a > b) == up) { key[lo] = b; key[hi] = a; }
+                }
+                __syncthreads();
+            }
+        }
+        for (uint32_t i = tid; i < n; i += KEY_SORT_THREADS) {
+            const uint32_t src = (uint32_t)key[i];
+            oslamk_kplace pl;
+            pl.w = s_w[src];
+            pl.ix = s_ix[src];
+            kwx[base + i] = pl;
+        }
+        const uint32_t K = OSLAMK_PDIR_CELLS(n);
+        for (uint32_t c = tid; c <= K; c += KEY_SORT_THREADS) {
+            uint32_t lo = 0, hi = n;
+            while (lo < hi) {
+                const uint32_t mid = (lo + hi) >> 1;
+                const uint32_t cell = (uint32_t)(((key[mid] >> 32) * (unsigned long long)K) >> 32);
+                if (cell < c) lo = mid + 1; else hi = mid;
+            }
+            kdir[(base << OSLAMK_PDIR_SHIFT) + c] = (uint16_t)lo;
+        }
+        __syncthreads();
+    }
+}
+
+#ifndef EDGE_THREADS
+#define EDGE_THREADS 256
+#endif
+#define EDGE_WAVES (EDGE_THREADS / WAVE)
+#ifndef EDGE_SPLIT
+#define EDGE_SPLIT 4
+#endif
+#ifndef EDGE_REEVAL_THREADS
+#define EDGE_REEVAL_THREADS 256
+#endif
+#define EDGE_QCAP 128
+#define EDGE_ITEM 3u
+
+__device__ __forceinline__ uint32_t *edge_region(const oslamk_vote_args &a, uint32_t ref_local, uint32_t &words)
+{
+    const unsigned long long r0 = oslamk_move_at(a.hit_off[ref_local], a.mv_w16), r1 = oslamk_move_at(a.hit_off[ref_local + 1], a.mv_w16);
+    words = r1 - r0 < 0xffffffffull ? (uint32_t)(r1 - r0) : 0xffffffffu;
+    return a.mv_buf + r0;
+}
+
+__global__ __launch_bounds__(EDGE_THREADS) void k_edge_search(oslamk_vote_args a)
+{
+    __shared__ uint32_t s_q[EDGE_WAVES][EDGE_ITEM * EDGE_QCAP];
+    const int tid = threadIdx.x, lane = tid & (WAVE - 1), wid = tid / WAVE;
+    const uint32_t ref_local = a.ref_order ? uni_u32(a.ref_order[blockIdx.x]) : blockIdx.x;
+    if (ref_local >= (uint32_t)a.n_launch) return;
+    const size_t off = a.hit_off[ref_local];
+    const uint32_t slots = (uint32_t)(a.hit_off[ref_local + 1] - off);
+    const uint32_t n_hits = a.hit_count[ref_local] < slots ? a.hit_count[ref_local] : slots;
+    const uint32_t n_pass = (n_hits + WAVE - 1u) / WAVE;
+    const oslamk_pay *hits = a.hit_sorted + off;
+    const uint32_t *skeys = a.hit_key + off;
+    const oslamk_kplace *kwx = a.ent.kwx;
+    const uint16_t *kdir = a.ent.kdir;
+    uint32_t *q = s_q[wid];
+    uint32_t qn = 0;
+    uint32_t room;
+    uint32_t *region = edge_region(a, ref_local, room);
+    auto flush = [&]() {
+        asm volatile("s_waitcnt lgkmcnt(0)" ::: "memory");
+        uint32_t at = 0, ok = 0;
+        if (lane == 0) {
+            at = atomicAdd(&a.mv_item_head[ref_local], EDGE_ITEM * qn);
+            ok = at <= room && EDGE_ITEM * qn <= room - at;
+            if (!ok) atomicOr(&a.counters->list_overflow, 16u);
+        }
+        ok = readlane_u(ok, 0);
+        at = readlane_u(at, 0);
+        if (ok)
+            for (uint32_t i = (uint32_t)lane; i < EDGE_ITEM * qn; i += WAVE) region[at + i] = q[i];
+        asm volatile("" ::: "memory");
+        qn = 0;
+    };
+    auto bperm = [&](uint32_t from_lane, uint32_t v) -> uint32_t {
+        return (uint32_t)__builtin_amdgcn_ds_bpermute((int)(from_lane << 2), (int)v);
+    };
+
+    for (uint32_t pass = blockIdx.y * EDGE_WAVES + (uint32_t)wid; pass < n_pass; pass += EDGE_WAVES * gridDim.y) {
+        const uint32_t hit = pass * WAVE + (uint32_t)lane;
+        const bool in = hit < n_hits;
+        const uint32_t kwd = skeys[in ? hit : 0u];
+        const bool key_ok = (kwd & RUN_SLOT_MASK) < a.table.uinfo_stride;
+        const oslamk_uinfo kr = a.ent.krec[key_ok ? kwd & RUN_SLOT_MASK : 0u];
+        uint32_t ln = in && key_ok && !(kwd >> 31) ? kr.len & 0x7fffffffu : 0u;
+        const bool places_ok = ln == 0u || (kr.start <= a.ent.k_real && ln <= a.ent.k_real - kr.start);
+        if (!places_ok) ln = 0;
+        if (__ballot((in && !key_ok) || !places_ok)) {
+            if (in && !key_ok) atomicOr(&a.counters->list_overflow, 2u);
+            if (!places_ok) atomicOr(&a.counters->list_overflow, 4u);
+        }
+        const uint32_t A = pc_vote_base_t32(hits[in ? hit : 0u].theta_t22) * 30u - (PC_T24_EDGE - 1u), B = A + (PC_T24_EDGE - 1u);
+        for (uint32_t seg = 0; __ballot(seg < ln); seg += OSLAMK_PSEG) {
+            const uint32_t n = seg < ln ? (ln - seg < OSLAMK_PSEG ? ln - seg : OSLAMK_PSEG) : 0u;
+            const uint32_t sbase = n ? kr.start + seg : 0u, K = OSLAMK_PDIR_CELLS(n);
+            const uint32_t cA = __umulhi(A, K), cB = __umulhi(B, K);
+            const uint32_t d0 = n ? kdir[((size_t)sbase << OSLAMK_PDIR_SHIFT) + cA] : 0u, d1 = n ? kdir[((size_t)sbase << OSLAMK_PDIR_SHIFT) + cB + 1u] : 0u;
+            uint32_t cnt = K == 1u ? n : B < A ? n - d0 + d1 : d1 - d0;
+            if (d0 > n || d1 > n || cnt > 2u * n) {
+                atomicOr(&a.counters->list_overflow, 8u);
+                cnt = 0;
+            }
+            uint32_t incl = cnt;
+            for (int o = 1; o < WAVE; o <<= 1) {
+                const uint32_t up = __shfl_up(incl, o, WAVE);
+                if (lane >= o) incl += up;
+            }
+            const uint32_t excl = incl - cnt, total = readlane_u(incl, WAVE - 1);
+            const uint32_t hit0 = pass * WAVE;
+            for (uint32_t base = 0; base < total; base += 4u * WAVE) {
+                uint32_t own[4];
+                oslamk_kplace w[4];
+                bool inl[4];
+#pragma unroll
+                for (int u = 0; u < 4; u++) {
+                    const uint32_t f = base + (uint32_t)u * WAVE + (uint32_t)lane;
+                    inl[u] = f < total;
+                    own[u] = 0;
+                    w[u].w = w[u].ix = 0;
+                    if (base + (uint32_t)u * WAVE >= total) continue;
+                    uint32_t o = 0;
+#pragma unroll
+                    for (uint32_t s2 = WAVE / 2; s2 > 0; s2 >>= 1) o += bperm(o + s2 - 1u, incl) <= f ? s2 : 0u;
+                    o = o < (uint32_t)WAVE - 1u ? o : (uint32_t)WAVE - 1u;
+                    const uint32_t no = bperm(o, n), d0o = bperm(o, d0), exo = bperm(o, excl), sbo = bperm(o, sbase);
+                    uint32_t k = d0o + (f - exo);
+                    k = k >= no ? k - no : k;
+                    k = k < no ? k : 0u;
+                    own[u] = o;
+                    w[u] = kwx[inl[u] ? sbo + k : 0u];
+                }
+#pragma unroll
+                for (int u = 0; u < 4; u++) {
+                    if (base + (uint32_t)u * WAVE >= total) continue;
+                    const uint32_t Ao = bperm(own[u], A);
+                    const bool near = inl[u] && w[u].w * 30u - Ao < PC_T24_EDGE;
+                    const unsigned long long nm = __ballot(near);
+                    if (nm) {
+                        if (qn > EDGE_QCAP - WAVE) flush();
+                        if (near) {
+                            const uint32_t at = qn + (uint32_t)__popcll(nm & ((1ull << lane) - 1ull));
+                            q[EDGE_ITEM * at] = w[u].w;
+                            q[EDGE_ITEM * at + 1u] = w[u].ix;
+                            q[EDGE_ITEM * at + 2u] = hit0 + own[u];
+                        }
+                        qn += (uint32_t)__popcll(nm);
+                    }
+                }
+            }
+        }
+    }
+    if (qn) flush();
+}
+
+__global__ __launch_bounds__(EDGE_REEVAL_THREADS) void k_edge_reeval(oslamk_vote_args a)
+{
+    __shared__ uint32_t s_tbl[32], s_first[64], s_count;
+    const int tid = threadIdx.x, lane = tid & (WAVE - 1);
+    const uint32_t ref_local = a.ref_order ? uni_u32(a.ref_order[blockIdx.x]) : blockIdx.x;
+    if (ref_local >= (uint32_t)a.n_launch) return;
+    if (tid < 32) s_tbl[tid] = k_alpha_thr[tid];
+    if (tid < 64) s_first[tid] = tid < a.table.n_slices ? a.table.slots[(size_t)tid * a.table.cap].start : 0xffffffffu;
+    if (tid == 0) s_count = 0;
+    __syncthreads();
+    const size_t off = a.hit_off[ref_local];
+    const uint32_t slots = (uint32_t)(a.hit_off[ref_local + 1] - off);
+    const uint32_t n_hits = a.hit_count[ref_local] < slots ? a.hit_count[ref_local] : slots;
+    const oslamk_pay *hits = a.hit_sorted + off;
+    const float *rows = a.tsg + 8 * (size_t)(a.first_ref + (int)ref_local);
+    const uint32_t n_slices = (uint32_t)a.table.n_slices < 64u ? (uint32_t)a.table.n_slices : 64u;
+    uint32_t room;
+    uint32_t *region = edge_region(a, ref_local, room);
+    const uint32_t asked = a.mv_item_head[ref_local];
+    const uint32_t n_items = asked <= room ? asked / EDGE_ITEM : 0u;
+    for (uint32_t base = 0; base < n_items; base += EDGE_REEVAL_THREADS) {
+        const uint32_t it = base + (uint32_t)tid;
+        uint32_t ew = 0, ix = 0, hi = 0;
+        if (it < n_items) {
+            ew = region[EDGE_ITEM * it];
+            ix = region[EDGE_ITEM * it + 1u];
+            hi = region[EDGE_ITEM * it + 2u];
+        }
+        __syncthreads();
+        bool move = false;
+        uint32_t record = 0;
+        if (it < n_items) {
+            if (hi >= n_hits) {
+                atomicOr(&a.counters->list_overflow, 32u);
+            } else {
+                const oslamk_pay hp = hits[hi];
+                if (ix == OSLAMK_KPLACE_MARKED) {
+                } else if (ix >= a.ent.n_real || hp.idx >= (uint32_t)a.scene.n) {
+                    atomicOr(&a.counters->list_overflow, 4u);
+                } else {
+                    uint32_t sl = 0;
+                    for (uint32_t s2 = 1; s2 < n_slices; s2++) sl += s_first[s2] <= ix;
+                    const uint32_t i = hp.idx;
+                    const float x = a.scene.px[i], y = a.scene.py[i], z = a.scene.pz[i];
+                    const float vy = pc_row_dot(rows, x, y, z);
+                    const float vz = pc_row_dot(rows + 4, x, y, z);
+                    const float2 uv = *reinterpret_cast<const float2 *>(&a.ent.puv[ix]);
+                    const unsigned bin = alpha_bin_reeval(uv.x, uv.y, vy, vz, s_tbl);
+                    uint32_t qbin, pos;
+                    vote_product(pc_vote_base_t32(hp.theta_t22) - ew, qbin, pos);
+                    move = bin != qbin;
+                    record = OSLAMK_MOVE(sl, ew & PC_ROW10_MASK, (ew >> PC_ROW_HALF_BIT) & 1u, qbin & 31u,
+                                         bin < OSLAMK_NBIN ? bin : OSLAMK_MOVE_DROPPED);
+                }
+            }
+        }
+        const unsigned long long mm = __ballot(move);
+        if (mm) {
+            uint32_t at = 0;
+            if (lane == 0) at = atomicAdd(&s_count, (uint32_t)__popcll(mm));
+            at = readlane_u(at, 0);
+            if (move) region[at + (uint32_t)__popcll(mm & ((1ull << lane) - 1ull))] = record;
+        }
+    }
+    __syncthreads();
+    if (tid == 0) a.mv_head[ref_local] = s_count;
+}
+
+extern "C" int oslamk_key_lens(oslamk_table t, uint32_t *klen, void *stream)
+{
+    if (t.uinfo_stride == 0) return 0;
+    hipLaunchKernelGGL(k_key_lens, dim3((t.uinfo_stride + 255u) / 256u), dim3(256), 0, (hipStream_t)stream, t, klen);
+    return (int)hipGetLastError();
+}
+
+extern "C" int oslamk_key_psort(oslamk_table t, oslamk_entries ent, oslamk_kplace *kwx, uint16_t *kdir, void *stream)
+{
+    if (t.uinfo_stride == 0) return 0;
+    hipLaunchKernelGGL(k_key_psort, dim3(t.uinfo_stride), dim3(KEY_SORT_THREADS), 0, (hipStream_t)stream, t, ent, kwx, kdir);
+    return (int)hipGetLastError();
+}
+
+extern "C" int oslamk_edge_moves(const oslamk_vote_args *a, void *stream)
+{
+    if (a->n_launch <= 0 || a->mode != 0) return 0;
+    if (!a->ent.krec || !a->mv_buf || !a->mv_item_head) return (int)hipErrorInvalidValue;
+    hipLaunchKernelGGL(k_edge_search, dim3((unsigned)a->n_launch, EDGE_SPLIT), dim3(EDGE_THREADS), 0, (hipStream_t)stream, *a);
+    hipLaunchKernelGGL(k_edge_reeval, dim3((unsigned)a->n_launch), dim3(EDGE_REEVAL_THREADS), 0, (hipStream_t)stream, *a);
+    return (int)hipGetLastError();
+}
diff --git a/objective-slam_amd/csrc/oslam_host.c b/objective-slam_amd/csrc/oslam_host.c
--- a/objective-slam_amd/csrc/oslam_host.c
+++ b/objective-slam_amd/csrc/oslam_host.c
@@ -46,6 +46,7 @@
     p->no_bucket_spread = 0;
     p->scratch_gib = 0;
     p->vote_order = 0;
+    p->move_words = 0;
     return OSLAM_OK;
 }
 
diff --git a/objective-slam_amd/csrc/oslam_internal.h b/objective-slam_amd/csrc/oslam_internal.h
--- a/objective-slam_amd/csrc/oslam_internal.h
+++ b/objective-slam_amd/csrc/oslam_internal.h
@@ -179,6 +179,7 @@
     uint32_t launches;
     uint64_t probed;
 } oslam_vote_times;
+int oslam_pool_read_moves(const scratch_pool *p, uint32_t *records_out, size_t cap, size_t *n_out);
 int oslam_pool_read_hits(const scratch_pool *p, uint32_t *numbers_out, uint32_t *theta_out, uint32_t *idx_out, size_t cap,
                          size_t *n_out, uint32_t *keep_out);
 int oslam_run_votes_group(scratch_pool *pool, oslam_model *const *ms, int nm, oslam_scene *s, const uint32_t *d_ref_idx,
diff --git a/objective-slam_amd/csrc/oslam_kernels.h b/objective-slam_amd/csrc/oslam_kernels.h
--- a/objective-slam_amd/csrc/oslam_kernels.h
+++ b/objective-slam_amd/csrc/oslam_kernels.h
@@ -18,6 +18,11 @@
     uint32_t len;
     uint32_t cur;
 } oslamk_slot;
+
+typedef struct oslamk_uinfo {
+    uint32_t start;
+    uint32_t len;
+} oslamk_uinfo;
 
 typedef struct oslamk_uv {
     float uy, uz;
@@ -31,7 +36,15 @@
     oslamk_uv *puv;
     uint16_t *pdir;
     uint32_t n_real;
+    const oslamk_uinfo *krec;
+    const struct oslamk_kplace *kwx;
+    const uint16_t *kdir;
+    uint32_t k_real;
 } oslamk_entries;
+typedef struct oslamk_kplace {
+    uint32_t w, ix;
+} oslamk_kplace;
+#define OSLAMK_KPLACE_MARKED 0xffffffffu
 #define OSLAMK_PSEG 4096
 #ifndef OSLAMK_PDIR_SHIFT
 #define OSLAMK_PDIR_SHIFT 0
@@ -50,11 +63,6 @@
     const float *box;
 } oslamk_order;
 #define OSLAMK_ORDER_GROUP 64
-
-typedef struct oslamk_uinfo {
-    uint32_t start;
-    uint32_t len;
-} oslamk_uinfo;
 
 typedef struct oslamk_table {
     oslamk_slot *slots;
@@ -155,9 +163,25 @@
     uint32_t *redo;
     const uint32_t *ref_order;
     oslamk_order order;
+    uint32_t *mv_buf, *mv_head, *mv_item_head;
+    uint32_t mv_w16;
 } oslamk_vote_args;
 
+#define oslamk_move_at(off, w16) (((unsigned long long)(off) * (unsigned long long)(w16)) >> 4)
+
+#define OSLAMK_MOVE(slice, row, half, qbin, rbin) ((uint32_t)(slice) << 22 | (uint32_t)(row) << 12 | (uint32_t)(half) << 11 | (uint32_t)(qbin) << 6 | (uint32_t)(rbin))
+#define OSLAMK_MOVE_SLICE(r) ((r) >> 22 & 63u)
+#define OSLAMK_MOVE_ROW(r) ((r) >> 12 & 1023u)
+#define OSLAMK_MOVE_HALF(r) ((r) >> 11 & 1u)
+#define OSLAMK_MOVE_QBIN(r) ((r) >> 6 & 31u)
+#define OSLAMK_MOVE_RBIN(r) ((r) & 63u)
+#define OSLAMK_MOVE_DROPPED 63u
+
 int oslamk_uinfo_build(oslamk_table t, void *stream);
+
+int oslamk_key_lens(oslamk_table t, uint32_t *klen, void *stream);
+int oslamk_key_psort(oslamk_table t, oslamk_entries ent, oslamk_kplace *kwx, uint16_t *kdir, void *stream);
+int oslamk_edge_moves(const oslamk_vote_args *a, void *stream);
 
 int oslamk_scene_count(const oslamk_vote_args *a, void *stream);
 int oslamk_scene_hits(const oslamk_vote_args *a, void *stream);
diff --git a/objective-slam_amd/csrc/oslam_model.c b/objective-slam_amd/csrc/oslam_model.c
--- a/objective-slam_amd/csrc/oslam_model.c
+++ b/objective-slam_amd/csrc/oslam_model.c
@@ -3,6 +3,17 @@
 #include "oslam_internal.h"
 #include "oslam_pose.h"
 #include "ppf_core.h"
+
+static void key_order_free(oslam_model *m)
+{
+    if (m->ent.krec) (void)hipFree((void *)m->ent.krec);
+    if (m->ent.kwx) (void)hipFree((void *)m->ent.kwx);
+    if (m->ent.kdir) (void)hipFree((void *)m->ent.kdir);
+    m->ent.krec = NULL;
+    m->ent.kwx = NULL;
+    m->ent.kdir = NULL;
+    m->ent.k_real = 0;
+}
 
 void oslam_model_destroy(oslam_model *m)
 {
@@ -15,6 +26,7 @@
     if (m->ent.pw) (void)hipFree(m->ent.pw);
     if (m->ent.puv) (void)hipFree(m->ent.puv);
     if (m->ent.pdir) (void)hipFree(m->ent.pdir);
+    key_order_free(m);
     if (m->ent.mi) (void)hipFree(m->ent.mi);
     if (m->table.ukeys && !m->shared_union) (void)hipFree(m->table.ukeys);
     if (m->table.reach && !m->shared_union) (void)hipFree(m->table.reach);
@@ -187,6 +199,62 @@
     return rc;
 }
 
+static int build_key_order(oslam_model *m)
+{
+    int rc = OSLAM_OK;
+    const size_t nk = m->table.uinfo_stride;
+    uint32_t *d_len = NULL, *h_len = NULL;
+    oslamk_kplace *kwx = NULL;
+    uint16_t *kdir = NULL;
+    oslamk_uinfo *h_rec = NULL, *d_rec = NULL;
+    uint64_t run = 0;
+    size_t k, places;
+    key_order_free(m);
+    if (!m->ent.pw || nk == 0) return OSLAM_OK;
+    h_len = (uint32_t *)malloc(sizeof(uint32_t) * nk);
+    h_rec = (oslamk_uinfo *)malloc(sizeof(oslamk_uinfo) * nk);
+    if (!h_len || !h_rec) { rc = fail(OSLAM_E_NOMEM, "host allocation failed"); goto done; }
+    HIPCHK(hipMalloc((void **)&d_len, sizeof(uint32_t) * nk));
+    KCHK(oslamk_key_lens(m->table, d_len, oslam_stream()));
+    HIPCHK(hipStreamSynchronize((hipStream_t)oslam_stream()));
+    HIPCHK(hipMemcpy(h_len, d_len, sizeof(uint32_t) * nk, hipMemcpyDeviceToHost));
+    for (k = 0; k < nk; k++) {
+        const uint32_t n = h_len[k] & 0x7fffffffu;
+        h_rec[k].start = (uint32_t)run;
+        h_rec[k].len = h_len[k];
+        run += ((uint64_t)n + 1u) & ~(uint64_t)1u;
+        if (n == 0x7fffffffu || run > 0xfffffff0ull) { rc = fail(OSLAM_E_LIMIT, "the model's entries do not fit the key-wide order"); goto done; }
+    }
+    places = (size_t)run + 8;
+    HIPCHK(hipMalloc((void **)&d_rec, sizeof(oslamk_uinfo) * nk));
+    HIPCHK(hipMalloc((void **)&kwx, sizeof(oslamk_kplace) * places));
+    HIPCHK(hipMalloc((void **)&kdir, sizeof(uint16_t) * (places << OSLAMK_PDIR_SHIFT)));
+    HIPCHK(hipMemcpy(d_rec, h_rec, sizeof(oslamk_uinfo) * nk, hipMemcpyHostToDevice));
+    HIPCHK(hipMemsetAsync(kwx, 0, sizeof(oslamk_kplace) * places, (hipStream_t)oslam_stream()));
+    HIPCHK(hipMemsetAsync(kdir, 0, sizeof(uint16_t) * (places << OSLAMK_PDIR_SHIFT), (hipStream_t)oslam_stream()));
+    m->ent.krec = d_rec;
+    m->ent.k_real = (uint32_t)run;
+    KCHK(oslamk_key_psort(m->table, m->ent, kwx, kdir, oslam_stream()));
+    HIPCHK(hipStreamSynchronize((hipStream_t)oslam_stream()));
+    m->ent.kwx = kwx;
+    m->ent.kdir = kdir;
+    d_rec = NULL;
+    kwx = NULL;
+    kdir = NULL;
+done:
+    free(h_len);
+    free(h_rec);
+    if (d_len) (void)hipFree(d_len);
+    if (rc != OSLAM_OK) {
+        if (d_rec) (void)hipFree(d_rec);
+        if (kwx) (void)hipFree(kwx);
+        if (kdir) (void)hipFree(kdir);
+        m->ent.krec = NULL;
+        m->ent.k_real = 0;
+    }
+    return rc;
+}
+
 int oslam_build_uinfo(oslam_model *m)
 {
     int rc = OSLAM_OK;
@@ -195,6 +263,7 @@
     HIPCHK(hipMalloc((void **)&m->table.uinfo, bytes));
     HIPCHK(hipMemsetAsync(m->table.uinfo, 0, bytes, (hipStream_t)oslam_stream()));
     KCHK(oslamk_uinfo_build(m->table, oslam_stream()));
+    rc = build_key_order(m);
 done:
     return rc;
 }
@@ -555,7 +624,7 @@
         *table_bytes = sizeof(oslamk_slot) * (uint64_t)m->table.cap * (uint64_t)m->table.n_slices +
                        sizeof(uint32_t) * (uint64_t)m->table.ucap + sizeof(uint32_t) * (OSLAMK_REACH_BINS / 32) +
                        sizeof(oslamk_uinfo) * (uint64_t)m->table.uinfo_stride * (uint64_t)m->table.n_slices +
-                       (uint64_t)m->n_entries * (4 + 2 + (m->ent.pw ? 12 + (2 << OSLAMK_PDIR_SHIFT) : 0)) + 24ull * (uint64_t)m->c.n;
+                       (uint64_t)m->n_entries * (4 + 2 + (m->ent.pw ? 12 + (2 << OSLAMK_PDIR_SHIFT) : 0) + (m->ent.krec ? 8 + (2 << OSLAMK_PDIR_SHIFT) : 0)) + 24ull * (uint64_t)m->c.n;
     return OSLAM_OK;
 }
 
diff --git a/objective-slam_amd/csrc/oslam_taps.c b/objective-slam_amd/csrc/oslam_taps.c
--- a/objective-slam_amd/csrc/oslam_taps.c
+++ b/objective-slam_amd/csrc/oslam_taps.c
@@ -171,7 +171,8 @@
 }
 
 static int tap_one_ref(oslam_model *m, oslam_scene *s, size_t ref_index, uint32_t *acc_out, uint32_t *numbers_out,
-                       uint32_t *theta_out, uint32_t *idx_out, size_t cap, size_t *n_out, uint32_t *keep_out)
+                       uint32_t *theta_out, uint32_t *idx_out, size_t cap, size_t *n_out, uint32_t *keep_out,
+                       uint32_t *moves_out, size_t moves_cap, size_t *n_moves_out)
 {
     int rc = OSLAM_OK;
     uint32_t *d_dump = NULL, *d_ref = NULL, *h_dump = NULL;
@@ -199,6 +200,10 @@
         rc = oslam_pool_read_hits(pool, numbers_out, theta_out, idx_out, cap, n_out, keep_out);
         if (rc != OSLAM_OK) goto done;
     }
+    if (n_moves_out) {
+        rc = oslam_pool_read_moves(pool, moves_out, moves_cap, n_moves_out);
+        if (rc != OSLAM_OK) goto done;
+    }
     if (acc_out) {
         h_dump = (uint32_t *)malloc(sizeof(uint32_t) * cells);
         if (!h_dump) { rc = fail(OSLAM_E_NOMEM, "host allocation failed"); goto done; }
@@ -217,7 +222,7 @@
 int oslam_vote_accumulator(oslam_model *m, oslam_scene *s, size_t ref_index, uint32_t *acc_out)
 {
     if (!acc_out) return fail(OSLAM_E_INVALID, "bad reference index");
-    return tap_one_ref(m, s, ref_index, acc_out, NULL, NULL, NULL, 0, NULL, NULL);
+    return tap_one_ref(m, s, ref_index, acc_out, NULL, NULL, NULL, 0, NULL, NULL, NULL, 0, NULL);
 }
 
 int oslam_vote_hits(oslam_model *m, oslam_scene *s, size_t ref_index, uint32_t *numbers_out, uint32_t *theta_out,
@@ -225,7 +230,17 @@
 {
     if (!n_out) return fail(OSLAM_E_INVALID, "NULL argument");
     *n_out = 0;
-    return tap_one_ref(m, s, ref_index, NULL, numbers_out, theta_out, idx_out, cap, n_out, keep_out);
+    return tap_one_ref(m, s, ref_index, NULL, numbers_out, theta_out, idx_out, cap, n_out, keep_out, NULL, 0, NULL);
+}
+
+int oslam_vote_moves(oslam_model *m, oslam_scene *s, size_t ref_index, uint32_t *records_out, size_t cap, size_t *n_out,
+                     uint32_t *acc_out)
+{
+    size_t n_hits = 0;
+    if (!n_out) return fail(OSLAM_E_INVALID, "NULL argument");
+    *n_out = 0;
+    if (m && m->params.vote_mode == OSLAM_VOTE_FAST) return fail(OSLAM_E_INVALID, "fast vote mode moves no votes");
+    return tap_one_ref(m, s, ref_index, acc_out, NULL, NULL, NULL, 0, &n_hits, NULL, records_out, cap, n_out);
 }
 
 int oslam_sort_hits_tap(const uint32_t *numbers, const uint32_t *theta, const uint32_t *idx, const uint32_t *offsets,
diff --git a/objective-slam_amd/csrc/oslam_vote.c b/objective-slam_amd/csrc/oslam_vote.c
--- a/objective-slam_amd/csrc/oslam_vote.c
+++ b/objective-slam_amd/csrc/oslam_vote.c
@@ -32,14 +32,18 @@
     BUF_REDO,
     BUF_VARGS,
     BUF_ORDER,
+    BUF_MOVES,
     N_BUFS
 };
-static const int g_buf_host[N_BUFS] = {HOST_NONE, HOST_MALLOC, HOST_NONE, HOST_NONE, HOST_PINNED, HOST_PINNED};
+static const int g_buf_host[N_BUFS] = {HOST_NONE, HOST_MALLOC, HOST_NONE, HOST_NONE, HOST_PINNED, HOST_PINNED, HOST_NONE};
 
 struct scratch_pool {
     pthread_mutex_t lock;
     pool_buf b[N_BUFS];
     oslam_vote_plan plan;
+    size_t mv_heads, mv_area;
+    uint32_t mv_w16;
+    uint32_t mv_floor;
     hipEvent_t ev[N_EVENTS];
     int have_events;
 };
@@ -126,6 +130,7 @@
     oslam_ego_release();
     free(p->plan.b);
     memset(&p->plan, 0, sizeof p->plan);
+    p->mv_floor = 0;
     oslam_pool_unlock(p);
     return OSLAM_OK;
 }
@@ -216,6 +221,24 @@
     return rc;
 }
 
+int oslam_pool_read_moves(const scratch_pool *p, uint32_t *records_out, size_t cap, size_t *n_out)
+{
+    int rc = OSLAM_OK;
+    const uint32_t *blk = (const uint32_t *)p->b[BUF_MOVES].d;
+    uint32_t n = 0;
+    size_t room;
+    *n_out = 0;
+    if (!blk || p->plan.nb < 1) return OSLAM_OK;
+    room = (size_t)oslamk_move_at(p->plan.b[0].slots, p->mv_w16);
+    HIPCHK(hipMemcpy(&n, blk, sizeof n, hipMemcpyDeviceToHost));
+    if (n > room) n = (uint32_t)room;
+    *n_out = n;
+    if (n > cap) n = (uint32_t)cap;
+    if (n && records_out) HIPCHK(hipMemcpy(records_out, blk + p->mv_heads, sizeof(uint32_t) * n, hipMemcpyDeviceToHost));
+done:
+    return rc;
+}
+
 #define REF_ORDER_CLASSES 1024
 void oslam_ref_order(const uint32_t *keep, size_t n, uint32_t *order)
 {
@@ -242,6 +265,10 @@
     size_t redo_stride;
     int ordered;
     int one_grid;
+    int repeat;
+    int exact;
+    size_t mv_area;
+    uint32_t mv_w16;
 } vote_pass;
 
 static void member_args(oslamk_vote_args *a, const oslam_model *m)
@@ -286,6 +313,7 @@
     v->a.fixed_gmax = fixed_gmax;
     v->a.acc_dump = acc_dump;
     v->a.dump_ref = acc_dump ? 0 : -1;
+    for (j = 0; j < nm; j++) if (ms[j]->params.vote_mode != OSLAM_VOTE_FAST) v->exact = 1;
     member_args(&v->a, ms[0]);
 }
 
@@ -356,6 +384,21 @@
     if (rc != OSLAM_OK) return rc;
     if (plan->n_off) HIPCHK(hipMemcpyAsync(v->d_off, v->h_off, sizeof(uint32_t) * plan->n_off, hipMemcpyHostToDevice, v->st));
     v->one_grid = v->one_grid && oslam_vote_plan_is_one_batch(plan);
+    if (v->exact) {
+        const size_t heads = 2 * (size_t)v->nm * (size_t)(v->n_ref > 0 ? v->n_ref : 1);
+        const unsigned forced = v->ms[0]->params.move_words;
+        size_t need;
+        v->mv_w16 = OSLAM_MOVE_W16;
+        if (forced && !v->repeat) v->mv_w16 = forced;
+        else if (v->mv_w16 < v->pool->mv_floor) v->mv_w16 = v->pool->mv_floor;
+        if (v->mv_w16 > OSLAM_MOVE_W16_MAX) v->mv_w16 = OSLAM_MOVE_W16_MAX;
+        v->mv_area = oslam_move_area_words(plan->max_slots, v->mv_w16);
+        v->pool->mv_heads = heads;
+        v->pool->mv_area = v->mv_area;
+        v->pool->mv_w16 = v->mv_w16;
+        need = heads + (size_t)v->nm * v->mv_area;
+        rc = pool_buf_grow(&v->pool->b[BUF_MOVES], need, need + need / 8, sizeof(uint32_t) * (need + need / 8), 0);
+    }
 done:
     return rc;
 }
@@ -386,8 +429,22 @@
         HIPCHK(hipMemcpyAsync(d_order, h_order, sizeof(uint32_t) * (size_t)b->n, hipMemcpyHostToDevice, v->st));
         a->ref_order = d_order;
     }
+    a->mv_buf = a->mv_head = a->mv_item_head = NULL;
+    a->mv_w16 = 0;
+    if (v->exact) {
+        a->mv_w16 = v->mv_w16;
+        HIPCHK(hipMemsetAsync(pool->b[BUF_MOVES].d, 0, sizeof(uint32_t) * 2 * (size_t)v->nm * (size_t)b->n, v->st));
+    }
     for (j = 0; j < v->nm; j++) {
         member_args(a, v->ms[j]);
+        if (v->exact) {
+            a->mv_head = (uint32_t *)pool->b[BUF_MOVES].d + 2 * (size_t)j * (size_t)b->n;
+            a->mv_item_head = a->mv_head + b->n;
+            a->mv_buf = (uint32_t *)pool->b[BUF_MOVES].d + pool->mv_heads + (size_t)j * v->mv_area;
+        }
+#ifndef VOTE_DIAG_NOCORRECT
+        KCHK(oslamk_edge_moves(a, oslam_stream()));
+#endif
         if (v->one_grid) {
             a->redo = (uint32_t *)pool->b[BUF_REDO].d + (size_t)j * v->redo_stride;
             h_vargs[j] = *a;
@@ -422,8 +479,18 @@
         }
     if (again) HIPCHK(hipStreamSynchronize(v->st));
     for (j = 0; j < v->nm; j++)
+        if ((cnt[j].list_overflow & ~16u) == 0 && (cnt[j].list_overflow & 16u)) again = 2;
+    for (j = 0; j < v->nm; j++) if (cnt[j].list_overflow & ~16u) again = 0;
+    if (again == 2) {
+        if (v->mv_w16 >= OSLAM_MOVE_W16_MAX) return fail(OSLAM_E_LIMIT, "a reference point's near-edge list exceeds 4096 words per place of its hit list");
+        pool->mv_floor = 2 * v->mv_w16;
+        if (t) t->launches += (uint32_t)pool->plan.nb;
+        return OSLAM_E_MOVES_AGAIN;
+    }
+    for (j = 0; j < v->nm; j++)
         if (cnt[j].list_overflow)
-            return fail(OSLAM_E_DEVICE, cnt[j].list_overflow & 1u
+            return fail(OSLAM_E_DEVICE, cnt[j].list_overflow & 32u ? "near-edge search: an item names a place or a hit out of range"
+                            : cnt[j].list_overflow & 1u
                             ? "a hit list overflowed: the counting pass and the hit pass disagreed on the pairs within reach"
                             : cnt[j].list_overflow & 2u ? "near-edge search: a hit's key number lies outside the model's bucket records"
                             : cnt[j].list_overflow & 4u ? "near-edge search: a bucket lies outside the model's entry arrays"
@@ -447,16 +514,27 @@
                           oslam_vote_times *t)
 {
     vote_pass v;
-    int rc = OSLAM_OK, j, nb;
+    int rc = OSLAM_OK, j, nb, tries = 0;
     pass_open(&v, pool, ms, nm, s, d_ref_idx, d_tsg, n_ref, fixed_gmax, acc_dump);
     rc = pass_reserve(&v);
     if (rc != OSLAM_OK) return rc;
-    for (j = 0; j < nm; j++) HIPCHK(hipMemsetAsync(ms[j]->d_counters, 0, sizeof(oslamk_counters), v.st));
-    HIPCHK(hipEventRecord(pool->ev[0], v.st));
-    rc = pass_demand(&v, t);
-    if (rc == OSLAM_OK) rc = pass_plan(&v);
-    for (nb = 0; rc == OSLAM_OK && nb < pool->plan.nb; nb++) rc = pass_batch(&v, nb);
-    if (rc == OSLAM_OK) rc = pass_collect(&v, cnt, t);
+    do {
+        oslam_vote_times t0;
+        if (t) t0 = *t;
+        for (j = 0; j < nm; j++) HIPCHK(hipMemsetAsync(ms[j]->d_counters, 0, sizeof(oslamk_counters), v.st));
+        HIPCHK(hipEventRecord(pool->ev[0], v.st));
+        rc = pass_demand(&v, t);
+        if (rc == OSLAM_OK) rc = pass_plan(&v);
+        for (nb = 0; rc == OSLAM_OK && nb < pool->plan.nb; nb++) rc = pass_batch(&v, nb);
+        if (rc == OSLAM_OK) rc = pass_collect(&v, cnt, t);
+        if (rc == OSLAM_E_MOVES_AGAIN && t) {
+            const uint32_t launches = t->launches;
+            *t = t0;
+            t->launches = launches;
+        }
+        v.repeat = 1;
+    } while (rc == OSLAM_E_MOVES_AGAIN && ++tries < 40);
+    if (rc == OSLAM_E_MOVES_AGAIN) rc = fail(OSLAM_E_LIMIT, "the near-edge move lists kept overflowing");
 done:
     return rc;
 }
@@ -534,6 +612,25 @@
         }
     }
     t.ms += ms_first;
+    if (getenv("OSLAM_PROF") && pool->b[BUF_MOVES].d && pool->plan.nb == 1 && s->n_ref > 0) {
+        uint32_t *h = (uint32_t *)malloc(sizeof(uint32_t) * 2 * (size_t)s->n_ref);
+        if (h && hipMemcpy(h, pool->b[BUF_MOVES].d, sizeof(uint32_t) * 2 * (size_t)s->n_ref, hipMemcpyDeviceToHost) == hipSuccess) {
+            unsigned long long recs = 0, words = 0;
+            double fullest = 0.0;
+            uint32_t most = 0;
+            int i;
+            for (i = 0; i < s->n_ref; i++) {
+                const double given = (double)(oslamk_move_at(pool->plan.b[0].slots ? ((const uint32_t *)pool->b[BUF_COUNTS].h)[i] : 0, pool->mv_w16));
+                recs += h[i];
+                words += h[s->n_ref + i];
+                if (h[i] > most) most = h[i];
+                if (given > 0.0 && h[s->n_ref + i] / given > fullest) fullest = h[s->n_ref + i] / given;
+            }
+            fprintf(stderr, "[oslam prof] near-edge lists: %llu items, %llu moves (most of one reference point: %u), fullest region %.3f of its words, %llu hits\n",
+                    words / 2, recs, most, fullest, (unsigned long long)cnt->hits);
+        }
+        free(h);
+    }
     if (getenv("OSLAM_PROF"))
         fprintf(stderr, "[oslam prof] k_vote wave cycles: pre-scan %llu, voting %llu, wait at the barrier behind it %llu, "
                         "of the voting: near-edge search %llu\n",
diff --git a/objective-slam_amd/csrc/oslam_vote_body.inc b/objective-slam_amd/csrc/oslam_vote_body.inc
--- a/objective-slam_amd/csrc/oslam_vote_body.inc
+++ b/objective-slam_amd/csrc/oslam_vote_body.inc
@@ -437,88 +437,20 @@
                 }
             }
         };
-        const uint32_t *skeys = a.hit_key + off;
-        const uint32_t n_hits = a.hit_count[ref_local] < (uint32_t)(a.hit_off[ref_local + 1] - off) ? a.hit_count[ref_local]
-                                                                                                   : (uint32_t)(a.hit_off[ref_local + 1] - off);
-        const uint32_t n_cq = (n_hits + WAVE - 1u) / WAVE;
-        uint32_t cq = uni_u32((uint32_t)wid);
-#ifdef VOTE_PROF
-        long long prof_corr = 0;
-#endif
-        auto correct_pass = [&]() {
-#ifdef VOTE_PROF
-            const long long pc0 = clock64();
-#endif
-            const uint32_t *pw = a.ent.pw;
-            const uint16_t *pdir = a.ent.pdir;
-            const uint32_t hit = cq * WAVE + (uint32_t)lane;
-            cq += VOTE_THREADS / WAVE;
-            const bool in = hit < n_hits;
-            const uint32_t kw = skeys[in ? hit : 0u];
-            const bool key_ok = (kw & RUN_SLOT_MASK) < a.table.uinfo_stride;
-            const oslamk_uinfo ui = uinfo[key_ok ? kw & RUN_SLOT_MASK : 0u];
-            uint32_t ln = in && key_ok && !((kw | ui.len) >> 31) ? ui.len : 0u;
-            const bool bucket_ok = ln == 0u || (ui.start <= a.ent.n_real && ln <= a.ent.n_real - ui.start);
-            if (!bucket_ok) ln = 0;
-            if (__ballot((in && !key_ok) || !bucket_ok)) {
-                if (in && !key_ok) atomicOr(&a.counters->list_overflow, 2u);
-                if (!bucket_ok) atomicOr(&a.counters->list_overflow, 4u);
-            }
-            const uint32_t A = pc_vote_base_t32(hits[in ? hit : 0u].theta_t22) * 30u - (PC_T24_EDGE - 1u), B = A + (PC_T24_EDGE - 1u);
-            for (uint32_t seg = 0; __ballot(seg < ln); seg += OSLAMK_PSEG) {
-                const uint32_t n = seg < ln ? (ln - seg < OSLAMK_PSEG ? ln - seg : OSLAMK_PSEG) : 0u;
-                const uint32_t sbase = n ? ui.start + seg : 0u, K = OSLAMK_PDIR_CELLS(n);
-                const uint32_t cA = __umulhi(A, K), cB = __umulhi(B, K);
-                const uint32_t d0 = n ? pdir[((size_t)sbase << OSLAMK_PDIR_SHIFT) + cA] : 0u, d1 = n ? pdir[((size_t)sbase << OSLAMK_PDIR_SHIFT) + cB + 1u] : 0u;
-                uint32_t cnt = K == 1u ? n : B < A ? n - d0 + d1 : d1 - d0;
-#ifdef VOTE_DIAG_NOCAND
-                cnt = 0;
-#endif
-                if (d0 > n || d1 > n || cnt > 2u * n) {
-                    atomicOr(&a.counters->list_overflow, 8u);
-                    cnt = 0;
-                }
-                uint32_t incl = cnt;
-                for (int o = 1; o < WAVE; o <<= 1) {
-                    const uint32_t up = __shfl_up(incl, o, WAVE);
-                    if (lane >= o) incl += up;
-                }
-                const uint32_t excl = incl - cnt, total = readlane_u(incl, WAVE - 1);
-                const uint32_t hit0 = hit - (uint32_t)lane;
-                for (uint32_t base = 0; base < total; base += 4u * WAVE) {
-                    uint32_t kk[4], own[4], w[4];
-                    bool inl[4];
-    #pragma unroll
-                    for (int u = 0; u < 4; u++) {
-                        const uint32_t f = base + (uint32_t)u * WAVE + (uint32_t)lane;
-                        inl[u] = f < total;
-                        kk[u] = own[u] = w[u] = 0;
-                        if (base + (uint32_t)u * WAVE >= total) continue;
-                        uint32_t o = 0;
-    #pragma unroll
-                        for (uint32_t s2 = WAVE / 2; s2 > 0; s2 >>= 1) o += bperm(o + s2 - 1u, incl) <= f ? s2 : 0u;
-                        o = o < (uint32_t)WAVE - 1u ? o : (uint32_t)WAVE - 1u;
-                        const uint32_t no = bperm(o, n), d0o = bperm(o, d0), exo = bperm(o, excl), sbo = bperm(o, sbase);
-                        uint32_t k = d0o + (f - exo);
-                        k = k >= no ? k - no : k;
-                        k = k < no ? k : 0u;
-                        own[u] = o;
-                        kk[u] = inl[u] ? sbo + k : 0u;
-                        w[u] = pw[kk[u]];
-                    }
-    #pragma unroll
-                    for (int u = 0; u < 4; u++) {
-                        if (base + (uint32_t)u * WAVE >= total) continue;
-                        const uint32_t Ao = bperm(own[u], A);
-                        const bool near = inl[u] && w[u] * 30u - Ao < PC_T24_EDGE;
-                        const unsigned long long nm = __ballot(near);
-                        if (nm) sq_n = slow_push((lds_ctx *)sc, (lds_u32 *)acc, (lds_u32 *)s_tbl, (lds_u64 *)sq, sq_n, nm, kk[u] | SLOW_VERIFY, (hit0 + own[u]) | (1u << SLOW_HIT_BITS), lane);
-                    }
-                }
-            }
-#ifdef VOTE_PROF
-            prof_corr += clock64() - pc0;
-#endif
+        auto apply_moves = [&]() {
+            const unsigned long long r0 = oslamk_move_at(off, a.mv_w16), r1 = oslamk_move_at(a.hit_off[ref_local + 1], a.mv_w16);
+            const uint32_t room = r1 - r0 < 0xffffffffull ? (uint32_t)(r1 - r0) : 0xffffffffu, have = a.mv_head[ref_local];
+            const uint32_t n = have < room ? have : room;
+            const uint32_t *recs = a.mv_buf + r0;
+            for (uint32_t i = (uint32_t)tid; i < n; i += VOTE_THREADS) {
+                const uint32_t rec = recs[i];
+                if (OSLAMK_MOVE_SLICE(rec) != (uint32_t)slice) continue;
+                const uint32_t row = OSLAMK_MOVE_ROW(rec), rbin = OSLAMK_MOVE_RBIN(rec);
+                const uint32_t inc = OSLAMK_MOVE_HALF(rec) ? sc->inc_hi : sc->inc_lo;
+                atomicSub((uint32_t *)&acc[row * ACC_STRIDE + OSLAMK_MOVE_QBIN(rec)], inc);
+                if (rbin < OSLAMK_NBIN) atomicAdd((uint32_t *)&acc[row * ACC_STRIDE + rbin], inc);
+                else atomicAdd((uint32_t *)&s_ctx.dropped, 1u);
+            }
         };
         auto marked = [&](const uint2 &ru, const uint2 &inf) -> bool { return MODE == 0 && ((inf.y | ru.y) >> 31); };
 
@@ -598,18 +530,10 @@
                     turn++;
                 }
                 vote_set(take, split, u0, stride);
+            }
+        }
 #ifndef VOTE_DIAG_NOCORRECT
-                if (MODE == 0 && cq < n_cq) correct_pass();
-#endif
-            }
-        }
-#ifndef VOTE_DIAG_NOCORRECT
-        if (MODE == 0) {
-            while (cq < n_cq) correct_pass();
-#ifdef VOTE_PROF
-            if (lane == 0) atomicAdd(&a.counters->prof[3], (unsigned long long)prof_corr);
-#endif
-        }
+        if (MODE == 0) apply_moves();
 #endif
         if (MODE == 0) {
             for (uint32_t k0 = (uint32_t)wid * WAVE; k0 < n_runs; k0 += VOTE_THREADS) {
diff --git a/objective-slam_amd/csrc/oslam_vote_plan.h b/objective-slam_amd/csrc/oslam_vote_plan.h
--- a/objective-slam_amd/csrc/oslam_vote_plan.h
+++ b/objective-slam_amd/csrc/oslam_vote_plan.h
@@ -63,6 +63,14 @@
     return 0;
 }
 
+#define OSLAM_MOVE_W16 48u
+#define OSLAM_MOVE_W16_MAX (1u << 16)
+static inline size_t oslam_move_area_words(size_t max_slots, uint32_t w16)
+{
+    return (size_t)(((unsigned long long)max_slots * w16) >> 4) + 16u;
+}
+#define OSLAM_E_MOVES_AGAIN (-1000)
+
 static inline int oslam_vote_plan_is_one_batch(const oslam_vote_plan *p) { return p->nb == 1; }
 
 #endif
diff --git a/objective-slam_amd/ppf.py b/objective-slam_amd/ppf.py
--- a/objective-slam_amd/ppf.py
+++ b/objective-slam_amd/ppf.py
@@ -24,7 +24,7 @@
                 ("cpu_clustering", C.c_int), ("use_l1_norm", C.c_int), ("use_averaged_clusters", C.c_int),
                 ("dev", C.c_int), ("vote_mode", C.c_int), ("shard_rank", C.c_int), ("shard_world", C.c_int),
                 ("max_cells", C.c_uint), ("pose_gpu_min", C.c_uint), ("no_bucket_spread", C.c_int),
-                ("scratch_gib", C.c_uint), ("pose_two_sorts", C.c_int), ("vote_order", C.c_int), ("reserved", C.c_int * 1)]
+                ("scratch_gib", C.c_uint), ("pose_two_sorts", C.c_int), ("vote_order", C.c_int), ("move_words", C.c_uint)]
 
 
 class Stats(C.Structure):
@@ -566,6 +566,7 @@
     "oslam_model_bucket": (_i, [_vp, C.c_uint32, _vp, _sz, C.POINTER(_sz)]),
     "oslam_model_bucket_words": (_i, [_vp, C.c_uint32, _i, _vp, _sz, C.POINTER(_sz)]),
     "oslam_vote_accumulator": (_i, [_vp, _vp, _sz, _vp]),
+    "oslam_vote_moves": (_i, [_vp, _vp, _sz, _vp, _sz, C.POINTER(_sz), _vp]),
     "oslam_vote_hits": (_i, [_vp, _vp, _sz, _vp, _vp, _vp, _sz, C.POINTER(_sz), C.POINTER(C.c_uint32)]),
     "oslam_sort_hits_tap": (_i, [_vp, _vp, _vp, _vp, _vp, _sz, C.c_uint32, _i, _vp, _vp, _vp, _vp, _vp]),
     "oslam_model_key_numbers": (_i, [_vp, _vp, _vp, _vp, _sz, C.POINTER(_sz)]),
@@ -1328,6 +1329,14 @@
         acc = np.zeros((self.n, 32), np.uint32)
         _check(lib().oslam_vote_accumulator(self._h, scene._h, int(ref_index), _p(acc)))
         return acc
+
+    def vote_moves(self, scene, ref_index):
+        n = C.c_size_t(0)
+        _check(lib().oslam_vote_moves(self._h, scene._h, int(ref_index), None, 0, C.byref(n), None))
+        rec = np.zeros(max(n.value, 1), np.uint32)
+        acc = np.zeros((self.n, 32), np.uint32)
+        _check(lib().oslam_vote_moves(self._h, scene._h, int(ref_index), _p(rec), n.value, C.byref(n), _p(acc)))
+        return rec[: n.value].copy(), acc
 
     def vote_hits(self, scene, ref_index):
         n, keep = C.c_size_t(0), C.c_uint32(0)
```

Result: no change. 26.04 billion scene PPFs/s (-0.6%).
